# slothfulxtx/Texture-GS

Hardware: AMD Instinct MI355X
Metric: fwd+bwd views/sec @800x800, 300k Gaussians + 1024^2 texture; HBM GB/s vs roofline (higher is better)
Workload: dtype f32; 1 GPU; c3: N=300000 Gaussians, cubemap 6x1024x1024x3 f32, 800x800, fwd+bwd, sh_degree 3; parallelism=views sharded dp1, view_pipeline=3 HIP streams, order=accumulate, forwards begun one view per stream ahead, grad_allreduce=none (1 GPU)

## Files before the change

### include/texgs.h

```cpp
#ifndef TEXGS_H
#define TEXGS_H

#include <stddef.h>
#include <stdint.h>

#ifdef __cplusplus
extern "C" {
#endif

#define TEXGS_ABI_VERSION 19
#define TEXGS_TILE 16
#define TEXGS_REC_TEST_FLOATS 8
#define TEXGS_REC_SHADE_FLOATS 20
#define TEXGS_ACC_FLOATS 32

typedef struct TexGSFrame {
    int32_t image_height;
    int32_t image_width;
    float   tanfovx;
    float   tanfovy;
    float   scale_modifier;
    int32_t sh_degree;
    int32_t sh_coeffs;
    int32_t tex_res;
    int32_t num_gaussians;
    int32_t debug;
    const float* bg;
    const float* viewmatrix;
    const float* projmatrix;
    const float* campos;
} TexGSFrame;

typedef struct TexGSInputs {
    const float* means3D;
    const float* shs;
    const float* opacities;
    const float* scales;
    const float* rotations;
    const float* uvs;
    const float* gradient_uvs;
    const float* texture;
    const float* color_offset;
    const float* cov3D_precomp;
} TexGSInputs;

typedef struct TexGSGeom {
    float*    rec_test;
    float*    rec_shade;
    float*    depth;
    int32_t*  radii;
    uint32_t* rect;
    uint32_t* tiles_touched;
    uint32_t* offsets;
    void*     scan_temp;
    size_t    scan_temp_bytes;
} TexGSGeom;

typedef struct TexGSBinning {
    uint32_t  num_rendered;
    uint64_t* keys_unsorted;
    uint64_t* keys_sorted;
    uint32_t* point_list;
    uint32_t* ranges;
    uint32_t* tile_order;
    void*     sort_temp;
    size_t    sort_temp_bytes;
} TexGSBinning;

typedef struct TexGSImage {
    float*    out_color;
    float*    out_depth;
    float*    out_norm;
    float*    out_alpha;
    float*    final_T;
    uint32_t* n_contrib;
    uint32_t* tex_bin_count;
    uint32_t* survivors;
    uint16_t* surv_qmask;
    uint32_t* surv_count;
    uint32_t* tex_bin_resv;
} TexGSImage;
#define TEXGS_RESV_WORDS 192

#define TEXGS_ACC_MEANS3D 1
#define TEXGS_ACC_MEANS2D 2
#define TEXGS_ACC_SHS 4
#define TEXGS_ACC_OPACITIES 8
#define TEXGS_ACC_SCALES 16
#define TEXGS_ACC_ROTATIONS 32
#define TEXGS_ACC_UVS 64
#define TEXGS_ACC_COLOR_OFFSET 128
#define TEXGS_ACC_COV3D 256
#define TEXGS_ACC_ALL 511

#define TEXGS_WANT_TEXTURE   1
#define TEXGS_WANT_GAUSSIANS 2
#define TEXGS_WANT_ALL       3

typedef struct TexGSGrads {
    const float* dL_dcolor;
    const float* dL_ddepth;
    const float* dL_dnorm;
    const float* dL_dalpha;
    float* acc;
    float* dL_dmeans3D;
    float* dL_dmeans2D;
    float* dL_dshs;
    float* dL_dopacities;
    float* dL_dscales;
    float* dL_drotations;
    float* dL_duvs;
    float* dL_dtexture;
    float* dL_dcolor_offset;
    float* dL_dcov3D;
    uint32_t want;
    float*    tex_bins;
    uint32_t* tex_bin_cursor;
    uint32_t* tex_bin_base;
    uint32_t  tex_rec_cap;
    int32_t accumulate;
} TexGSGrads;

int         texgs_abi_version(void);
const char* texgs_build_id(void);
const char* texgs_last_error(void);

size_t texgs_scan_temp_bytes(int32_t num_gaussians);
size_t texgs_sort_temp_bytes(uint32_t num_rendered, uint32_t num_tiles);
size_t texgs_tex_bin_count(int32_t tex_res);
#define TEXGS_TEXBIN_RECORD_FLOATS 4

int texgs_preprocess_forward(const TexGSFrame* frame, const TexGSInputs* in, TexGSGeom* geom, void* stream);

size_t texgs_num_rendered_words(int32_t num_gaussians);
int texgs_num_rendered_begin(const TexGSGeom* geom, int32_t num_gaussians, uint32_t* host_pinned, size_t host_words, int32_t sort_first,
                             void* stream);
int texgs_num_rendered_reduce(const uint32_t* host_pinned, int32_t num_gaussians, uint32_t* host_out, uint64_t* fingerprint_out);
int texgs_depth_sort_scan(TexGSGeom* geom, int32_t num_gaussians, void* stream);

int texgs_bin_sort_render_forward(const TexGSFrame* frame, const TexGSInputs* in, const TexGSGeom* geom,
                                  TexGSBinning* bin, TexGSImage* img, void* stream);

int texgs_render_forward(const TexGSFrame* frame, const TexGSInputs* in, const TexGSGeom* geom,
                         const TexGSBinning* bin, TexGSImage* img, void* stream);

int texgs_backward(const TexGSFrame* frame, const TexGSInputs* in, const TexGSGeom* geom,
                   const TexGSBinning* bin, const TexGSImage* img, TexGSGrads* grads, void* stream);

int texgs_backward_render(const TexGSFrame* frame, const TexGSInputs* in, const TexGSGeom* geom,
                          const TexGSBinning* bin, const TexGSImage* img, TexGSGrads* grads, void* stream);
int texgs_backward_preprocess(const TexGSFrame* frame, const TexGSInputs* in, const TexGSGeom* geom, TexGSGrads* grads,
                              void* stream);

enum {
    TEXGS_K_PREPROCESS_FWD = 0, TEXGS_K_SCAN = 1, TEXGS_K_DUPLICATE = 2, TEXGS_K_SORT = 3, TEXGS_K_RANGES = 4,
    TEXGS_K_RENDER_FWD = 5, TEXGS_K_RENDER_BWD = 6, TEXGS_K_PREPROCESS_BWD = 7, TEXGS_K_TEXGRAD_REDUCE = 8,
    TEXGS_NUM_KERNELS = 9
};
int texgs_profile_enable(int on);
int texgs_profile_select(uint32_t kernel_mask);
int texgs_profile_read(float* ms_sum_host, uint32_t* launches_host);

int texgs_rgb_alpha_loss(const float* image, const float* gt_image, const float* alpha, const float* gt_alpha,
                         int32_t H, int32_t W, float lambda_dssim, float lambda_alpha, float* scratch, float* sums,
                         float* dL_dimage, float* dL_dalpha, void* stream);

int texgs_geom_losses(const float* norm, const float* gt_norm, const float* gt_image, const float* mask, const float* depth,
                      const float* gt_depth, int32_t H, int32_t W, float lambda_norm, float lambda_smooth, float gamma,
                      float lambda_depth, float* sums, float* dL_dnorm, float* dL_ddepth, void* stream);

int texgs_norm_from_depth(const float* depth, const float* viewmatrix, float tanfovx, float tanfovy, int32_t H, int32_t W,
                          float threshold, float* out_norm, float* out_mask, void* stream);

typedef struct TexGSUVNet {
    const float *W1, *b1;
    const float *W2, *b2;
    const float *emb;
    const float *W3, *b3, *W4, *b4;
    const float *W5, *b5;
    const float *xyz_offset, *xyz_scale;
    int32_t hidden;
} TexGSUVNet;
enum { TEXGS_UV_FP32 = 0, TEXGS_UV_BF16X3 = 1, TEXGS_UV_MIXED = 2 };
size_t texgs_uv_packed_bytes(int32_t precision);
int texgs_uv_pack(const TexGSUVNet* net, int32_t precision, void* packed, void* stream);
int texgs_uv_taylor_packed(const TexGSUVNet* net, int32_t precision, const void* packed, const float* xyz, int32_t N, float* uvs,
                           float* grad_uvs, void* stream);

typedef struct TexGSUVNetGrad {
    float *dW1, *db1;
    float *dW2, *db2;
    float *dW3, *db3, *dW4, *db4;
    float *dW5, *db5;
} TexGSUVNetGrad;
size_t texgs_uv_backward_temp_bytes(int32_t N);
int texgs_uv_backward(const TexGSUVNet* net, int32_t precision, const float* xyz, const float* g_uvs, int32_t N, const TexGSUVNetGrad* out,
                      void* temp, void* stream);

#define TEXGS_HASHGRID_MAX_LEVELS 16
#define TEXGS_HASHGRID_FEATURES 4
typedef struct TexGSHashGrid {
    int32_t n_levels;
    int32_t n_features;
    int32_t log2_hashmap_size;
    float   base_resolution;
    float   per_level_scale;
} TexGSHashGrid;
int texgs_hashgrid_levels(const TexGSHashGrid* grid, float* scale, uint32_t* res, uint32_t* size, uint32_t* offset, uint32_t* n_params);
int texgs_hashgrid_forward(const TexGSHashGrid* grid, const float* params, const float* x, int32_t N, float* enc, void* stream);
size_t texgs_hashgrid_backward_temp_bytes(const TexGSHashGrid* grid, int32_t N);
int texgs_hashgrid_backward(const TexGSHashGrid* grid, const float* params, const float* x, const float* d_enc, int32_t N,
                            float* d_params, float* d_x, void* temp, void* stream);
size_t texgs_chamfer_nn_temp_bytes(int32_t P);
int texgs_chamfer_nn(const float* a, int32_t P, const float* b, int32_t Q, float* d2, int32_t* idx, void* temp, void* stream);

size_t texgs_knn3_temp_bytes(int32_t n);
int texgs_knn3_mean_dist2(const float* xyz, int32_t n, float* mean_d2, void* temp, void* stream);
size_t texgs_fps_temp_bytes(int32_t n, int32_t k);
int texgs_farthest_points(const float* xyz, int32_t n, int32_t k, int32_t start, int32_t* idx, void* temp, void* stream);

#define TEXGS_CUBE_LINEAR 0
#define TEXGS_CUBE_NEAREST 1
int texgs_cube_sample(const float* tex, int32_t R, int32_t C, const float* dirs, int32_t N, int32_t filter, int32_t tap_map,
                      float* out, void* stream);
int texgs_cube_latlong(const float* tex, int32_t R, int32_t C, int32_t H, int32_t W, int32_t tap_map, float* out, void* stream);
int texgs_cube_sample_backward(const float* tex, int32_t R, int32_t C, const float* dirs, int32_t N, const float* g_out,
                               float* d_tex, float* d_dirs, void* stream);
int texgs_cube_sample_nearest_backward(int32_t R, int32_t C, const float* dirs, int32_t N, const float* g_out, float* d_tex,
                                       void* stream);

int texgs_density_stats(const float* grad, const int32_t* radii, int32_t n, float* accum, float* denom, float* max_radii, void* stream);

#define TEXGS_DENSITY_KEEP       1
#define TEXGS_DENSITY_CLONE      2
#define TEXGS_DENSITY_CLONE_KEPT 4
#define TEXGS_DENSITY_SPLIT      8
#define TEXGS_DENSITY_CHILD      16
typedef struct {
    const float* accum;
    const float* denom;
    const float* scaling;
    const float* opacity;
    int32_t n;
    float max_grad, min_opacity, dense_scale, big_scale;
    int32_t densify, use_big;
} TexGSDensityPlan;
size_t texgs_density_plan_temp_bytes(int32_t n);
int texgs_density_plan(const TexGSDensityPlan* plan, uint8_t* action, int32_t* rank, uint32_t* totals, void* temp, void* stream);

#define TEXGS_DENSITY_ROW_COPY    0
#define TEXGS_DENSITY_ROW_MOMENT  1
#define TEXGS_DENSITY_ROW_SCALING 2
#define TEXGS_DENSITY_ROW_XYZ     3
#define TEXGS_DENSITY_MAX_ROWS    24
typedef struct {
    const float* src;
    float* dst;
    int32_t width;
    int32_t kind;
} TexGSDensityRow;
typedef struct {
    TexGSDensityRow row[TEXGS_DENSITY_MAX_ROWS];
    int32_t rows;
    int32_t n;
    const uint8_t* action;
    const int32_t* rank;
    int32_t n_kept, n_clone, n_split, n_child;
    const float* scaling;
    const float* rotation;
    const float* noise;
} TexGSDensityMove;
int texgs_density_move(const TexGSDensityMove* move, void* stream);

#define TEXGS_METRICS_ROW     16
#define TEXGS_METRICS_L1      0
#define TEXGS_METRICS_SE      1
#define TEXGS_METRICS_SSIM    4
#define TEXGS_METRICS_MAE_NUM 7
#define TEXGS_METRICS_MAE_DEN 8
#define TEXGS_METRICS_PIXELS  9
#define TEXGS_METRICS_CROPPED 10
size_t texgs_eval_metrics_temp_bytes(int32_t H, int32_t W);
int texgs_eval_metrics(const float* image, const float* gt_image, const float* norm, const float* gt_norm, const float* alpha,
                       int32_t H, int32_t W, int32_t clamp01, void* temp, double* row, void* stream);

int texgs_selftest_waveops(const float* seed128, float* out576, void* stream);

int texgs_mark_visible(const TexGSFrame* frame, const float* means3D, uint8_t* visible, void* stream);

#ifdef __cplusplus
}
#endif
#endif
```

### texture-gs_amd/build.py

```python
import os
import subprocess
import sys

HERE = os.path.dirname(os.path.abspath(__file__))
ROOT = os.path.dirname(HERE)
CSRC = os.path.join(HERE, "csrc")
OBJ = os.path.join(HERE, "build")
LIB = os.path.join(HERE, os.environ.get("TEXGS_LIB_NAME", "libtexgs.so"))
OBJ = os.path.join(HERE, os.environ.get("TEXGS_OBJ_DIR", "build"))
HIPCC = os.environ.get("HIPCC", "/opt/rocm/bin/hipcc")

COMMON = ["--offload-arch=gfx950", "-O3", "-std=c++17", "-fPIC", "-I" + os.path.join(ROOT, "include"),
          "-I" + CSRC, "-Wall"]
UNITS = {
    "preprocess.hip": ["-ffp-contract=off"],
    "binning.hip": [],
    "render.hip": ["-munsafe-fp-atomics", "-ffp-contract=fast", "-fno-slp-vectorize"],
    "loss.hip": [],
    "selftest.hip": [],
    "uvnet.hip": [],
    "uvmap.hip": ["-munsafe-fp-atomics"],
    "points.hip": ["-ffp-contract=off"],
    "cubetex.hip": ["-munsafe-fp-atomics"],
    "density.hip": ["-ffp-contract=off"],
    "metrics.hip": ["-ffp-contract=off"],
    "optim.hip": ["-ffp-contract=off"],
    "abi.hip": [],
}
HEADERS = [os.path.join(CSRC, "common.h"), os.path.join(CSRC, "wave_ops.h"), os.path.join(CSRC, "render_bwd_body.h"),
           os.path.join(ROOT, "include", "texgs.h"), os.path.join(ROOT, "include", "texgs_optim.h")]


def build_id():
    import hashlib
    h = hashlib.sha256()
    files = sorted(os.path.join(CSRC, f) for f in os.listdir(CSRC) if f.endswith((".hip", ".h"))) \
        + [os.path.join(ROOT, "include", "texgs.h"), os.path.join(ROOT, "include", "texgs_optim.h")]
    for f in files:
        h.update(os.path.basename(f).encode())
        h.update(open(f, "rb").read())
    h.update(repr((COMMON[:4], sorted(UNITS.items()), os.environ.get("TEXGS_EXTRA_FLAGS", ""))).encode())
    return h.hexdigest()[:16]


def _newer(src_list, target):
    if not os.path.exists(target):
        return True
    t = os.path.getmtime(target)
    return any(os.path.getmtime(s) > t for s in src_list)


def build(force=False, verbose=False):
    os.makedirs(OBJ, exist_ok=True)
    objs = []
    bid = build_id()
    idfile = os.path.join(OBJ, "build_id.txt")
    stale_id = not os.path.exists(idfile) or open(idfile).read().strip() != bid
    for src, flags in UNITS.items():
        sp = os.path.join(CSRC, src)
        op = os.path.join(OBJ, src.replace(".hip", ".o"))
        objs.append(op)
        if src == "abi.hip":
            flags = flags + ['-DTEXGS_BUILD_ID="%s"' % bid]
        if force or _newer([sp] + HEADERS + [os.path.abspath(__file__)], op) or (src == "abi.hip" and stale_id):
            cmd = [HIPCC] + COMMON + flags + os.environ.get("TEXGS_EXTRA_FLAGS", "").split() + ["-c", sp, "-o", op]
            if verbose:
                print(" ".join(cmd), flush=True)
            subprocess.check_call(cmd)
    if force or _newer(objs, LIB):
        cmd = [HIPCC, "--offload-arch=gfx950", "-shared", "-fPIC", "-o", LIB] + objs
        if verbose:
            print(" ".join(cmd), flush=True)
        subprocess.check_call(cmd)
    with open(idfile, "w") as f:
        f.write(bid + "\n")
    return LIB


if __name__ == "__main__":
    print(build(force="--force" in sys.argv, verbose="--verbose" in sys.argv or True))
```

### texture-gs_amd/csrc/abi.hip

```cpp
#include "common.h"
#include <stdio.h>
#include <stdlib.h>

#include <mutex>
#include <vector>

namespace {

thread_local char g_err[512] = "";

struct EvRec { int kid; hipEvent_t a, b; };
std::mutex g_prof_mu;
bool g_prof_on = false;
uint32_t g_prof_mask = 0xFFFFFFFFu;
std::vector<EvRec> g_prof_log;
std::vector<hipEvent_t> g_prof_free;

hipEvent_t prof_event() {
    if (!g_prof_free.empty()) { hipEvent_t e = g_prof_free.back(); g_prof_free.pop_back(); return e; }
    hipEvent_t e = nullptr;
    return hipEventCreate(&e) == hipSuccess ? e : nullptr;
}

struct ProfScope {
    int kid; hipStream_t s; hipEvent_t a; bool on;
    ProfScope(int k, hipStream_t st) : kid(k), s(st), a(nullptr), on(false) {
        std::lock_guard<std::mutex> l(g_prof_mu);
        if (g_prof_on && ((g_prof_mask >> k) & 1u)) { a = prof_event(); on = a != nullptr; if (on) (void)hipEventRecord(a, s); }
    }
    ~ProfScope() {
        if (!on) return;
        std::lock_guard<std::mutex> l(g_prof_mu);
        hipEvent_t b = prof_event();
        if (!b) { g_prof_free.push_back(a); return; }
        (void)hipEventRecord(b, s);
        g_prof_log.push_back({kid, a, b});
    }
};

int fail(const char* where, hipError_t e) {
    snprintf(g_err, sizeof(g_err), "%s: %s", where, hipGetErrorString(e));
    return (int)e ? (int)e : -1;
}

int fail_msg(const char* msg) {
    snprintf(g_err, sizeof(g_err), "%s", msg);
    return -1;
}

int launched(const char* where, hipError_t st, hipStream_t s, bool debug) {
    if (st == hipSuccess && debug) st = hipStreamSynchronize(s);
    return st == hipSuccess ? 0 : fail(where, st);
}

int validate_frame(const TexGSFrame* f) {
    if (!f) return fail_msg("frame is NULL");
    if (f->image_height <= 0 || f->image_width <= 0) return fail_msg("image size must be positive");
    if (f->image_width > 65535 * TEXGS_TILE || f->image_height > 65535 * TEXGS_TILE) return fail_msg("image too large");
    {
        const long long tx = (f->image_width + TEXGS_TILE - 1) / TEXGS_TILE, ty = (f->image_height + TEXGS_TILE - 1) / TEXGS_TILE;
        if (tx * ty > (1ll << 24)) return fail_msg("image too large: more than 2^24 tiles");
    }
    if (f->sh_degree < 0 || f->sh_degree > 3) return fail_msg("sh_degree must be in [0,3]");
    if (f->num_gaussians < 0) return fail_msg("num_gaussians < 0");
    if (f->tex_res <= 0) return fail_msg("tex_res must be positive");
    if (f->tex_res > 7168) return fail_msg("tex_res > 7168: the blend kernels address texels with 32-bit byte offsets (6 R^2 x 12 B < 2^32)");
    if (!f->bg || !f->viewmatrix || !f->projmatrix || !f->campos) return fail_msg("frame device pointers must be non-NULL");
    return 0;
}

}

extern "C" {

int texgs_abi_version(void) { return TEXGS_ABI_VERSION; }

#ifndef TEXGS_BUILD_ID
#define TEXGS_BUILD_ID "unknown"
#endif
const char* texgs_build_id(void) { return TEXGS_BUILD_ID; }

const char* texgs_last_error(void) { return g_err; }

size_t texgs_scan_temp_bytes(int32_t num_gaussians) { return scan_temp_bytes(num_gaussians); }

size_t texgs_sort_temp_bytes(uint32_t num_rendered, uint32_t num_tiles) { return sort_temp_bytes(num_rendered, num_tiles); }

size_t texgs_tex_bin_count(int32_t tex_res) { return tex_bin_count(tex_res); }

int texgs_preprocess_forward(const TexGSFrame* frame, const TexGSInputs* in, TexGSGeom* geom, void* stream) {
    if (int r = validate_frame(frame)) return r;
    if (!in || !geom) return fail_msg("NULL argument");
    if (frame->num_gaussians == 0) return 0;
    if (!in->means3D || !in->opacities) return fail_msg("per-Gaussian input pointer is NULL");
    if (in->texture && (!in->uvs || !in->gradient_uvs)) return fail_msg("uvs / gradient_uvs are required with a texture");
    if (in->cov3D_precomp && in->texture) return fail_msg("cov3D_precomp is an input of the untextured surface only (texture must be NULL)");
    if (!in->cov3D_precomp && (!in->scales || !in->rotations)) return fail_msg("scales and rotations (or cov3D_precomp) are required");
    if (geom->scan_temp_bytes < scan_temp_bytes(frame->num_gaussians)) return fail_msg("scan_temp too small");
    hipStream_t s = (hipStream_t)stream;
    const CamConst c = make_cam(frame);
    hipError_t st;
    { ProfScope p(TEXGS_K_PREPROCESS_FWD, s); st = launch_preprocess_fwd(c, frame, in, geom, s); }
    return launched("preprocess_fwd", st, s, frame->debug);
}

static int depth_sort_scan(const TexGSGeom* geom, int32_t num_gaussians, hipStream_t s, bool debug) {
    if (num_gaussians == 0) return 0;
    hipError_t st;
    { ProfScope p(TEXGS_K_SCAN, s); st = launch_depth_sort_scan(geom, num_gaussians, s); }
    return launched("depth sort / scan", st, s, debug);
}

size_t texgs_num_rendered_words(int32_t num_gaussians) {
    return num_gaussians <= 0 ? 0 : 3 * (((size_t)num_gaussians + TG_BLOCK - 1) / TG_BLOCK);
}
int texgs_num_rendered_begin(const TexGSGeom* geom, int32_t num_gaussians, uint32_t* host_pinned, size_t host_words, int32_t sort_first,
                             void* stream) {
    if (!geom || !host_pinned) return fail_msg("NULL argument");
    if (num_gaussians <= 0) return 0;
    const size_t nw = texgs_num_rendered_words(num_gaussians);
    if (host_words < nw) return fail_msg("host buffer too small (texgs_num_rendered_words)");
    hipStream_t s = (hipStream_t)stream;
    hipError_t e = hipMemcpyAsync(host_pinned, bin_block_sums_ptr(geom, num_gaussians), nw * sizeof(uint32_t), hipMemcpyDeviceToHost, s);
    if (e != hipSuccess) return fail("num_rendered readback", e);
    return sort_first ? depth_sort_scan(geom, num_gaussians, s, false) : 0;
}
int texgs_num_rendered_reduce(const uint32_t* host_pinned, int32_t num_gaussians, uint32_t* host_out, uint64_t* fingerprint_out) {
    if (!host_pinned || !host_out) return fail_msg("NULL argument");
    *host_out = 0;
    if (fingerprint_out) *fingerprint_out = 0;
    if (num_gaussians <= 0) return 0;
    const size_t nblk = ((size_t)num_gaussians + TG_BLOCK - 1) / TG_BLOCK;
    unsigned long long total = 0ull;
    uint32_t fa = 0u, fb = 0u;
    for (size_t k = 0; k < nblk; ++k) { total += host_pinned[k]; fa += host_pinned[nblk + k]; fb += host_pinned[2 * nblk + k]; }
    if (total > 0xFFFFFFFFull) return fail_msg("num_rendered exceeds 2^32 - 1 instances");
    *host_out = (uint32_t)total;
    if (fingerprint_out) *fingerprint_out = ((uint64_t)fb << 32) | (uint64_t)fa;
    return 0;
}

int texgs_depth_sort_scan(TexGSGeom* geom, int32_t num_gaussians, void* stream) {
    if (!geom) return fail_msg("NULL argument");
    return depth_sort_scan(geom, num_gaussians, (hipStream_t)stream, false);
}

static int render_forward_impl(const TexGSFrame* frame, const TexGSInputs* in, const TexGSGeom* geom,
                               const TexGSBinning* bin, TexGSImage* img, void* stream, bool counters_zeroed) {
    if (int r = validate_frame(frame)) return r;
    if (!in || !geom || !bin || !img) return fail_msg("NULL argument");
    hipStream_t s = (hipStream_t)stream;
    const CamConst c = make_cam(frame);
    if (img->tex_bin_count && in->texture && !counters_zeroed) {
        hipError_t e = hipMemsetAsync(img->tex_bin_count, 0, sizeof(uint32_t) * 2 * tex_bin_count(c.R), s);
        if (e != hipSuccess) return fail("tex_bin_count memset", e);
    }
    hipError_t st;
    { ProfScope p(TEXGS_K_RENDER_FWD, s); st = launch_render_fwd(c, frame, in, geom, bin, img, s); }
    return launched("render_fwd", st, s, frame->debug);
}

int texgs_render_forward(const TexGSFrame* frame, const TexGSInputs* in, const TexGSGeom* geom,
                         const TexGSBinning* bin, TexGSImage* img, void* stream) {
    return render_forward_impl(frame, in, geom, bin, img, stream, false);
}

int texgs_bin_sort_render_forward(const TexGSFrame* frame, const TexGSInputs* in, const TexGSGeom* geom,
                                  TexGSBinning* bin, TexGSImage* img, void* stream) {
    if (int r = validate_frame(frame)) return r;
    if (!in || !geom || !bin || !img) return fail_msg("NULL argument");
    hipStream_t s = (hipStream_t)stream;
    const CamConst c = make_cam(frame);
    hipError_t st;
    if (bin->num_rendered > 0) {
        if (bin->sort_temp_bytes < sort_temp_bytes(bin->num_rendered, (uint32_t)(c.tiles_x * c.tiles_y))) return fail_msg("sort_temp too small");
        { ProfScope p(TEXGS_K_DUPLICATE, s); st = launch_duplicate(c, geom, bin, s); }
        if (int r = launched("duplicate_with_keys", st, s, frame->debug)) return r;
        { ProfScope p(TEXGS_K_SORT, s); st = launch_sort(c, geom, bin, s); }
        if (int r = launched("tile sort", st, s, frame->debug)) return r;
    }
    { ProfScope p(TEXGS_K_RANGES, s);
      st = launch_ranges(c, bin, img->tex_bin_count, img->tex_bin_count ? 2 * (int)tex_bin_count(c.R) : 0, s); }
    if (int r = launched("tile_ranges", st, s, frame->debug)) return r;
    return render_forward_impl(frame, in, geom, bin, img, stream, true);
}

int texgs_backward_render(const TexGSFrame* frame, const TexGSInputs* in, const TexGSGeom* geom,
                          const TexGSBinning* bin, const TexGSImage* img, TexGSGrads* grads, void* stream) {
    if (int r = validate_frame(frame)) return r;
    if (!in || !geom || !bin || !img || !grads) return fail_msg("NULL argument");
    if (!(grads->want & TEXGS_WANT_ALL)) return fail_msg("TexGSGrads.want is empty: ask for TEXGS_WANT_TEXTURE and / or TEXGS_WANT_GAUSSIANS");
    if ((grads->want & TEXGS_WANT_GAUSSIANS) && !grads->acc) return fail_msg("acc must be allocated (zero-filled) when Gaussian gradients are wanted");
    if ((grads->want & TEXGS_WANT_TEXTURE) && in->texture && !grads->dL_dtexture) return fail_msg("dL_dtexture must be allocated (zero-filled) when the texture gradient is wanted");
    if (!img->survivors || !img->surv_qmask || !img->surv_count)
        return fail_msg("the forward of this call left no survivor lists (TexGSImage.survivors / surv_qmask / surv_count were NULL): "
                        "run the forward with them to be able to run its backward");
    hipStream_t s = (hipStream_t)stream;
    const CamConst c = make_cam(frame);
    if (bin->num_rendered > 0) {
        hipError_t st;
        { ProfScope p(TEXGS_K_RENDER_BWD, s); st = launch_render_bwd(c, frame, in, geom, bin, img, grads, s); }
        if (int r = launched("render_bwd", st, s, frame->debug)) return r;
        if (tex_bins_enabled(c, in, img, grads)) {
            { ProfScope p(TEXGS_K_TEXGRAD_REDUCE, s); st = launch_texgrad_reduce(c, img, grads, s); }
            return launched("texgrad_reduce", st, s, frame->debug);
        }
    }
    return 0;
}

int texgs_backward_preprocess(const TexGSFrame* frame, const TexGSInputs* in, const TexGSGeom* geom, TexGSGrads* grads,
                              void* stream) {
    if (int r = validate_frame(frame)) return r;
    if (!in || !geom || !grads) return fail_msg("NULL argument");
    if (!(grads->want & TEXGS_WANT_GAUSSIANS)) return 0;
    if (!grads->acc) return fail_msg("acc must be allocated");
    if (in->cov3D_precomp && !grads->dL_dcov3D) return fail_msg("dL_dcov3D is required with cov3D_precomp");
    hipStream_t s = (hipStream_t)stream;
    const CamConst c = make_cam(frame);
    hipError_t st;
    { ProfScope p(TEXGS_K_PREPROCESS_BWD, s); st = launch_preprocess_bwd(c, frame, in, geom, grads, s); }
    return launched("preprocess_bwd", st, s, frame->debug);
}

int texgs_backward(const TexGSFrame* frame, const TexGSInputs* in, const TexGSGeom* geom,
                   const TexGSBinning* bin, const TexGSImage* img, TexGSGrads* grads, void* stream) {
    if (int r = texgs_backward_render(frame, in, geom, bin, img, grads, stream)) return r;
    return texgs_backward_preprocess(frame, in, geom, grads, stream);
}

int texgs_profile_enable(int on) {
    std::lock_guard<std::mutex> l(g_prof_mu);
    g_prof_on = on != 0;
    if (!g_prof_on) {
        for (auto& r : g_prof_log) { g_prof_free.push_back(r.a); g_prof_free.push_back(r.b); }
        g_prof_log.clear();
    }
    return 0;
}

int texgs_profile_select(uint32_t kernel_mask) {
    std::lock_guard<std::mutex> l(g_prof_mu);
    g_prof_mask = kernel_mask;
    return 0;
}

int texgs_profile_read(float* ms_sum_host, uint32_t* launches_host) {
    if (!ms_sum_host || !launches_host) return fail_msg("NULL argument");
    std::lock_guard<std::mutex> l(g_prof_mu);
    for (auto& r : g_prof_log) {
        hipError_t e = hipEventSynchronize(r.b);
        if (e != hipSuccess) return fail("profile event sync", e);
        float ms = 0.f;
        e = hipEventElapsedTime(&ms, r.a, r.b);
        if (e != hipSuccess) return fail("profile elapsed", e);
        if (r.kid >= 0 && r.kid < TEXGS_NUM_KERNELS) { ms_sum_host[r.kid] += ms; launches_host[r.kid] += 1; }
        g_prof_free.push_back(r.a); g_prof_free.push_back(r.b);
    }
    g_prof_log.clear();
    return 0;
}

int texgs_rgb_alpha_loss(const float* image, const float* gt_image, const float* alpha, const float* gt_alpha,
                         int32_t H, int32_t W, float lambda_dssim, float lambda_alpha, float* scratch, float* sums,
                         float* dL_dimage, float* dL_dalpha, void* stream) {
    if (!image || !gt_image || !scratch || !sums || !dL_dimage) return fail_msg("NULL argument");
    if (H <= 0 || W <= 0) return fail_msg("image size must be positive");
    hipStream_t s = (hipStream_t)stream;
    return launched("rgb_alpha_loss", launch_rgb_alpha_loss(image, gt_image, alpha, gt_alpha, H, W, lambda_dssim, lambda_alpha, scratch,
                                                            sums, dL_dimage, dL_dalpha, s), s, false);
}

int texgs_geom_losses(const float* norm, const float* gt_norm, const float* gt_image, const float* mask, const float* depth,
                      const float* gt_depth, int32_t H, int32_t W, float lambda_norm, float lambda_smooth, float gamma,
                      float lambda_depth, float* sums, float* dL_dnorm, float* dL_ddepth, void* stream) {
    if (!sums) return fail_msg("NULL argument");
    if (H <= 0 || W <= 0 || !(gamma > 0.f)) return fail_msg("image size and gamma must be positive");
    if (lambda_norm != 0.f && (!norm || !gt_norm || !dL_dnorm)) return fail_msg("norm term needs norm, gt_norm, dL_dnorm");
    if (lambda_smooth != 0.f && (!norm || !gt_image || !dL_dnorm)) return fail_msg("smoothness term needs norm, gt_image, dL_dnorm");
    if (lambda_depth != 0.f && (!depth || !gt_depth || !dL_ddepth)) return fail_msg("depth term needs depth, gt_depth, dL_ddepth");
    hipStream_t s = (hipStream_t)stream;
    return launched("geom_losses", launch_geom_losses(norm, gt_norm, gt_image, mask, depth, gt_depth, H, W, lambda_norm, lambda_smooth,
                                                      gamma, lambda_depth, sums, dL_dnorm, dL_ddepth, s), s, false);
}

int texgs_norm_from_depth(const float* depth, const float* viewmatrix, float tanfovx, float tanfovy, int32_t H, int32_t W,
                          float threshold, float* out_norm, float* out_mask, void* stream) {
    if (!depth || !viewmatrix || !out_norm || !out_mask) return fail_msg("NULL argument");
    if (H <= 0 || W <= 0) return fail_msg("image size must be positive");
    hipStream_t s = (hipStream_t)stream;
    return launched("norm_from_depth", launch_norm_from_depth(depth, viewmatrix, tanfovx, tanfovy, H, W, threshold, out_norm, out_mask, s),
                    s, false);
}

static int check_uvnet(const TexGSUVNet* net, int32_t precision) {
    if (precision != TEXGS_UV_FP32 && precision != TEXGS_UV_BF16X3 && precision != TEXGS_UV_MIXED)
        return fail_msg("precision must be TEXGS_UV_FP32, TEXGS_UV_BF16X3 or TEXGS_UV_MIXED");
    if (net->hidden != 128) return fail_msg("the UV-map kernels support the shipped UVNet shape only (hidden width 128)");
    if (!net->W1 || !net->W2 || !net->W3 || !net->W4 || !net->W5 || !net->emb) return fail_msg("weight pointer is NULL");
    return 0;
}

size_t texgs_uv_packed_bytes(int32_t precision) { return uv_packed_bytes(precision); }

int texgs_uv_pack(const TexGSUVNet* net, int32_t precision, void* packed, void* stream) {
    if (!net || !packed) return fail_msg("NULL argument");
    if (int r = check_uvnet(net, precision)) return r;
    hipStream_t s = (hipStream_t)stream;
    return launched("uv_pack", launch_uv_pack(net, precision, packed, s), s, false);
}

int texgs_uv_taylor_packed(const TexGSUVNet* net, int32_t precision, const void* packed, const float* xyz, int32_t N, float* uvs,
                           float* grad_uvs, void* stream) {
    if (!net || !packed) return fail_msg("NULL argument");
    if (int r = check_uvnet(net, precision)) return r;
    if (N < 0) return fail_msg("N < 0");
    if (N > 0 && (!xyz || !uvs || !grad_uvs)) return fail_msg("NULL argument");
    hipStream_t s = (hipStream_t)stream;
    return launched("uv_taylor", launch_uv_taylor_packed(net, precision, packed, xyz, N, uvs, grad_uvs, s), s, false);
}

size_t texgs_uv_backward_temp_bytes(int32_t N) { return uv_backward_temp_bytes(N < 0 ? 0 : N); }

int texgs_uv_backward(const TexGSUVNet* net, int32_t precision, const float* xyz, const float* g_uvs, int32_t N, const TexGSUVNetGrad* out,
                      void* temp, void* stream) {
    if (!net || !out || !temp) return fail_msg("NULL argument");
    if (int r = check_uvnet(net, precision)) return r;
    if (N < 0) return fail_msg("N < 0");
    if (N > 0 && (!xyz || !g_uvs)) return fail_msg("NULL argument");
    hipStream_t s = (hipStream_t)stream;
    return launched("uv_backward", launch_uv_backward(net, xyz, g_uvs, N, out, temp, precision != TEXGS_UV_FP32, s), s, false);
}

static int check_hashgrid(const TexGSHashGrid* g, uint32_t* n_params) {
    if (!g) return fail_msg("grid is NULL");
    float sc[TEXGS_HASHGRID_MAX_LEVELS];
    uint32_t r[TEXGS_HASHGRID_MAX_LEVELS], sz[TEXGS_HASHGRID_MAX_LEVELS], off[TEXGS_HASHGRID_MAX_LEVELS];
    switch (hashgrid_levels(g, sc, r, sz, off, n_params)) {
    case 0: return 0;
    case -1: return fail_msg("hash grid: n_levels must be in [1, 16]");
    case -2: return fail_msg("hash grid: n_features must be 4");
    case -3: return fail_msg("hash grid: log2_hashmap_size must be in [1, 24]");
    case -4: return fail_msg("hash grid: base_resolution must be >= 1 and per_level_scale in [1, 16]");
    case -5: return fail_msg("hash grid: a level's resolution is out of range");
    default: return fail_msg("hash grid: more than 2^31 parameters");
    }
}

int texgs_hashgrid_levels(const TexGSHashGrid* grid, float* scale, uint32_t* res, uint32_t* size, uint32_t* offset, uint32_t* n_params) {
    uint32_t n = 0;
    if (int r = check_hashgrid(grid, &n)) return r;
    float sc[TEXGS_HASHGRID_MAX_LEVELS];
    uint32_t rs[TEXGS_HASHGRID_MAX_LEVELS], sz[TEXGS_HASHGRID_MAX_LEVELS], off[TEXGS_HASHGRID_MAX_LEVELS];
    hashgrid_levels(grid, sc, rs, sz, off, &n);
    for (int l = 0; l < grid->n_levels; ++l) {
        if (scale) scale[l] = sc[l];
        if (res) res[l] = rs[l];
        if (size) size[l] = sz[l];
        if (offset) offset[l] = off[l];
    }
    if (n_params) *n_params = n;
    return 0;
}

int texgs_hashgrid_forward(const TexGSHashGrid* grid, const float* params, const float* x, int32_t N, float* enc, void* stream) {
    uint32_t n = 0;
    if (int r = check_hashgrid(grid, &n)) return r;
    if (N < 0) return fail_msg("N < 0");
    if ((int64_t)N * grid->n_levels * TEXGS_HASHGRID_FEATURES > INT32_MAX) return fail_msg("N * L * F >= 2^31");
    if (N > 0 && (!params || !x || !enc)) return fail_msg("NULL argument");
    if (N > 0 && (((uintptr_t)params | (uintptr_t)enc) & 15)) return fail_msg("params and enc must be 16-byte aligned");
    hipStream_t s = (hipStream_t)stream;
    return launched("hashgrid_forward", launch_hashgrid_forward(grid, params, x, N, enc, s), s, false);
}

size_t texgs_hashgrid_backward_temp_bytes(const TexGSHashGrid* grid, int32_t N) {
    uint32_t n = 0;
    if (!grid || check_hashgrid(grid, &n)) return 0;
    return hashgrid_backward_temp_bytes(grid, N);
}

int texgs_hashgrid_backward(const TexGSHashGrid* grid, const float* params, const float* x, const float* d_enc, int32_t N,
                            float* d_params, float* d_x, void* temp, void* stream) {
    uint32_t n = 0;
    if (int r = check_hashgrid(grid, &n)) return r;
    if (N < 0) return fail_msg("N < 0");
    if ((int64_t)N * grid->n_levels * TEXGS_HASHGRID_FEATURES > INT32_MAX) return fail_msg("N * L * F >= 2^31");
    if (N > 0 && (!params || !x || !d_enc)) return fail_msg("NULL argument");
    if (N > 0 && (((uintptr_t)params | (uintptr_t)d_enc | (uintptr_t)d_params) & 15))
        return fail_msg("params, d_enc and d_params must be 16-byte aligned");
    if (N > 0 && d_x && !temp) return fail_msg("temp is NULL (d_x needs texgs_hashgrid_backward_temp_bytes)");
    hipStream_t s = (hipStream_t)stream;
    return launched("hashgrid_backward", launch_hashgrid_backward(grid, params, x, d_enc, N, d_params, d_x, temp, s), s, false);
}

size_t texgs_chamfer_nn_temp_bytes(int32_t P) { return chamfer_nn_temp_bytes(P); }

int texgs_chamfer_nn(const float* a, int32_t P, const float* b, int32_t Q, float* d2, int32_t* idx, void* temp, void* stream) {
    if (P < 0) return fail_msg("P < 0");
    if (Q < 1) return fail_msg("the reference set is empty (Q < 1)");
    if ((int64_t)Q > 65535ll * 512) return fail_msg("Q > 65535 * 512");
    if (P > 0 && (!a || !b || !d2 || !idx || !temp)) return fail_msg("NULL argument");
    hipStream_t s = (hipStream_t)stream;
    return launched("chamfer_nn", launch_chamfer_nn(a, P, b, Q, d2, idx, temp, s), s, false);
}

size_t texgs_knn3_temp_bytes(int32_t n) { return knn3_temp_bytes(n); }

int texgs_knn3_mean_dist2(const float* xyz, int32_t n, float* mean_d2, void* temp, void* stream) {
    if (n < 4) return fail_msg("n < 4: three nearest other points need at least four points");
    if (!xyz || !mean_d2 || !temp) return fail_msg("NULL argument");
    hipStream_t s = (hipStream_t)stream;
    return launched("knn3_mean_dist2", launch_knn3_mean_dist2(xyz, n, mean_d2, temp, s), s, false);
}

size_t texgs_fps_temp_bytes(int32_t n, int32_t k) { return fps_temp_bytes(n, k); }

int texgs_farthest_points(const float* xyz, int32_t n, int32_t k, int32_t start, int32_t* idx, void* temp, void* stream) {
    if (n < 1) return fail_msg("n < 1");
    if (k < 1 || k > n) return fail_msg("k must be in [1, n]");
    if (start < 0 || start >= n) return fail_msg("start must be in [0, n)");
    if (!xyz || !idx || !temp) return fail_msg("NULL argument");
    hipStream_t s = (hipStream_t)stream;
    return launched("farthest_points", launch_farthest_points(xyz, n, k, start, idx, temp, s), s, false);
}

static int cube_shape_ok(int32_t R, int32_t C) {
    if (R < 2) return fail_msg("R < 2: a cubemap face needs at least 2 x 2 texels");
    if (C < 1) return fail_msg("C < 1");
    if (6ll * R * R * C >= (1ll << 31)) return fail_msg("6 R R C must be below 2^31");
    return 0;
}

int texgs_cube_sample(const float* tex, int32_t R, int32_t C, const float* dirs, int32_t N, int32_t filter, int32_t tap_map,
                      float* out, void* stream) {
    if (int r = cube_shape_ok(R, C)) return r;
    if (N < 0) return fail_msg("N < 0");
    if (filter != TEXGS_CUBE_LINEAR && filter != TEXGS_CUBE_NEAREST) return fail_msg("filter must be TEXGS_CUBE_LINEAR or TEXGS_CUBE_NEAREST");
    if (!tex || (N > 0 && (!dirs || !out))) return fail_msg("NULL argument");
    hipStream_t s = (hipStream_t)stream;
    return launched("cube_sample", launch_cube_sample(tex, R, C, dirs, N, filter, tap_map, out, s), s, false);
}

int texgs_cube_latlong(const float* tex, int32_t R, int32_t C, int32_t H, int32_t W, int32_t tap_map, float* out, void* stream) {
    if (int r = cube_shape_ok(R, C)) return r;
    if (H < 1 || W < 1) return fail_msg("H and W must be positive");
    if ((long long)H * W >= (1ll << 31)) return fail_msg("H W must be below 2^31");
    if (!tex || !out) return fail_msg("NULL argument");
    hipStream_t s = (hipStream_t)stream;
    return launched("cube_latlong", launch_cube_latlong(tex, R, C, H, W, tap_map, out, s), s, false);
}

int texgs_cube_sample_backward(const float* tex, int32_t R, int32_t C, const float* dirs, int32_t N, const float* g_out,
                               float* d_tex, float* d_dirs, void* stream) {
    if (int r = cube_shape_ok(R, C)) return r;
    if (N < 0) return fail_msg("N < 0");
    if (!d_tex && !d_dirs) return fail_msg("d_tex and d_dirs are both NULL: nothing to compute");
    if ((d_dirs && !tex) || (N > 0 && (!dirs || !g_out))) return fail_msg("NULL argument");
    hipStream_t s = (hipStream_t)stream;
    return launched("cube_sample_backward", launch_cube_sample_backward(tex, R, C, dirs, N, g_out, d_tex, d_dirs, s), s, false);
}

int texgs_cube_sample_nearest_backward(int32_t R, int32_t C, const float* dirs, int32_t N, const float* g_out, float* d_tex,
                                       void* stream) {
    if (int r = cube_shape_ok(R, C)) return r;
    if (N < 0) return fail_msg("N < 0");
    if (!d_tex || (N > 0 && (!dirs || !g_out))) return fail_msg("NULL argument");
    hipStream_t s = (hipStream_t)stream;
    return launched("cube_sample_nearest_backward", launch_cube_sample_nearest_backward(R, C, dirs, N, g_out, d_tex, s), s, false);
}

int texgs_density_stats(const float* grad, const int32_t* radii, int32_t n, float* accum, float* denom, float* max_radii, void* stream) {
    if (n < 0) return fail_msg("n < 0");
    if (n > 0 && (!grad || !radii || !accum || !denom || !max_radii)) return fail_msg("NULL argument");
    hipStream_t s = (hipStream_t)stream;
    return launched("density_stats", launch_density_stats(grad, radii, n, accum, denom, max_radii, s), s, false);
}

size_t texgs_density_plan_temp_bytes(int32_t n) { return density_plan_temp_bytes(n); }

int texgs_density_plan(const TexGSDensityPlan* plan, uint8_t* action, int32_t* rank, uint32_t* totals, void* temp, void* stream) {
    if (!plan || !totals) return fail_msg("NULL argument");
    if (plan->n < 0) return fail_msg("n < 0");
    if (plan->n > 0 && (!plan->scaling || !plan->opacity || !action || !rank || !temp)) return fail_msg("NULL argument");
    if (plan->n > 0 && plan->densify && (!plan->accum || !plan->denom)) return fail_msg("accum and denom are required to densify");
    if (plan->densify && !(plan->max_grad > 0.0f)) return fail_msg("max_grad must be positive (with 0 the reference splits its own clones)");
    hipStream_t s = (hipStream_t)stream;
    return launched("density_plan", launch_density_plan(plan, action, rank, totals, temp, s), s, false);
}

int texgs_density_move(const TexGSDensityMove* m, void* stream) {
    if (!m) return fail_msg("NULL argument");
    if (m->n < 0 || m->n_kept < 0 || m->n_clone < 0 || m->n_split < 0 || m->n_child < 0) return fail_msg("negative count");
    if (m->n_kept > m->n || m->n_clone > m->n || m->n_split > m->n || m->n_child > m->n_split) return fail_msg("totals exceed n");
    if ((int64_t)m->n_kept + m->n_clone + 2ll * m->n_child >= (1ll << 31)) return fail_msg("the new row count reaches 2^31");
    if (m->rows < 0 || m->rows > TEXGS_DENSITY_MAX_ROWS) return fail_msg("rows must be in [0, TEXGS_DENSITY_MAX_ROWS]");
    if (m->n == 0 || m->rows == 0) return 0;
    if (!m->action || !m->rank) return fail_msg("NULL argument");
    const bool out_rows = m->n_kept + m->n_clone + m->n_child > 0;
    for (int d = 0; d < m->rows; ++d) {
        const TexGSDensityRow& r = m->row[d];
        if (r.width < 1) return fail_msg("row width < 1");
        if (r.kind < TEXGS_DENSITY_ROW_COPY || r.kind > TEXGS_DENSITY_ROW_XYZ) return fail_msg("unknown row kind");
        if (r.kind == TEXGS_DENSITY_ROW_XYZ && r.width != 3) return fail_msg("an XYZ row has width 3");
        if (!r.src || (out_rows && !r.dst)) return fail_msg("NULL row pointer");
        if (r.kind == TEXGS_DENSITY_ROW_XYZ && m->n_child > 0 && (!m->scaling || !m->rotation || !m->noise))
            return fail_msg("an XYZ row with children needs scaling, rotation and noise");
    }
    if (!out_rows) return 0;
    return launched("density_move", launch_density_move(m, (hipStream_t)stream), (hipStream_t)stream, false);
}

size_t texgs_eval_metrics_temp_bytes(int32_t H, int32_t W) { return eval_metrics_temp_bytes(H, W); }

int texgs_eval_metrics(const float* image, const float* gt_image, const float* norm, const float* gt_norm, const float* alpha,
                       int32_t H, int32_t W, int32_t clamp01, void* temp, double* row, void* stream) {
    if (!image || !gt_image || !temp || !row) return fail_msg("NULL argument");
    if (H < 7 || W < 7) return fail_msg("H and W must be at least 7: the 7x7 SSIM window does not fit");
    if ((!norm) != (!gt_norm)) return fail_msg("norm and gt_norm must be both NULL or both set");
    if ((((int64_t)W + 31) / 32) * (((int64_t)H + 31) / 32) >= (1ll << 31)) return fail_msg("image too large: 2^31 tiles or more");
    hipStream_t s = (hipStream_t)stream;
    return launched("eval_metrics", launch_eval_metrics(image, gt_image, norm, gt_norm, alpha, H, W, clamp01 != 0, temp, row, s), s, false);
}

int texgs_adam_step(const TexGSAdamTensor* tensors, int32_t count, int32_t zero_grads, void* stream) {
    if (count < 0) return fail_msg("count < 0");
    if (count == 0) return 0;
    if (!tensors) return fail_msg("tensors is NULL");
    for (int32_t k = 0; k < count; ++k) {
        const TexGSAdamTensor& t = tensors[k];
        if (t.numel < 0) return fail_msg("numel < 0");
        if (t.numel == 0) continue;
        if (!t.p || !t.g || !t.m || !t.v) return fail_msg("NULL pointer (p, g, m or v) in a record with numel > 0");
        if (((uintptr_t)t.p | (uintptr_t)t.g | (uintptr_t)t.m | (uintptr_t)t.v) & 3)
            return fail_msg("p, g, m and v must be 4-byte aligned");
    }
    hipStream_t s = (hipStream_t)stream;
    for (int32_t first = 0; first < count; first += TEXGS_ADAM_MAX_TENSORS) {
        const int32_t n = count - first < TEXGS_ADAM_MAX_TENSORS ? count - first : TEXGS_ADAM_MAX_TENSORS;
        if (int r = launched("adam_step", launch_adam_step(tensors + first, n, zero_grads, s), s, false)) return r;
    }
    return 0;
}

int texgs_selftest_waveops(const float* seed128, float* out576, void* stream) {
    if (!seed128 || !out576) return fail_msg("NULL argument");
    return launched("selftest_waveops", launch_selftest_waveops(seed128, out576, (hipStream_t)stream), (hipStream_t)stream, false);
}

int texgs_mark_visible(const TexGSFrame* frame, const float* means3D, uint8_t* visible, void* stream) {
    if (int r = validate_frame(frame)) return r;
    if (!means3D || !visible) return fail_msg("NULL argument");
    hipStream_t s = (hipStream_t)stream;
    return launched("mark_visible", launch_mark_visible(frame, means3D, visible, s), s, frame->debug);
}

}
```

### texture-gs_amd/csrc/common.h

```cpp
#pragma once
#include <hip/hip_runtime.h>
#include <stdint.h>
#include "texgs.h"
#include "texgs_optim.h"

#define TG_NEAR_Z        0.2f
#define TG_LOWPASS       0.3f
#define TG_FRUSTUM_CLAMP 1.3f
#define TG_ALPHA_MAX     0.99f
#define TG_ALPHA_MIN     (1.0f / 255.0f)
#define TG_T_EPS         1e-4f
#define TG_PLANE_EPS     5e-2f
#define TG_DEN_MIN       0.2f
#define TG_MA_MIN        1e-20f
#define TG_SH_C0         0.28209479177387814f

enum {
    R_XY = 0, R_CONIC = 2, R_OP = 5, R_G2 = 6, R_GM = 8, R_PHI = 14, R_VD = 17, R_DEPTH = 20, R_N = 21
};
enum {
    M_P = 0, M_DEN = 6, M_DN = 9, M_PHI = 18, M_VD = 21, M_DEPTH = 24, M_N = 25
};

#define TG_BLOCK 256

struct CamConst {
    int W, H, tiles_x, tiles_y;
    float fx, fy, tanfovx, tanfovy;
    float scale_modifier;
    int sh_degree, sh_coeffs, R, N;
};

static inline CamConst make_cam(const TexGSFrame* f) {
    CamConst c;
    c.W = f->image_width; c.H = f->image_height;
    c.tiles_x = (c.W + TEXGS_TILE - 1) / TEXGS_TILE;
    c.tiles_y = (c.H + TEXGS_TILE - 1) / TEXGS_TILE;
    c.tanfovx = f->tanfovx; c.tanfovy = f->tanfovy;
    c.fx = (float)c.W / (2.0f * f->tanfovx);
    c.fy = (float)c.H / (2.0f * f->tanfovy);
    c.scale_modifier = f->scale_modifier;
    c.sh_degree = f->sh_degree; c.sh_coeffs = f->sh_coeffs; c.R = f->tex_res; c.N = f->num_gaussians;
    return c;
}

struct LaunchStatus {
    hipError_t first = hipSuccess;
    void operator+=(hipError_t e) { if (first == hipSuccess) first = e; }
    hipError_t after_launches() { *this += hipGetLastError(); return first; }
};

hipError_t launch_preprocess_fwd(const CamConst& c, const TexGSFrame* f, const TexGSInputs* in, TexGSGeom* g, hipStream_t s);
hipError_t launch_preprocess_bwd(const CamConst& c, const TexGSFrame* f, const TexGSInputs* in, const TexGSGeom* g,
                           TexGSGrads* gr, hipStream_t s);
hipError_t launch_mark_visible(const TexGSFrame* f, const float* means3D, uint8_t* visible, hipStream_t s);
hipError_t launch_depth_sort_scan(const TexGSGeom* g, int N, hipStream_t s);
uint32_t* bin_block_sums_ptr(const TexGSGeom* g, int N);
uint32_t* bin_header_ptr(const TexGSGeom* g, int N, int* words);
size_t scan_temp_bytes(int N);
size_t sort_temp_bytes(uint32_t D, uint32_t T);
hipError_t launch_duplicate(const CamConst& c, const TexGSGeom* g, TexGSBinning* b, hipStream_t s);
hipError_t launch_sort(const CamConst& c, const TexGSGeom* g, TexGSBinning* b, hipStream_t s);
hipError_t launch_ranges(const CamConst& c, TexGSBinning* b, uint32_t* zero_words, int num_zero_words, hipStream_t s);
hipError_t launch_render_fwd(const CamConst& c, const TexGSFrame* f, const TexGSInputs* in, const TexGSGeom* g,
                       const TexGSBinning* b, TexGSImage* img, hipStream_t s);
size_t tex_bin_count(int R);
bool tex_bins_enabled(const CamConst& c, const TexGSInputs* in, const TexGSImage* img, const TexGSGrads* gr);
hipError_t launch_texgrad_reduce(const CamConst& c, const TexGSImage* img, TexGSGrads* gr, hipStream_t s);
hipError_t launch_render_bwd(const CamConst& c, const TexGSFrame* f, const TexGSInputs* in, const TexGSGeom* g,
                       const TexGSBinning* b, const TexGSImage* img, TexGSGrads* gr, hipStream_t s);
hipError_t launch_rgb_alpha_loss(const float* image, const float* gt_image, const float* alpha, const float* gt_alpha, int H,
                          int W, float lambda_dssim, float lambda_alpha, float* scratch, float* sums, float* d_image,
                          float* d_alpha, hipStream_t s);
hipError_t launch_selftest_waveops(const float* seed128, float* out576, hipStream_t s);
hipError_t launch_geom_losses(const float* norm, const float* gt_norm, const float* gt_image, const float* mask, const float* depth,
                       const float* gt_depth, int H, int W, float lambda_norm, float lambda_smooth, float gamma,
                       float lambda_depth, float* sums, float* d_norm, float* d_depth, hipStream_t s);
hipError_t launch_norm_from_depth(const float* depth, const float* viewmatrix, float tanfovx, float tanfovy, int H, int W, float threshold,
                           float* out_norm, float* out_mask, hipStream_t s);
size_t uv_packed_bytes(int precision);
hipError_t launch_uv_pack(const TexGSUVNet* net, int precision, void* packed, hipStream_t s);
hipError_t launch_uv_taylor_packed(const TexGSUVNet* net, int precision, const void* packed, const float* xyz, int N, float* uvs, float* grad_uvs,
                            hipStream_t s);
size_t uv_backward_temp_bytes(int N);
hipError_t launch_uv_backward(const TexGSUVNet* net, const float* xyz, const float* g, int N, const TexGSUVNetGrad* out, void* temp, int mixed,
                       hipStream_t s);
int hashgrid_levels(const TexGSHashGrid* g, float* scale, uint32_t* res, uint32_t* size, uint32_t* offset, uint32_t* n_params);
hipError_t launch_hashgrid_forward(const TexGSHashGrid* g, const float* params, const float* x, int N, float* enc, hipStream_t s);
size_t hashgrid_backward_temp_bytes(const TexGSHashGrid* g, int N);
hipError_t launch_hashgrid_backward(const TexGSHashGrid* g, const float* params, const float* x, const float* d_enc, int N, float* d_params,
                             float* d_x, void* temp, hipStream_t s);
size_t chamfer_nn_temp_bytes(int P);
hipError_t launch_chamfer_nn(const float* a, int P, const float* b, int Q, float* d2, int32_t* idx, void* temp, hipStream_t s);
size_t sort_pairs32_temp_bytes(uint32_t n);
hipError_t launch_sort_pairs32(const uint32_t* keys_in, uint32_t n, int key_bits, uint32_t* keys_out, uint32_t* vals_out, void* temp, hipStream_t s);
size_t knn3_temp_bytes(int n);
hipError_t launch_knn3_mean_dist2(const float* xyz, int n, float* mean_d2, void* temp, hipStream_t s);
size_t fps_temp_bytes(int n, int k);
hipError_t launch_farthest_points(const float* xyz, int n, int k, int start, int32_t* idx, void* temp, hipStream_t s);
hipError_t launch_cube_sample(const float* tex, int R, int C, const float* dirs, int N, int filter, int tap_map, float* out, hipStream_t s);
hipError_t launch_cube_latlong(const float* tex, int R, int C, int H, int W, int tap_map, float* out, hipStream_t s);
hipError_t launch_cube_sample_backward(const float* tex, int R, int C, const float* dirs, int N, const float* g_out, float* d_tex,
                                float* d_dirs, hipStream_t s);
hipError_t launch_cube_sample_nearest_backward(int R, int C, const float* dirs, int N, const float* g_out, float* d_tex, hipStream_t s);
hipError_t launch_density_stats(const float* grad, const int32_t* radii, int n, float* accum, float* denom, float* max_radii, hipStream_t s);
size_t density_plan_temp_bytes(int n);
hipError_t launch_density_plan(const TexGSDensityPlan* p, uint8_t* action, int32_t* rank, uint32_t* totals, void* temp, hipStream_t s);
hipError_t launch_density_move(const TexGSDensityMove* m, hipStream_t s);
size_t eval_metrics_temp_bytes(int H, int W);
hipError_t launch_eval_metrics(const float* image, const float* gt_image, const float* norm, const float* gt_norm, const float* alpha, int H,
                        int W, int clamp01, void* temp, double* row, hipStream_t s);
hipError_t launch_adam_step(const TexGSAdamTensor* tensors, int count, int zero_grads, hipStream_t s);
```

### texture-gs_amd/csrc/preprocess.hip

```cpp
#include "common.h"

namespace {

struct Frame {
    float V[16];
    float P[16];
    float cam[3];
};

__device__ __forceinline__ Frame load_frame(const float* vm, const float* pm, const float* cp) {
    Frame f;
#pragma unroll
    for (int i = 0; i < 16; ++i) { f.V[i] = vm[i]; f.P[i] = pm[i]; }
    f.cam[0] = cp[0]; f.cam[1] = cp[1]; f.cam[2] = cp[2];
    return f;
}

struct Geo {
    bool  valid;
    float m[3], t[3];
    float hx, hy, hw, pw, xy[2];
    float q[4], s[3], R[9], M[9], S[6];
    float txc, tyc; bool clx, cly;
    float J00, J02, J11, J12, T0[3], T1[3];
    float a, b, c, det, inv, conic[3];
    int   radius;
    int   kmin; float sign; float n[3];
    float nv[3], sdot; bool degen; float gx, gy, G[6], K[9];
    float dir[3], dlen;
};

#define WR(F, r, c) ((F).V[(c) * 4 + (r)])

__device__ __forceinline__ void smallest_eigvec(const float* S6, float* n) {
    const float tr = S6[0] + S6[3] + S6[5];
    const float sc = (tr > 0.f) ? 1.0f / tr : 1.0f;
    float a00 = S6[0] * sc, a01 = S6[1] * sc, a02 = S6[2] * sc, a11 = S6[3] * sc, a12 = S6[4] * sc, a22 = S6[5] * sc;
    float v00 = 1.f, v01 = 0.f, v02 = 0.f, v10 = 0.f, v11 = 1.f, v12 = 0.f, v20 = 0.f, v21 = 0.f, v22 = 1.f;
    auto rot = [](float& app, float& aqq, float& apq, float& arp, float& arq, float& v0p, float& v0q, float& v1p, float& v1q,
                  float& v2p, float& v2q) {
        if (fabsf(apq) < 1e-30f) return;
        const float theta = (aqq - app) / (2.0f * apq);
        const float t = ((theta >= 0.f) ? 1.0f : -1.0f) / (fabsf(theta) + sqrtf(theta * theta + 1.0f));
        const float c = 1.0f / sqrtf(t * t + 1.0f), sn = t * c;
        app -= t * apq; aqq += t * apq; apq = 0.f;
        const float rp = arp, rq = arq;
        arp = c * rp - sn * rq; arq = sn * rp + c * rq;
        float x;
        x = v0p; v0p = c * x - sn * v0q; v0q = sn * x + c * v0q;
        x = v1p; v1p = c * x - sn * v1q; v1q = sn * x + c * v1q;
        x = v2p; v2p = c * x - sn * v2q; v2q = sn * x + c * v2q;
    };
#pragma unroll 1
    for (int sweep = 0; sweep < 6; ++sweep) {
        rot(a00, a11, a01, a02, a12, v00, v01, v10, v11, v20, v21);
        rot(a00, a22, a02, a01, a12, v00, v02, v10, v12, v20, v22);
        rot(a11, a22, a12, a01, a02, v01, v02, v11, v12, v21, v22);
    }
    int k = 0; float m = a00;
    if (a11 < m) { m = a11; k = 1; }
    if (a22 < m) { m = a22; k = 2; }
    n[0] = (k == 0) ? v00 : ((k == 1) ? v01 : v02);
    n[1] = (k == 0) ? v10 : ((k == 1) ? v11 : v12);
    n[2] = (k == 0) ? v20 : ((k == 1) ? v21 : v22);
}

template <bool COV = false>
__device__ __forceinline__ void geo_forward(Geo& g, const Frame& F, const CamConst& C, int i,
                                            const float* __restrict__ means, const float* __restrict__ scales,
                                            const float* __restrict__ rots, const float* __restrict__ juv,
                                            const float* __restrict__ cov6 = nullptr) {
    g.m[0] = means[3 * i + 0]; g.m[1] = means[3 * i + 1]; g.m[2] = means[3 * i + 2];
    const float mx = g.m[0], my = g.m[1], mz = g.m[2];
    g.t[0] = F.V[0] * mx + F.V[4] * my + F.V[8] * mz + F.V[12];
    g.t[1] = F.V[1] * mx + F.V[5] * my + F.V[9] * mz + F.V[13];
    g.t[2] = F.V[2] * mx + F.V[6] * my + F.V[10] * mz + F.V[14];
    g.valid = g.t[2] > TG_NEAR_Z;
    g.radius = 0;
    if (!g.valid) return;
    const float tx = g.t[0], ty = g.t[1], tz = g.t[2];

    g.hx = F.P[0] * mx + F.P[4] * my + F.P[8] * mz + F.P[12];
    g.hy = F.P[1] * mx + F.P[5] * my + F.P[9] * mz + F.P[13];
    g.hw = F.P[3] * mx + F.P[7] * my + F.P[11] * mz + F.P[15];
    g.pw = 1.0f / (g.hw + 1e-7f);
    const float ndcx = g.hx * g.pw, ndcy = g.hy * g.pw;
    g.xy[0] = ((ndcx + 1.0f) * (float)C.W - 1.0f) * 0.5f;
    g.xy[1] = ((ndcy + 1.0f) * (float)C.H - 1.0f) * 0.5f;

    float s0 = 0.f, s1 = 0.f, s2 = 0.f;
    if constexpr (COV) {
#pragma unroll
        for (int k = 0; k < 6; ++k) g.S[k] = cov6[6 * i + k];
#pragma unroll
        for (int k = 0; k < 9; ++k) { g.R[k] = 0.f; g.M[k] = 0.f; }
        g.q[0] = g.q[1] = g.q[2] = g.q[3] = 0.f; g.s[0] = g.s[1] = g.s[2] = 0.f;
    } else {
    g.q[0] = rots[4 * i + 0]; g.q[1] = rots[4 * i + 1]; g.q[2] = rots[4 * i + 2]; g.q[3] = rots[4 * i + 3];
    const float r = g.q[0], x = g.q[1], y = g.q[2], z = g.q[3];
    g.R[0] = 1.0f - 2.0f * (y * y + z * z); g.R[1] = 2.0f * (x * y - r * z); g.R[2] = 2.0f * (x * z + r * y);
    g.R[3] = 2.0f * (x * y + r * z); g.R[4] = 1.0f - 2.0f * (x * x + z * z); g.R[5] = 2.0f * (y * z - r * x);
    g.R[6] = 2.0f * (x * z - r * y); g.R[7] = 2.0f * (y * z + r * x); g.R[8] = 1.0f - 2.0f * (x * x + y * y);
    s0 = scales[3 * i + 0]; s1 = scales[3 * i + 1]; s2 = scales[3 * i + 2];
    g.s[0] = C.scale_modifier * s0; g.s[1] = C.scale_modifier * s1; g.s[2] = C.scale_modifier * s2;
#pragma unroll
    for (int rr = 0; rr < 3; ++rr)
#pragma unroll
        for (int cc = 0; cc < 3; ++cc) g.M[rr * 3 + cc] = g.R[rr * 3 + cc] * g.s[cc];
    const float* M = g.M;
    g.S[0] = M[0] * M[0] + M[1] * M[1] + M[2] * M[2];
    g.S[1] = M[0] * M[3] + M[1] * M[4] + M[2] * M[5];
    g.S[2] = M[0] * M[6] + M[1] * M[7] + M[2] * M[8];
    g.S[3] = M[3] * M[3] + M[4] * M[4] + M[5] * M[5];
    g.S[4] = M[3] * M[6] + M[4] * M[7] + M[5] * M[8];
    g.S[5] = M[6] * M[6] + M[7] * M[7] + M[8] * M[8];
    }

    const float limx = TG_FRUSTUM_CLAMP * C.tanfovx, limy = TG_FRUSTUM_CLAMP * C.tanfovy;
    const float txtz = tx / tz, tytz = ty / tz;
    g.clx = (txtz < -limx) || (txtz > limx);
    g.cly = (tytz < -limy) || (tytz > limy);
    g.txc = fminf(limx, fmaxf(-limx, txtz)) * tz;
    g.tyc = fminf(limy, fmaxf(-limy, tytz)) * tz;
    if (!g.clx) g.txc = tx;
    if (!g.cly) g.tyc = ty;
    const float tz2 = tz * tz;
    g.J00 = C.fx / tz; g.J02 = -(C.fx * g.txc) / tz2;
    g.J11 = C.fy / tz; g.J12 = -(C.fy * g.tyc) / tz2;
#pragma unroll
    for (int k = 0; k < 3; ++k) {
        g.T0[k] = g.J00 * WR(F, 0, k) + g.J02 * WR(F, 2, k);
        g.T1[k] = g.J11 * WR(F, 1, k) + g.J12 * WR(F, 2, k);
    }
    const float* S = g.S;
    const float v00 = S[0] * g.T0[0] + S[1] * g.T0[1] + S[2] * g.T0[2];
    const float v01 = S[1] * g.T0[0] + S[3] * g.T0[1] + S[4] * g.T0[2];
    const float v02 = S[2] * g.T0[0] + S[4] * g.T0[1] + S[5] * g.T0[2];
    const float v10 = S[0] * g.T1[0] + S[1] * g.T1[1] + S[2] * g.T1[2];
    const float v11 = S[1] * g.T1[0] + S[3] * g.T1[1] + S[4] * g.T1[2];
    const float v12 = S[2] * g.T1[0] + S[4] * g.T1[1] + S[5] * g.T1[2];
    g.a = (g.T0[0] * v00 + g.T0[1] * v01 + g.T0[2] * v02) + TG_LOWPASS;
    g.b = g.T1[0] * v00 + g.T1[1] * v01 + g.T1[2] * v02;
    g.c = (g.T1[0] * v10 + g.T1[1] * v11 + g.T1[2] * v12) + TG_LOWPASS;
    g.det = g.a * g.c - g.b * g.b;
    if (g.det == 0.0f) { g.valid = false; return; }
    g.inv = 1.0f / g.det;
    g.conic[0] = g.c * g.inv; g.conic[1] = -g.b * g.inv; g.conic[2] = g.a * g.inv;
    const float mid = 0.5f * (g.a + g.c);
    const float lam = mid + sqrtf(fmaxf(0.1f, mid * mid - g.det));
    g.radius = (int)ceilf(3.0f * sqrtf(lam));

    g.dir[0] = mx - F.cam[0]; g.dir[1] = my - F.cam[1]; g.dir[2] = mz - F.cam[2];
    float n0, n1, n2;
    if constexpr (COV) {
        float ev[3];
        smallest_eigvec(g.S, ev);
        n0 = ev[0]; n1 = ev[1]; n2 = ev[2];
        g.kmin = -1;
    } else {
        g.kmin = 0; float smin = s0;
        if (s1 < smin) { smin = s1; g.kmin = 1; }
        if (s2 < smin) { smin = s2; g.kmin = 2; }
        n0 = (g.kmin == 0) ? g.R[0] : ((g.kmin == 1) ? g.R[1] : g.R[2]);
        n1 = (g.kmin == 0) ? g.R[3] : ((g.kmin == 1) ? g.R[4] : g.R[5]);
        n2 = (g.kmin == 0) ? g.R[6] : ((g.kmin == 1) ? g.R[7] : g.R[8]);
    }
    g.sign = ((n0 * g.dir[0] + n1 * g.dir[1] + n2 * g.dir[2]) > 0.0f) ? -1.0f : 1.0f;
    g.n[0] = g.sign * n0; g.n[1] = g.sign * n1; g.n[2] = g.sign * n2;
    g.dlen = sqrtf(g.dir[0] * g.dir[0] + g.dir[1] * g.dir[1] + g.dir[2] * g.dir[2]);
    g.dir[0] /= g.dlen; g.dir[1] /= g.dlen; g.dir[2] /= g.dlen;

#pragma unroll
    for (int k = 0; k < 3; ++k)
        g.nv[k] = WR(F, k, 0) * g.n[0] + WR(F, k, 1) * g.n[1] + WR(F, k, 2) * g.n[2];
    g.sdot = g.nv[0] * tx + g.nv[1] * ty + g.nv[2] * tz;
    const float tn = sqrtf(tx * tx + ty * ty + tz * tz);
    g.degen = (juv == nullptr) || fabsf(g.sdot) <= TG_PLANE_EPS * tn;
#pragma unroll
    for (int rr = 0; rr < 3; ++rr)
#pragma unroll
        for (int cc = 0; cc < 3; ++cc)
            g.K[rr * 3 + cc] = (juv == nullptr) ? 0.0f
                             : juv[9 * i + rr * 3 + 0] * WR(F, cc, 0) + juv[9 * i + rr * 3 + 1] * WR(F, cc, 1)
                             + juv[9 * i + rr * 3 + 2] * WR(F, cc, 2);
    if (g.degen) {
        g.gx = 0.0f; g.gy = 0.0f;
#pragma unroll
        for (int k = 0; k < 6; ++k) g.G[k] = 0.0f;
    } else {
        const float ax = tz * g.nv[0] / g.sdot, ay = tz * g.nv[1] / g.sdot;
        g.gx = ax / C.fx; g.gy = ay / C.fy;
        const float B00 = tz / C.fx - tx * g.gx, B01 = -tx * g.gy;
        const float B10 = -ty * g.gx,            B11 = tz / C.fy - ty * g.gy;
        const float B20 = -tz * g.gx,            B21 = -tz * g.gy;
#pragma unroll
        for (int rr = 0; rr < 3; ++rr) {
            g.G[rr * 2 + 0] = g.K[rr * 3 + 0] * B00 + g.K[rr * 3 + 1] * B10 + g.K[rr * 3 + 2] * B20;
            g.G[rr * 2 + 1] = g.K[rr * 3 + 0] * B01 + g.K[rr * 3 + 1] * B11 + g.K[rr * 3 + 2] * B21;
        }
    }
}

__device__ __forceinline__ void tile_rect(const Geo& g, const CamConst& C, int& x0, int& y0, int& x1, int& y1) {
    const float rf = (float)g.radius;
    x0 = min(C.tiles_x, max(0, (int)((g.xy[0] - rf) / (float)TEXGS_TILE)));
    y0 = min(C.tiles_y, max(0, (int)((g.xy[1] - rf) / (float)TEXGS_TILE)));
    x1 = min(C.tiles_x, max(0, (int)((g.xy[0] + rf + (float)(TEXGS_TILE - 1)) / (float)TEXGS_TILE)));
    y1 = min(C.tiles_y, max(0, (int)((g.xy[1] + rf + (float)(TEXGS_TILE - 1)) / (float)TEXGS_TILE)));
}

__device__ __forceinline__ void sh_basis(int deg, float x, float y, float z, float* b) {
    const float C1 = 0.4886025119029199f;
    b[0] = -C1 * y; b[1] = C1 * z; b[2] = -C1 * x;
    if (deg > 1) {
        const float xx = x * x, yy = y * y, zz = z * z, xy = x * y, yz = y * z, xz = x * z;
        b[3] = 1.0925484305920792f * xy;
        b[4] = -1.0925484305920792f * yz;
        b[5] = 0.31539156525252005f * (2.0f * zz - xx - yy);
        b[6] = -1.0925484305920792f * xz;
        b[7] = 0.5462742152960396f * (xx - yy);
        if (deg > 2) {
            b[8]  = -0.5900435899266435f * y * (3.0f * xx - yy);
            b[9]  = 2.890611442640554f * xy * z;
            b[10] = -0.4570457994644658f * y * (4.0f * zz - xx - yy);
            b[11] = 0.3731763325901154f * z * (2.0f * zz - 3.0f * xx - 3.0f * yy);
            b[12] = -0.4570457994644658f * x * (4.0f * zz - xx - yy);
            b[13] = 1.445305721320277f * z * (xx - yy);
            b[14] = -0.5900435899266435f * x * (xx - 3.0f * yy);
        }
    }
}

__device__ __forceinline__ void sh_basis_grad(int deg, float x, float y, float z, float* bx, float* by, float* bz) {
    const float C1 = 0.4886025119029199f;
    bx[0] = 0.f; by[0] = -C1; bz[0] = 0.f;
    bx[1] = 0.f; by[1] = 0.f; bz[1] = C1;
    bx[2] = -C1; by[2] = 0.f; bz[2] = 0.f;
    if (deg > 1) {
        const float c20 = 1.0925484305920792f, c22 = 0.31539156525252005f, c24 = 0.5462742152960396f;
        bx[3] = c20 * y;   by[3] = c20 * x;   bz[3] = 0.f;
        bx[4] = 0.f;       by[4] = -c20 * z;  bz[4] = -c20 * y;
        bx[5] = c22 * (-2.0f * x); by[5] = c22 * (-2.0f * y); bz[5] = c22 * 4.0f * z;
        bx[6] = -c20 * z;  by[6] = 0.f;       bz[6] = -c20 * x;
        bx[7] = c24 * 2.0f * x; by[7] = -c24 * 2.0f * y; bz[7] = 0.f;
        if (deg > 2) {
            const float xx = x * x, yy = y * y, zz = z * z;
            const float c30 = -0.5900435899266435f, c31 = 2.890611442640554f, c32 = -0.4570457994644658f,
                        c33 = 0.3731763325901154f, c35 = 1.445305721320277f;
            bx[8]  = c30 * 6.0f * x * y;            by[8]  = c30 * (3.0f * xx - 3.0f * yy);        bz[8]  = 0.f;
            bx[9]  = c31 * y * z;                   by[9]  = c31 * x * z;                          bz[9]  = c31 * x * y;
            bx[10] = c32 * (-2.0f * x * y);         by[10] = c32 * (4.0f * zz - xx - 3.0f * yy);   bz[10] = c32 * 8.0f * y * z;
            bx[11] = c33 * (-6.0f * x * z);         by[11] = c33 * (-6.0f * y * z);                bz[11] = c33 * (6.0f * zz - 3.0f * xx - 3.0f * yy);
            bx[12] = c32 * (4.0f * zz - 3.0f * xx - yy); by[12] = c32 * (-2.0f * x * y);           bz[12] = c32 * 8.0f * x * z;
            bx[13] = c35 * 2.0f * x * z;            by[13] = -c35 * 2.0f * y * z;                  bz[13] = c35 * (xx - yy);
            bx[14] = c30 * (3.0f * xx - 3.0f * yy); by[14] = c30 * (-6.0f * x * y);                bz[14] = 0.f;
        }
    }
}

__device__ __forceinline__ int sh_active(int deg, int K) {
    const int want = (deg + 1) * (deg + 1) - 1;
    return want < K ? want : K;
}

template <int BLOCK, bool ADD>
__device__ __forceinline__ void sh_rows_out(float* __restrict__ g, const float* __restrict__ s, int count, bool vec) {
    const int tid = (int)threadIdx.x;
    int done = 0;
    if (vec) {
        const int n4 = count >> 2;
        float4* __restrict__ g4 = reinterpret_cast<float4*>(g);
        const float4* s4 = reinterpret_cast<const float4*>(s);
        for (int k = tid; k < n4; k += 4 * BLOCK) {
            float4 v[4], o[4];
            bool nz[4];
#pragma unroll
            for (int u = 0; u < 4; ++u) {
                const bool in = k + u * BLOCK < n4;
                v[u] = in ? s4[k + u * BLOCK] : make_float4(0.f, 0.f, 0.f, 0.f);
                nz[u] = in && (!ADD || v[u].x != 0.f || v[u].y != 0.f || v[u].z != 0.f || v[u].w != 0.f);
            }
            if (ADD) {
#pragma unroll
                for (int u = 0; u < 4; ++u) if (nz[u]) o[u] = g4[k + u * BLOCK];
#pragma unroll
                for (int u = 0; u < 4; ++u) if (nz[u]) g4[k + u * BLOCK] = make_float4(o[u].x + v[u].x, o[u].y + v[u].y, o[u].z + v[u].z, o[u].w + v[u].w);
            } else {
#pragma unroll
                for (int u = 0; u < 4; ++u) if (nz[u]) g4[k + u * BLOCK] = v[u];
            }
        }
        done = n4 << 2;
    }
    for (int k = done + tid; k < count; k += BLOCK) {
        const float v = s[k];
        if (ADD) { if (v != 0.f) g[k] += v; } else g[k] = v;
    }
}

template <bool COV>
__global__ void __launch_bounds__(TG_BLOCK)
k_preprocess_fwd(CamConst C, const float* __restrict__ vm, const float* __restrict__ pm, const float* __restrict__ cp,
                 const float* __restrict__ means, const float* __restrict__ shs, const float* __restrict__ opac,
                 const float* __restrict__ scales, const float* __restrict__ rots, const float* __restrict__ uvs,
                 const float* __restrict__ juv, const float* __restrict__ coff, const float* __restrict__ cov6,
                 float4* __restrict__ rec_test, float4* __restrict__ rec_shade, float* __restrict__ depth, int32_t* __restrict__ radii,
                 uint2* __restrict__ rect, uint32_t* __restrict__ tiles_touched, uint32_t* __restrict__ block_D,
                 uint32_t* __restrict__ zero_words, int num_zero_words) {
    extern __shared__ __attribute__((aligned(16))) float s_sh[];
    __shared__ uint32_t s_tt[5 * (TG_BLOCK / 64)];
    const int i = blockIdx.x * TG_BLOCK + threadIdx.x;
    const bool live = i < C.N;
    for (int k = i; k < num_zero_words; k += (int)gridDim.x * TG_BLOCK) zero_words[k] = 0u;
    const Frame F = load_frame(vm, pm, cp);
    Geo g;
    g.valid = false;
    if (live) geo_forward<COV>(g, F, C, i, means, scales, rots, juv, cov6);
    int x0 = 0, y0 = 0, x1 = 0, y1 = 0;
    if (g.valid) {
        tile_rect(g, C, x0, y0, x1, y1);
        if ((x1 - x0) * (y1 - y0) == 0) g.valid = false;
    }
    const int na = (shs != nullptr && C.sh_degree > 0) ? sh_active(C.sh_degree, C.sh_coeffs) : 0;
    const int row = 3 * C.sh_coeffs;
    if (na > 0) {
        const size_t first = (size_t)blockIdx.x * TG_BLOCK * row;
        const size_t total = (size_t)C.N * row;
        const int count = (int)min((size_t)TG_BLOCK * row, total - first);
        for (int k = threadIdx.x; k < count; k += TG_BLOCK) s_sh[k] = shs[first + k];
        __syncthreads();
    }
    uint32_t tt = 0u, ha = 0u, hb = 0u;
    if (live) {
        ha = (uint32_t)i * 0x9E3779B1u + 0x85EBCA77u;
        hb = ((uint32_t)i * 0xC2B2AE3Du) ^ 0x27D4EB2Fu;
    }
    auto mix = [&](uint32_t w) {
        ha = (ha ^ w) * 0x01000193u;
        hb = __builtin_rotateleft32(hb ^ w, 13) * 5u + 0xE6546B64u;
    };
    if (live && !g.valid) {
        radii[i] = 0; tiles_touched[i] = 0; rect[i] = make_uint2(0u, 0u);
        depth[i] = __uint_as_float(0xFFFFFFFFu);
        mix(0xFFFFFFFFu);
    }
    if (live && g.valid) {
    float vd[3] = {0.f, 0.f, 0.f};
    if (na > 0) {
        float b[15];
#pragma unroll
        for (int k = 0; k < 15; ++k) b[k] = 0.f;
        sh_basis(C.sh_degree, g.dir[0], g.dir[1], g.dir[2], b);
        const float* sp = s_sh + threadIdx.x * row;
#pragma unroll
        for (int k = 0; k < 15; ++k) {
            if (k < na) { vd[0] += b[k] * sp[3 * k + 0]; vd[1] += b[k] * sp[3 * k + 1]; vd[2] += b[k] * sp[3 * k + 2]; }
        }
    }
    if (coff) { vd[0] += coff[3 * i + 0]; vd[1] += coff[3 * i + 1]; vd[2] += coff[3 * i + 2]; }
    radii[i] = g.radius;
    tt = (uint32_t)((x1 - x0) * (y1 - y0));
    tiles_touched[i] = tt;
    depth[i] = g.t[2];
    const uint2 rc = make_uint2((uint32_t)x0 | ((uint32_t)y0 << 16), (uint32_t)x1 | ((uint32_t)y1 << 16));
    rect[i] = rc;
    const float op = opac[i];
    const float thr = (op > 0.0f) ? (-logf(255.0f * op) - 1e-3f) : 1.0f;
    const float cmid = 0.5f * (g.a + g.c);
    const float clam = cmid + sqrtf(fmaxf(0.1f, cmid * cmid - g.det));
    const float rcull = (thr < 0.0f) ? (sqrtf(-2.0f * thr * clam) * 1.001f + 0.01f) : -1.0f;
    const float4 t0 = make_float4(g.xy[0], g.xy[1], -0.5f * g.conic[0], -g.conic[1]);
    const float4 t1 = make_float4(-0.5f * g.conic[2], op, rcull, thr);
    const float4 s0 = make_float4(g.gx, g.gy, g.G[0], g.G[1]);
    const float4 s1 = make_float4(g.G[2], g.G[3], g.G[4], g.G[5]);
    const float4 s2 = uvs ? make_float4(uvs[3 * i + 0], uvs[3 * i + 1], uvs[3 * i + 2], vd[0]) : make_float4(0.f, 0.f, 1.f, vd[0]);
    float4* rt = rec_test + (size_t)i * (TEXGS_REC_TEST_FLOATS / 4);
    rt[0] = t0; rt[1] = t1;
    float4* rs = rec_shade + (size_t)i * (TEXGS_REC_SHADE_FLOATS / 4);
    rs[0] = s0; rs[1] = s1; rs[2] = s2;
    rs[3] = make_float4(vd[1], vd[2], g.t[2], g.n[0]);
    rs[4] = make_float4(g.n[1], g.n[2], g.xy[0], g.xy[1]);
    mix(__float_as_uint(g.t[2])); mix(rc.x); mix(rc.y);
    mix(__float_as_uint(t0.x)); mix(__float_as_uint(t0.y)); mix(__float_as_uint(t0.z)); mix(__float_as_uint(t0.w));
    mix(__float_as_uint(t1.x)); mix(__float_as_uint(t1.y)); mix(__float_as_uint(t1.z)); mix(__float_as_uint(t1.w));
    mix(__float_as_uint(s0.x)); mix(__float_as_uint(s0.y)); mix(__float_as_uint(s0.z)); mix(__float_as_uint(s0.w));
    mix(__float_as_uint(s1.x)); mix(__float_as_uint(s1.y)); mix(__float_as_uint(s1.z)); mix(__float_as_uint(s1.w));
    mix(__float_as_uint(s2.x)); mix(__float_as_uint(s2.y)); mix(__float_as_uint(s2.z));
    }
    ha ^= ha >> 15; ha *= 0x2C1B3C6Du; ha ^= ha >> 12;
    hb ^= hb >> 16; hb *= 0x85EBCA6Bu; hb ^= hb >> 13;
    if (!live) { ha = 0u; hb = 0u; }
    uint32_t kmin = (live && g.valid) ? __float_as_uint(g.t[2]) : 0xFFFFFFFFu, kmax = (live && g.valid) ? __float_as_uint(g.t[2]) : 0u;
    for (int d = 32; d >= 1; d >>= 1) {
        tt += __shfl_xor(tt, d, 64); ha += __shfl_xor(ha, d, 64); hb += __shfl_xor(hb, d, 64);
        kmin = min(kmin, (uint32_t)__shfl_xor((int)kmin, d, 64)); kmax = max(kmax, (uint32_t)__shfl_xor((int)kmax, d, 64));
    }
    constexpr int NW = TG_BLOCK / 64;
    if ((threadIdx.x & 63) == 0) {
        const int w = threadIdx.x >> 6;
        s_tt[w] = tt; s_tt[NW + w] = ha; s_tt[2 * NW + w] = hb; s_tt[3 * NW + w] = kmin; s_tt[4 * NW + w] = kmax;
    }
    __syncthreads();
    if (threadIdx.x < 5) {
        uint32_t r = s_tt[threadIdx.x * NW];
        for (int w = 1; w < NW; ++w) {
            const uint32_t v = s_tt[threadIdx.x * NW + w];
            r = (threadIdx.x < 3) ? r + v : ((threadIdx.x == 3) ? min(r, v) : max(r, v));
        }
        block_D[threadIdx.x * gridDim.x + blockIdx.x] = r;
    }
}

#ifndef K8_BLOCK
#define K8_BLOCK 256
#endif
template <bool COV>
__global__ void __launch_bounds__(K8_BLOCK)
k_preprocess_bwd(CamConst C, const float* __restrict__ vm, const float* __restrict__ pm, const float* __restrict__ cp,
                 const float* __restrict__ means, const float* __restrict__ shs, const float* __restrict__ opac,
                 const float* __restrict__ scales,
                 const float* __restrict__ rots, const float* __restrict__ juv, const float* __restrict__ cov6,
                 const int32_t* __restrict__ radii, float* __restrict__ acc,
                 float* __restrict__ d_means, float* __restrict__ d_means2D, float* __restrict__ d_shs,
                 float* __restrict__ d_op, float* __restrict__ d_scales, float* __restrict__ d_rots,
                 float* __restrict__ d_uvs, float* __restrict__ d_coff, float* __restrict__ d_cov6, int accumulate) {
    extern __shared__ __attribute__((aligned(16))) float s_sh[];
    const int i = blockIdx.x * K8_BLOCK + threadIdx.x;
    const int K = C.sh_coeffs;
    const bool live = i < C.N;
    const int row = 3 * K;
    const int na = (shs != nullptr && C.sh_degree > 0) ? sh_active(C.sh_degree, K) : 0;
    const size_t first = (size_t)blockIdx.x * K8_BLOCK * row;
    const int count = d_shs ? (int)min((size_t)K8_BLOCK * row, (size_t)C.N * row - first) : 0;
    const bool vec = d_shs && (((size_t)d_shs) & 15) == 0;
    if (na > 0 && d_shs) {
        for (int k = threadIdx.x; k < count; k += K8_BLOCK) s_sh[k] = shs[first + k];
        __syncthreads();
    }
    const bool visible = live && radii[i] > 0;
    if (live && !visible) {
        if (!(accumulate & TEXGS_ACC_MEANS3D)) d_means[3 * i] = d_means[3 * i + 1] = d_means[3 * i + 2] = 0.f;
        if (!(accumulate & TEXGS_ACC_MEANS2D)) d_means2D[3 * i] = d_means2D[3 * i + 1] = d_means2D[3 * i + 2] = 0.f;
        if (!(accumulate & TEXGS_ACC_OPACITIES)) d_op[i] = 0.f;
        if constexpr (COV) {
            if (!(accumulate & TEXGS_ACC_COV3D)) { for (int k = 0; k < 6; ++k) d_cov6[6 * i + k] = 0.f; }
        } else {
            if (!(accumulate & TEXGS_ACC_SCALES)) d_scales[3 * i] = d_scales[3 * i + 1] = d_scales[3 * i + 2] = 0.f;
            if (!(accumulate & TEXGS_ACC_ROTATIONS)) d_rots[4 * i] = d_rots[4 * i + 1] = d_rots[4 * i + 2] = d_rots[4 * i + 3] = 0.f;
        }
        if (d_uvs && !(accumulate & TEXGS_ACC_UVS)) d_uvs[3 * i] = d_uvs[3 * i + 1] = d_uvs[3 * i + 2] = 0.f;
        if (d_coff && !(accumulate & TEXGS_ACC_COLOR_OFFSET)) d_coff[3 * i] = d_coff[3 * i + 1] = d_coff[3 * i + 2] = 0.f;
    }
    if (visible) {
#define OUT(BIT, P, V) do { if (accumulate & (BIT)) (P) += (V); else (P) = (V); } while (0)
    const Frame F = load_frame(vm, pm, cp);
    Geo g;
    geo_forward<COV>(g, F, C, i, means, scales, rots, juv, cov6);
    float A[24];
    {
        float Mo[TEXGS_ACC_FLOATS];
        float4* ap = reinterpret_cast<float4*>(acc + (size_t)i * TEXGS_ACC_FLOATS);
#pragma unroll
        for (int k = 0; k < TEXGS_ACC_FLOATS / 4; ++k) {
            const float4 v = ap[k];
            Mo[4 * k] = v.x; Mo[4 * k + 1] = v.y; Mo[4 * k + 2] = v.z; Mo[4 * k + 3] = v.w;
            ap[k] = make_float4(0.f, 0.f, 0.f, 0.f);
        }
        const float ca = g.conic[0], cb = g.conic[1], cc = g.conic[2];
        const float m00 = Mo[M_P], m10 = Mo[M_P + 1], m01 = Mo[M_P + 2];
        const float N00 = Mo[M_DN], N10 = Mo[M_DN + 3], N20 = Mo[M_DN + 6], D0 = Mo[M_DEN];
        A[R_XY]     = -(ca * m10 + cb * m01) - ((g.G[0] * N00 + g.G[2] * N10 + g.G[4] * N20) + g.gx * D0);
        A[R_XY + 1] = -(cc * m01 + cb * m10) - ((g.G[1] * N00 + g.G[3] * N10 + g.G[5] * N20) + g.gy * D0);
        A[R_CONIC] = -0.5f * Mo[M_P + 3]; A[R_CONIC + 1] = -Mo[M_P + 4]; A[R_CONIC + 2] = -0.5f * Mo[M_P + 5];
        const float op = opac[i];
        A[R_OP] = (op > 0.0f) ? m00 / op : 0.0f;
        A[R_G2] = Mo[M_DEN + 1]; A[R_G2 + 1] = Mo[M_DEN + 2];
#pragma unroll
        for (int cidx = 0; cidx < 3; ++cidx) {
            A[R_GM + 2 * cidx] = Mo[M_DN + 3 * cidx + 1]; A[R_GM + 2 * cidx + 1] = Mo[M_DN + 3 * cidx + 2];
            A[R_PHI + cidx] = Mo[M_PHI + cidx]; A[R_VD + cidx] = Mo[M_VD + cidx]; A[R_N + cidx] = Mo[M_N + cidx];
        }
        A[R_DEPTH] = Mo[M_DEPTH];
    }
    const float tx = g.t[0], ty = g.t[1], tz = g.t[2];
    float dt[3] = {0.f, 0.f, 0.f};
    float dm[3] = {0.f, 0.f, 0.f};
    float dR[9];
#pragma unroll
    for (int k = 0; k < 9; ++k) dR[k] = 0.f;

    OUT(TEXGS_ACC_OPACITIES, d_op[i], A[R_OP]);
    if (d_uvs) { OUT(TEXGS_ACC_UVS, d_uvs[3 * i + 0], A[R_PHI]); OUT(TEXGS_ACC_UVS, d_uvs[3 * i + 1], A[R_PHI + 1]); OUT(TEXGS_ACC_UVS, d_uvs[3 * i + 2], A[R_PHI + 2]); }
    if (d_coff) { OUT(TEXGS_ACC_COLOR_OFFSET, d_coff[3 * i + 0], A[R_VD]); OUT(TEXGS_ACC_COLOR_OFFSET, d_coff[3 * i + 1], A[R_VD + 1]); OUT(TEXGS_ACC_COLOR_OFFSET, d_coff[3 * i + 2], A[R_VD + 2]); }

    const float dA = A[R_CONIC], dB = A[R_CONIC + 1], dC = A[R_CONIC + 2];
    const float inv = g.inv, inv2 = inv * inv;
    const float da = dA * (-g.c * g.c * inv2) + dB * (g.b * g.c * inv2) + dC * (inv - g.a * g.c * inv2);
    const float db = dA * (2.0f * g.b * g.c * inv2) + dB * (-inv - 2.0f * g.b * g.b * inv2) + dC * (2.0f * g.a * g.b * inv2);
    const float dc = dA * (inv - g.a * g.c * inv2) + dB * (g.a * g.b * inv2) + dC * (-g.a * g.a * inv2);
    const float hb = 0.5f * db;
    const float* S = g.S;
    float TS0[3], TS1[3];
    TS0[0] = g.T0[0] * S[0] + g.T0[1] * S[1] + g.T0[2] * S[2];
    TS0[1] = g.T0[0] * S[1] + g.T0[1] * S[3] + g.T0[2] * S[4];
    TS0[2] = g.T0[0] * S[2] + g.T0[1] * S[4] + g.T0[2] * S[5];
    TS1[0] = g.T1[0] * S[0] + g.T1[1] * S[1] + g.T1[2] * S[2];
    TS1[1] = g.T1[0] * S[1] + g.T1[1] * S[3] + g.T1[2] * S[4];
    TS1[2] = g.T1[0] * S[2] + g.T1[1] * S[4] + g.T1[2] * S[5];
    float dT0[3], dT1[3];
#pragma unroll
    for (int k = 0; k < 3; ++k) {
        dT0[k] = 2.0f * (da * TS0[k] + hb * TS1[k]);
        dT1[k] = 2.0f * (hb * TS0[k] + dc * TS1[k]);
    }
    float dS[9];
#pragma unroll
    for (int k = 0; k < 3; ++k)
#pragma unroll
        for (int l = 0; l < 3; ++l)
            dS[k * 3 + l] = g.T0[k] * g.T0[l] * da + (g.T0[k] * g.T1[l] + g.T1[k] * g.T0[l]) * hb + g.T1[k] * g.T1[l] * dc;
    float dM[9];
#pragma unroll
    for (int rr = 0; rr < 3; ++rr)
#pragma unroll
        for (int cc = 0; cc < 3; ++cc)
            dM[rr * 3 + cc] = 2.0f * (dS[rr * 3 + 0] * g.M[0 * 3 + cc] + dS[rr * 3 + 1] * g.M[1 * 3 + cc] + dS[rr * 3 + 2] * g.M[2 * 3 + cc]);
    float dscale[3];
#pragma unroll
    for (int cc = 0; cc < 3; ++cc) {
        dscale[cc] = (dM[0 + cc] * g.R[0 + cc] + dM[3 + cc] * g.R[3 + cc] + dM[6 + cc] * g.R[6 + cc]) * C.scale_modifier;
#pragma unroll
        for (int rr = 0; rr < 3; ++rr) dR[rr * 3 + cc] += dM[rr * 3 + cc] * g.s[cc];
    }
    const float dJ00 = dT0[0] * WR(F, 0, 0) + dT0[1] * WR(F, 0, 1) + dT0[2] * WR(F, 0, 2);
    const float dJ02 = dT0[0] * WR(F, 2, 0) + dT0[1] * WR(F, 2, 1) + dT0[2] * WR(F, 2, 2);
    const float dJ11 = dT1[0] * WR(F, 1, 0) + dT1[1] * WR(F, 1, 1) + dT1[2] * WR(F, 1, 2);
    const float dJ12 = dT1[0] * WR(F, 2, 0) + dT1[1] * WR(F, 2, 1) + dT1[2] * WR(F, 2, 2);
    const float tz2 = tz * tz, tz3 = tz2 * tz;
    dt[2] += -dJ00 * C.fx / tz2 - dJ11 * C.fy / tz2 + 2.0f * dJ02 * C.fx * g.txc / tz3 + 2.0f * dJ12 * C.fy * g.tyc / tz3;
    if (!g.clx) dt[0] += -dJ02 * C.fx / tz2;
    if (!g.cly) dt[1] += -dJ12 * C.fy / tz2;

    const float dndx = A[R_XY] * 0.5f * (float)C.W, dndy = A[R_XY + 1] * 0.5f * (float)C.H;
    OUT(TEXGS_ACC_MEANS2D, d_means2D[3 * i + 0], dndx); OUT(TEXGS_ACC_MEANS2D, d_means2D[3 * i + 1], dndy); if (!(accumulate & TEXGS_ACC_MEANS2D)) d_means2D[3 * i + 2] = 0.f;
    {
        const float dhx = dndx * g.pw, dhy = dndy * g.pw;
        const float dhw = -(dndx * g.hx + dndy * g.hy) * g.pw * g.pw;
#pragma unroll
        for (int k = 0; k < 3; ++k) dm[k] += dhx * F.P[k * 4 + 0] + dhy * F.P[k * 4 + 1] + dhw * F.P[k * 4 + 3];
    }
    dt[2] += A[R_DEPTH];
    float dn[3] = {A[R_N], A[R_N + 1], A[R_N + 2]};

    if (!g.degen) {
        const float* dG = &A[R_GM];
        float dBm[6];
#pragma unroll
        for (int k = 0; k < 3; ++k)
#pragma unroll
            for (int cc = 0; cc < 2; ++cc)
                dBm[k * 2 + cc] = g.K[0 * 3 + k] * dG[0 * 2 + cc] + g.K[1 * 3 + k] * dG[1 * 2 + cc] + g.K[2 * 3 + k] * dG[2 * 2 + cc];
        float dtz = dBm[0] / C.fx + dBm[3] / C.fy;
        float dgt[2];
#pragma unroll
        for (int cc = 0; cc < 2; ++cc)
            dgt[cc] = A[R_G2 + cc] - (dBm[0 * 2 + cc] * tx + dBm[1 * 2 + cc] * ty + dBm[2 * 2 + cc] * tz);
#pragma unroll
        for (int k = 0; k < 3; ++k) dt[k] -= dBm[k * 2 + 0] * g.gx + dBm[k * 2 + 1] * g.gy;
        const float dax = dgt[0] / C.fx, day = dgt[1] / C.fy;
        const float dot_a_nv = dax * g.nv[0] + day * g.nv[1];
        dtz += dot_a_nv / g.sdot;
        float dnv[3] = {tz * dax / g.sdot, tz * day / g.sdot, 0.f};
        const float ds = -tz * dot_a_nv / (g.sdot * g.sdot);
        dnv[0] += ds * tx; dnv[1] += ds * ty; dnv[2] += ds * tz;
        dt[0] += ds * g.nv[0]; dt[1] += ds * g.nv[1]; dt[2] += ds * g.nv[2] + dtz;
#pragma unroll
        for (int k = 0; k < 3; ++k)
            dn[k] += dnv[0] * WR(F, 0, k) + dnv[1] * WR(F, 1, k) + dnv[2] * WR(F, 2, k);
    }
#pragma unroll
    for (int k = 0; k < 3; ++k) {
        const float on = (g.kmin == k) ? g.sign : 0.0f;
        dR[0 + k] += on * dn[0]; dR[3 + k] += on * dn[1]; dR[6 + k] += on * dn[2];
    }

    if (d_shs && na > 0) {
        float b[15], bx[15], by[15], bz[15];
#pragma unroll
        for (int k = 0; k < 15; ++k) { b[k] = 0.f; bx[k] = 0.f; by[k] = 0.f; bz[k] = 0.f; }
        sh_basis(C.sh_degree, g.dir[0], g.dir[1], g.dir[2], b);
        sh_basis_grad(C.sh_degree, g.dir[0], g.dir[1], g.dir[2], bx, by, bz);
        float* sp = s_sh + threadIdx.x * row;
        const float v0 = A[R_VD], v1 = A[R_VD + 1], v2 = A[R_VD + 2];
        float ddx = 0.f, ddy = 0.f, ddz = 0.f;
#pragma unroll
        for (int k = 0; k < 15; ++k) {
            if (k < na) {
                const float w = sp[3 * k + 0] * v0 + sp[3 * k + 1] * v1 + sp[3 * k + 2] * v2;
                ddx += bx[k] * w; ddy += by[k] * w; ddz += bz[k] * w;
                sp[3 * k + 0] = b[k] * v0; sp[3 * k + 1] = b[k] * v1; sp[3 * k + 2] = b[k] * v2;
            }
        }
        for (int k = 3 * na; k < row; ++k) sp[k] = 0.f;
        const float dd = g.dir[0] * ddx + g.dir[1] * ddy + g.dir[2] * ddz;
        dm[0] += (ddx - g.dir[0] * dd) / g.dlen;
        dm[1] += (ddy - g.dir[1] * dd) / g.dlen;
        dm[2] += (ddz - g.dir[2] * dd) / g.dlen;
    }

#pragma unroll
    for (int k = 0; k < 3; ++k) dm[k] += dt[0] * F.V[k * 4 + 0] + dt[1] * F.V[k * 4 + 1] + dt[2] * F.V[k * 4 + 2];
    OUT(TEXGS_ACC_MEANS3D, d_means[3 * i + 0], dm[0]); OUT(TEXGS_ACC_MEANS3D, d_means[3 * i + 1], dm[1]); OUT(TEXGS_ACC_MEANS3D, d_means[3 * i + 2], dm[2]);
    if constexpr (COV) {
        OUT(TEXGS_ACC_COV3D, d_cov6[6 * i + 0], dS[0]); OUT(TEXGS_ACC_COV3D, d_cov6[6 * i + 1], dS[1] + dS[3]);
        OUT(TEXGS_ACC_COV3D, d_cov6[6 * i + 2], dS[2] + dS[6]); OUT(TEXGS_ACC_COV3D, d_cov6[6 * i + 3], dS[4]);
        OUT(TEXGS_ACC_COV3D, d_cov6[6 * i + 4], dS[5] + dS[7]); OUT(TEXGS_ACC_COV3D, d_cov6[6 * i + 5], dS[8]);
    }
    if constexpr (!COV) { OUT(TEXGS_ACC_SCALES, d_scales[3 * i + 0], dscale[0]); OUT(TEXGS_ACC_SCALES, d_scales[3 * i + 1], dscale[1]); OUT(TEXGS_ACC_SCALES, d_scales[3 * i + 2], dscale[2]); }

    if constexpr (!COV) {
    const float r = g.q[0], x = g.q[1], y = g.q[2], z = g.q[3];
    OUT(TEXGS_ACC_ROTATIONS, d_rots[4 * i + 0], 2.0f * (-z * dR[1] + y * dR[2] + z * dR[3] - x * dR[5] - y * dR[6] + x * dR[7]));
    OUT(TEXGS_ACC_ROTATIONS, d_rots[4 * i + 1], 2.0f * (y * dR[1] + z * dR[2] + y * dR[3] - 2.0f * x * dR[4] - r * dR[5] + z * dR[6] + r * dR[7] - 2.0f * x * dR[8]));
    OUT(TEXGS_ACC_ROTATIONS, d_rots[4 * i + 2], 2.0f * (-2.0f * y * dR[0] + x * dR[1] + r * dR[2] + x * dR[3] + z * dR[5] - r * dR[6] + z * dR[7] - 2.0f * y * dR[8]));
    OUT(TEXGS_ACC_ROTATIONS, d_rots[4 * i + 3], 2.0f * (-2.0f * z * dR[0] - r * dR[1] + x * dR[2] + r * dR[3] - 2.0f * z * dR[4] + y * dR[5] + x * dR[6] + y * dR[7]));
    }
#undef OUT
    }
    if (d_shs) {
        if (na == 0 || (live && !visible)) {
            if (live) for (int k = 0; k < row; ++k) s_sh[threadIdx.x * row + k] = 0.f;
        }
        __syncthreads();
        if (accumulate & TEXGS_ACC_SHS) sh_rows_out<K8_BLOCK, true>(d_shs + first, s_sh, count, vec);
        else sh_rows_out<K8_BLOCK, false>(d_shs + first, s_sh, count, vec);
    }
}

__global__ void __launch_bounds__(TG_BLOCK)
k_mark_visible(int N, const float* __restrict__ vm, const float* __restrict__ means, uint8_t* __restrict__ visible) {
    const int i = blockIdx.x * TG_BLOCK + threadIdx.x;
    if (i >= N) return;
    const float tz = vm[2] * means[3 * i] + vm[6] * means[3 * i + 1] + vm[10] * means[3 * i + 2] + vm[14];
    visible[i] = tz > TG_NEAR_Z ? 1 : 0;
}

}

hipError_t launch_preprocess_fwd(const CamConst& c, const TexGSFrame* f, const TexGSInputs* in, TexGSGeom* g, hipStream_t s) {
    if (c.N <= 0) return hipSuccess;
    const int blocks = (c.N + TG_BLOCK - 1) / TG_BLOCK;
    const size_t lds = (in->shs && c.sh_degree > 0) ? (size_t)TG_BLOCK * 3 * c.sh_coeffs * sizeof(float) : 0;
    int hdr_words = 0;
    uint32_t* hdr = bin_header_ptr(g, c.N, &hdr_words);
#define K1_LAUNCH(COV) hipLaunchKernelGGL(k_preprocess_fwd<COV>, dim3(blocks), dim3(TG_BLOCK), lds, s, c, f->viewmatrix, f->projmatrix, f->campos, \
                       in->means3D, in->shs, in->opacities, in->scales, in->rotations, in->uvs, in->gradient_uvs, in->color_offset, \
                       in->cov3D_precomp, reinterpret_cast<float4*>(g->rec_test), reinterpret_cast<float4*>(g->rec_shade), g->depth, g->radii, \
                       reinterpret_cast<uint2*>(g->rect), g->tiles_touched, bin_block_sums_ptr(g, c.N), hdr, hdr_words)
    if (in->cov3D_precomp) K1_LAUNCH(true); else K1_LAUNCH(false);
#undef K1_LAUNCH
    return hipGetLastError();
}

hipError_t launch_preprocess_bwd(const CamConst& c, const TexGSFrame* f, const TexGSInputs* in, const TexGSGeom* g,
                           TexGSGrads* gr, hipStream_t s) {
    if (c.N <= 0) return hipSuccess;
    const int blocks = (c.N + K8_BLOCK - 1) / K8_BLOCK;
    const size_t lds = gr->dL_dshs ? (size_t)K8_BLOCK * 3 * c.sh_coeffs * sizeof(float) : 0;
#define K8_LAUNCH(COV) hipLaunchKernelGGL(k_preprocess_bwd<COV>, dim3(blocks), dim3(K8_BLOCK), lds, s, c, f->viewmatrix, f->projmatrix, f->campos, \
                       in->means3D, in->shs, in->opacities, in->scales, in->rotations, in->gradient_uvs, in->cov3D_precomp, \
                       g->radii, gr->acc, gr->dL_dmeans3D, gr->dL_dmeans2D, gr->dL_dshs, gr->dL_dopacities, gr->dL_dscales, \
                       gr->dL_drotations, gr->dL_duvs, gr->dL_dcolor_offset, gr->dL_dcov3D, gr->accumulate)
    if (in->cov3D_precomp) K8_LAUNCH(true); else K8_LAUNCH(false);
#undef K8_LAUNCH
    return hipGetLastError();
}

hipError_t launch_mark_visible(const TexGSFrame* f, const float* means3D, uint8_t* visible, hipStream_t s) {
    if (f->num_gaussians <= 0) return hipSuccess;
    const int blocks = (f->num_gaussians + TG_BLOCK - 1) / TG_BLOCK;
    hipLaunchKernelGGL(k_mark_visible, dim3(blocks), dim3(TG_BLOCK), 0, s, f->num_gaussians, f->viewmatrix, means3D, visible);
    return hipGetLastError();
}
```

### texture-gs_amd/texgs/_lib.py

```python
import contextlib
import ctypes as C
import os

_HERE = os.path.dirname(os.path.abspath(__file__))
LIB_PATH = os.environ.get("TEXGS_LIB") or os.path.join(os.path.dirname(_HERE), "libtexgs.so")

ABI_VERSION = 19
TILE = 16
REC_TEST_FLOATS = 8
REC_SHADE_FLOATS = 20
TEXBIN_RECORD_FLOATS = 4
RESV_WORDS = 192
ACC_FLOATS = 32
WANT_TEXTURE, WANT_GAUSSIANS, WANT_ALL = 1, 2, 3

_fp = C.c_void_p


class Frame(C.Structure):
    _fields_ = [("image_height", C.c_int32), ("image_width", C.c_int32), ("tanfovx", C.c_float),
                ("tanfovy", C.c_float), ("scale_modifier", C.c_float), ("sh_degree", C.c_int32),
                ("sh_coeffs", C.c_int32), ("tex_res", C.c_int32), ("num_gaussians", C.c_int32),
                ("debug", C.c_int32), ("bg", _fp), ("viewmatrix", _fp), ("projmatrix", _fp), ("campos", _fp)]


class Inputs(C.Structure):
    _fields_ = [("means3D", _fp), ("shs", _fp), ("opacities", _fp), ("scales", _fp), ("rotations", _fp),
                ("uvs", _fp), ("gradient_uvs", _fp), ("texture", _fp), ("color_offset", _fp), ("cov3D_precomp", _fp)]


class Geom(C.Structure):
    _fields_ = [("rec_test", _fp), ("rec_shade", _fp), ("depth", _fp), ("radii", _fp), ("rect", _fp), ("tiles_touched", _fp),
                ("offsets", _fp), ("scan_temp", _fp), ("scan_temp_bytes", C.c_size_t)]


class Binning(C.Structure):
    _fields_ = [("num_rendered", C.c_uint32), ("keys_unsorted", _fp), ("keys_sorted", _fp), ("point_list", _fp),
                ("ranges", _fp), ("tile_order", _fp), ("sort_temp", _fp), ("sort_temp_bytes", C.c_size_t)]


class Image(C.Structure):
    _fields_ = [("out_color", _fp), ("out_depth", _fp), ("out_norm", _fp), ("out_alpha", _fp),
                ("final_T", _fp), ("n_contrib", _fp), ("tex_bin_count", _fp),
                ("survivors", _fp), ("surv_qmask", _fp), ("surv_count", _fp), ("tex_bin_resv", _fp)]


class Grads(C.Structure):
    _fields_ = [("dL_dcolor", _fp), ("dL_ddepth", _fp), ("dL_dnorm", _fp), ("dL_dalpha", _fp), ("acc", _fp),
                ("dL_dmeans3D", _fp), ("dL_dmeans2D", _fp), ("dL_dshs", _fp), ("dL_dopacities", _fp),
                ("dL_dscales", _fp), ("dL_drotations", _fp), ("dL_duvs", _fp), ("dL_dtexture", _fp),
                ("dL_dcolor_offset", _fp), ("dL_dcov3D", _fp), ("want", C.c_uint32), ("tex_bins", _fp), ("tex_bin_cursor", _fp), ("tex_bin_base", _fp),
                ("tex_rec_cap", C.c_uint32),
                ("accumulate", C.c_int32)]


class UVNetStruct(C.Structure):
    _fields_ = [(n, _fp) for n in ("W1", "b1", "W2", "b2", "emb", "W3", "b3", "W4", "b4", "W5", "b5", "xyz_offset", "xyz_scale")] \
        + [("hidden", C.c_int32)]


class HashGridStruct(C.Structure):
    _fields_ = [("n_levels", C.c_int32), ("n_features", C.c_int32), ("log2_hashmap_size", C.c_int32), ("base_resolution", C.c_float),
                ("per_level_scale", C.c_float)]


HASHGRID_MAX_LEVELS = 16
HASHGRID_FEATURES = 4


class UVNetGradStruct(C.Structure):
    _fields_ = [(n, _fp) for n in ("dW1", "db1", "dW2", "db2", "dW3", "db3", "dW4", "db4", "dW5", "db5")]


DENSITY_KEEP, DENSITY_CLONE, DENSITY_CLONE_KEPT, DENSITY_SPLIT, DENSITY_CHILD = 1, 2, 4, 8, 16
DENSITY_ROW = {"copy": 0, "moment": 1, "scaling": 2, "xyz": 3}
DENSITY_MAX_ROWS = 24
METRICS_ROW = 16


class DensityPlanStruct(C.Structure):
    _fields_ = [("accum", _fp), ("denom", _fp), ("scaling", _fp), ("opacity", _fp), ("n", C.c_int32), ("max_grad", C.c_float),
                ("min_opacity", C.c_float), ("dense_scale", C.c_float), ("big_scale", C.c_float), ("densify", C.c_int32),
                ("use_big", C.c_int32)]


class DensityRowStruct(C.Structure):
    _fields_ = [("src", _fp), ("dst", _fp), ("width", C.c_int32), ("kind", C.c_int32)]


class DensityMoveStruct(C.Structure):
    _fields_ = [("row", DensityRowStruct * DENSITY_MAX_ROWS), ("rows", C.c_int32), ("n", C.c_int32), ("action", _fp), ("rank", _fp),
                ("n_kept", C.c_int32), ("n_clone", C.c_int32), ("n_split", C.c_int32), ("n_child", C.c_int32), ("scaling", _fp),
                ("rotation", _fp), ("noise", _fp)]


UV_PRECISION = {"fp32": 0, "bf16x3": 1, "mixed": 2}


_P = C.POINTER
_i32, _u32, _f32, _size, _vp = C.c_int32, C.c_uint32, C.c_float, C.c_size_t, C.c_void_p
_frame5 = [_P(Frame), _P(Inputs), _P(Geom), _P(Binning), _P(Image)]
SIGNATURES = {
    "texgs_abi_version": (C.c_int, []),
    "texgs_build_id": (C.c_char_p, []),
    "texgs_last_error": (C.c_char_p, []),
    "texgs_scan_temp_bytes": (_size, [_i32]),
    "texgs_sort_temp_bytes": (_size, [_u32, _u32]),
    "texgs_tex_bin_count": (_size, [_i32]),
    "texgs_preprocess_forward": (C.c_int, [_P(Frame), _P(Inputs), _P(Geom), _vp]),
    "texgs_num_rendered_words": (_size, [_i32]),
    "texgs_num_rendered_begin": (C.c_int, [_P(Geom), _i32, _vp, _size, _i32, _vp]),
    "texgs_num_rendered_reduce": (C.c_int, [_vp, _i32, _P(_u32), _P(C.c_uint64)]),
    "texgs_depth_sort_scan": (C.c_int, [_P(Geom), _i32, _vp]),
    "texgs_bin_sort_render_forward": (C.c_int, _frame5 + [_vp]),
    "texgs_render_forward": (C.c_int, _frame5 + [_vp]),
    "texgs_backward": (C.c_int, _frame5 + [_P(Grads), _vp]),
    "texgs_backward_render": (C.c_int, _frame5 + [_P(Grads), _vp]),
    "texgs_backward_preprocess": (C.c_int, [_P(Frame), _P(Inputs), _P(Geom), _P(Grads), _vp]),
    "texgs_profile_enable": (C.c_int, [C.c_int]),
    "texgs_profile_select": (C.c_int, [_u32]),
    "texgs_profile_read": (C.c_int, [_P(_f32), _P(_u32)]),
    "texgs_rgb_alpha_loss": (C.c_int, [_vp] * 4 + [_i32, _i32, _f32, _f32] + [_vp] * 5),
    "texgs_geom_losses": (C.c_int, [_vp] * 6 + [_i32, _i32, _f32, _f32, _f32, _f32] + [_vp] * 4),
    "texgs_norm_from_depth": (C.c_int, [_vp, _vp, _f32, _f32, _i32, _i32, _f32, _vp, _vp, _vp]),
    "texgs_uv_packed_bytes": (_size, [_i32]),
    "texgs_uv_pack": (C.c_int, [_P(UVNetStruct), _i32, _vp, _vp]),
    "texgs_uv_taylor_packed": (C.c_int, [_P(UVNetStruct), _i32, _vp, _vp, _i32, _vp, _vp, _vp]),
    "texgs_uv_backward_temp_bytes": (_size, [_i32]),
    "texgs_uv_backward": (C.c_int, [_P(UVNetStruct), _i32, _vp, _vp, _i32, _P(UVNetGradStruct), _vp, _vp]),
    "texgs_hashgrid_levels": (C.c_int, [_P(HashGridStruct), _vp, _vp, _vp, _vp, _P(_u32)]),
    "texgs_hashgrid_forward": (C.c_int, [_P(HashGridStruct), _vp, _vp, _i32, _vp, _vp]),
    "texgs_hashgrid_backward_temp_bytes": (_size, [_P(HashGridStruct), _i32]),
    "texgs_hashgrid_backward": (C.c_int, [_P(HashGridStruct), _vp, _vp, _vp, _i32, _vp, _vp, _vp, _vp]),
    "texgs_chamfer_nn_temp_bytes": (_size, [_i32]),
    "texgs_chamfer_nn": (C.c_int, [_vp, _i32, _vp, _i32, _vp, _vp, _vp, _vp]),
    "texgs_knn3_temp_bytes": (_size, [_i32]),
    "texgs_knn3_mean_dist2": (C.c_int, [_vp, _i32, _vp, _vp, _vp]),
    "texgs_fps_temp_bytes": (_size, [_i32, _i32]),
    "texgs_farthest_points": (C.c_int, [_vp, _i32, _i32, _i32, _vp, _vp, _vp]),
    "texgs_cube_sample": (C.c_int, [_vp, _i32, _i32, _vp, _i32, _i32, _i32, _vp, _vp]),
    "texgs_cube_latlong": (C.c_int, [_vp, _i32, _i32, _i32, _i32, _i32, _vp, _vp]),
    "texgs_cube_sample_backward": (C.c_int, [_vp, _i32, _i32, _vp, _i32, _vp, _vp, _vp, _vp]),
    "texgs_cube_sample_nearest_backward": (C.c_int, [_i32, _i32, _vp, _i32, _vp, _vp, _vp]),
    "texgs_density_stats": (C.c_int, [_vp, _vp, _i32, _vp, _vp, _vp, _vp]),
    "texgs_density_plan_temp_bytes": (_size, [_i32]),
    "texgs_density_plan": (C.c_int, [_P(DensityPlanStruct), _vp, _vp, _vp, _vp, _vp]),
    "texgs_density_move": (C.c_int, [_P(DensityMoveStruct), _vp]),
    "texgs_eval_metrics_temp_bytes": (_size, [_i32, _i32]),
    "texgs_eval_metrics": (C.c_int, [_vp] * 5 + [_i32, _i32, _i32, _vp, _vp, _vp]),
    "texgs_selftest_waveops": (C.c_int, [_vp, _vp, _vp]),
    "texgs_mark_visible": (C.c_int, [_P(Frame), _vp, _vp, _vp]),
}
EXPORTS = list(SIGNATURES)
KERNEL_NAMES = ["preprocess_fwd", "scan", "duplicate", "sort", "ranges", "render_fwd", "render_bwd", "preprocess_bwd",
                "texgrad_reduce"]

_lib = None


def load():
    global _lib
    if _lib is not None:
        return _lib
    if not os.path.exists(LIB_PATH):
        raise RuntimeError(
            f"libtexgs.so not found at {LIB_PATH}: build it with `python texture-gs_amd/build.py` "
            "(hipcc --offload-arch=gfx950). There is no CPU fallback for the rasterizer.")
    lib = C.CDLL(LIB_PATH)
    missing = [n for n in EXPORTS if not hasattr(lib, n)]
    if missing:
        raise RuntimeError(f"libtexgs.so at {LIB_PATH} does not export {', '.join(missing)}; rebuild it with "
                           "`python texture-gs_amd/build.py`")
    for name, (restype, argtypes) in SIGNATURES.items():
        fn = getattr(lib, name)
        fn.restype, fn.argtypes = restype, argtypes
    v = lib.texgs_abi_version()
    if v != ABI_VERSION:
        raise RuntimeError(f"libtexgs.so ABI version {v} != expected {ABI_VERSION}; rebuild it")
    global BUILD_ID
    BUILD_ID = lib.texgs_build_id().decode()
    if not os.environ.get("TEXGS_LIB"):
        want = tree_build_id()
        if want is not None and BUILD_ID != want:
            raise RuntimeError(f"libtexgs.so was built from other sources (build id {BUILD_ID}, this tree is {want}); "
                               "rebuild it with `python texture-gs_amd/build.py`")
    _lib = lib
    return lib


BUILD_ID = None


def tree_build_id():
    import importlib.util
    path = os.path.join(os.path.dirname(_HERE), "build.py")
    if not os.path.exists(path):
        return None
    spec = importlib.util.spec_from_file_location("texgs_build_script", path)
    mod = importlib.util.module_from_spec(spec)
    spec.loader.exec_module(mod)
    return mod.build_id()


def check(rc, what):
    if rc != 0:
        msg = load().texgs_last_error().decode("utf-8", "replace")
        raise RuntimeError(f"{what} failed (code {rc}): {msg}")


def call(fn, *args):
    rc = fn(*args)
    if rc != 0:
        check(rc, fn.__name__)


def ptr(t):
    return None if t is None else t.data_ptr()


@contextlib.contextmanager
def on(device):
    import torch
    with torch.cuda.device(device):
        yield torch.cuda.current_stream(device).cuda_stream


def profile_enable(on: bool, only=None):
    mask = 0xFFFFFFFF if only is None else sum(1 << KERNEL_NAMES.index(n) for n in only)
    call(load().texgs_profile_select, mask)
    call(load().texgs_profile_enable, 1 if on else 0)


def profile_read():
    n = len(KERNEL_NAMES)
    ms = (C.c_float * n)()
    cnt = (C.c_uint32 * n)()
    call(load().texgs_profile_read, ms, cnt)
    return {KERNEL_NAMES[i]: (float(ms[i]), int(cnt[i])) for i in range(n)}
```

### texture-gs_amd/texgs/multiview.py

```python
from typing import List, Sequence

import torch


def shard_views(num_views: int, rank: int, world: int) -> List[int]:
    if not (0 <= rank < world):
        raise ValueError(f"rank {rank} outside world {world}")
    views = list(range(rank, num_views, world))
    if not views:
        raise ValueError(f"rank {rank} gets no view: {num_views} views over {world} ranks")
    return views


def lpt_shard_views(costs: Sequence[float], rank: int, world: int) -> List[int]:
    if not (0 <= rank < world):
        raise ValueError(f"rank {rank} outside world {world}")
    n = len(costs)
    if n < world:
        raise ValueError(f"{n} views over {world} ranks")
    order = sorted(range(n), key=lambda v: (-float(costs[v]), v))
    quota = [n // world + (1 if r < n % world else 0) for r in range(world)]
    load = [0.0] * world
    mine = [[] for _ in range(world)]
    for v in order:
        r = min((r for r in range(world) if len(mine[r]) < quota[r]), key=lambda r: (load[r], r))
        mine[r].append(v)
        load[r] += float(costs[v])
    return sorted(mine[rank])


class GradBucket:

    def __init__(self, params: Sequence[torch.Tensor]):
        self.params = [p for p in params if p is not None and p.requires_grad]
        if not self.params:
            raise ValueError("no parameter requires grad")
        dev = self.params[0].device
        total = sum(p.numel() for p in self.params)
        self.flat = torch.zeros(total, dtype=torch.float32, device=dev)
        off = 0
        self.slices = []
        for p in self.params:
            if p.dtype != torch.float32 or p.device != dev:
                raise ValueError("GradBucket needs float32 parameters on one device")
            n = p.numel()
            p.grad = self.flat[off:off + n].view_as(p)
            self.slices.append((off, n))
            off += n
        self.replicas = []
        self.active = 0
        self.before_accumulate = None

    def select(self, k: int):
        while len(self.replicas) < k:
            self.replicas.append(torch.zeros_like(self.flat))
        self.active = k

    def fold(self):
        self.active = 0
        for r in self.replicas:
            self.flat.add_(r)
            r.zero_()

    def sink_for(self, tensor):
        for p, (off, n) in zip(self.params, self.slices):
            if p is tensor:
                sl = self.flat[off:off + n]
                if p.grad is None:
                    sl.zero_()
                    p.grad = sl.view_as(p)
                elif p.grad.data_ptr() != self.flat.data_ptr() + 4 * off or not p.grad.is_contiguous():
                    return None
                return sl if self.active == 0 else self.replicas[self.active - 1][off:off + n]
        return None

    def zero(self):
        self.flat.zero_()
        for p, (off, n) in zip(self.params, self.slices):
            if p.grad is None or p.grad.data_ptr() != self.flat.data_ptr() + 4 * off:
                p.grad = self.flat[off:off + n].view_as(p)

    def segment_of(self, tensors) -> tuple:
        idx = sorted(i for i, p in enumerate(self.params) if any(p is t for t in tensors))
        if not idx or idx != list(range(idx[0], idx[-1] + 1)):
            raise ValueError("the tensors of a segment must be registered parameters that are adjacent in the bucket")
        off = self.slices[idx[0]][0]
        return off, self.slices[idx[-1]][0] + self.slices[idx[-1]][1] - off

    def all_reduce_async(self, dist, segment=None, after=(), timing=False, wire_dtype=None):
        off, n = segment if segment is not None else (0, self.flat.numel())
        buf = self.flat[off:off + n]
        if dist.get_backend() != "nccl" or not self.flat.is_cuda:
            for ev in after:
                ev.synchronize()
            self._reduce_now(dist, buf, wire_dtype)
            return self
        cur = torch.cuda.current_stream(self.flat.device)
        if getattr(self, "_comm", None) is None:
            self._comm = torch.cuda.Stream(self.flat.device)
            self._comm_events = []
        self._comm.wait_stream(cur)
        for ev in after:
            self._comm.wait_event(ev)
        with torch.cuda.stream(self._comm):
            e0 = e1 = None
            if timing:
                e0, e1 = torch.cuda.Event(enable_timing=True), torch.cuda.Event(enable_timing=True)
                e0.record(self._comm)
            if wire_dtype is None or wire_dtype == torch.float32:
                dist.all_reduce(buf, op=dist.ReduceOp.SUM)
                wire_bytes = n * 4
            else:
                stage = buf.to(wire_dtype)
                dist.all_reduce(stage, op=dist.ReduceOp.SUM)
                buf.copy_(stage)
                wire_bytes = n * stage.element_size()
            if timing:
                e1.record(self._comm)
                self._comm_events.append((wire_bytes, e0, e1))
        self._pending = True
        return self

    def wait(self):
        if getattr(self, "_pending", False):
            torch.cuda.current_stream(self.flat.device).wait_stream(self._comm)
            self._pending = False
        return self.flat

    def comm_timings(self):
        out = []
        for nbytes, e0, e1 in getattr(self, "_comm_events", []):
            e1.synchronize()
            out.append((nbytes, e0.elapsed_time(e1)))
        if getattr(self, "_comm_events", None):
            self._comm_events.clear()
        return out

    def _reduce_now(self, dist, buf, wire_dtype=None):
        wd = torch.float32 if wire_dtype is None else wire_dtype
        if buf.is_cuda:
            host = torch.empty(buf.shape, dtype=wd).pin_memory()
            host.copy_(buf, non_blocking=True)
            torch.cuda.current_stream(buf.device).synchronize()
            dist.all_reduce(host, op=dist.ReduceOp.SUM)
            buf.copy_(host, non_blocking=True)
        elif wd != torch.float32:
            stage = buf.to(wd)
            dist.all_reduce(stage, op=dist.ReduceOp.SUM)
            buf.copy_(stage)
        else:
            dist.all_reduce(buf, op=dist.ReduceOp.SUM)

    def all_reduce(self, dist, average_over: int = 0):
        if dist.get_backend() == "nccl":
            dist.all_reduce(self.flat, op=dist.ReduceOp.SUM)
        else:
            if self.flat.is_cuda:
                if getattr(self, "_host", None) is None:
                    self._host = torch.empty(self.flat.shape, dtype=torch.float32).pin_memory()
                self._host.copy_(self.flat, non_blocking=True)
                torch.cuda.current_stream(self.flat.device).synchronize()
                dist.all_reduce(self._host, op=dist.ReduceOp.SUM)
                self.flat.copy_(self._host, non_blocking=True)
            else:
                dist.all_reduce(self.flat, op=dist.ReduceOp.SUM)
        if average_over:
            self.flat.div_(float(average_over))
        return self.flat


class ViewPipeline:

    def __init__(self, device, depth: int = 2):
        if depth < 1:
            raise ValueError("depth must be >= 1")
        self.device = torch.device(device)
        self.streams = [torch.cuda.Stream(self.device) for _ in range(depth)] if depth > 1 else []

    def close(self):
        from . import rasterizer
        for s in self.streams:
            s.synchronize()
            rasterizer.release_scratch(self.device, s.cuda_stream)
        self.streams = []

    def __del__(self):
        try:
            self.close()
        except Exception:
            pass

    def run(self, views, forward_fn, backward_fn=None, sink=None, order="accumulate", texture_ready=None, prefetch_fn=None,
            prefetch_ahead=1):
        results = []
        views = list(views)
        if not self.streams:
            for i, v in enumerate(views):
                obj = forward_fn(v)
                if prefetch_fn is not None and i + 1 < len(views):
                    prefetch_fn(views[i + 1])
                if backward_fn is not None:
                    if texture_ready is not None and sink is not None and i == len(views) - 1:
                        sink.before_accumulate = lambda: texture_ready([])
                    try:
                        backward_fn(obj)
                    finally:
                        if sink is not None:
                            sink.before_accumulate = None
                results.append(obj)
            return results
        if order not in ("backward", "accumulate", "none"):
            raise ValueError(order)
        if sink is None and order != "backward":
            order = "backward"
        cur = torch.cuda.current_stream(self.device)
        for s in self.streams:
            s.wait_stream(cur)
        prev_bwd = None
        render_done = {}
        depth = len(self.streams)
        try:
            ahead = depth * max(1, int(prefetch_ahead))
            if prefetch_fn is not None:
                for i, v in enumerate(views[:ahead]):
                    with torch.cuda.stream(self.streams[i % depth]):
                        prefetch_fn(v)
            for i, v in enumerate(views):
                k = i % depth
                s = self.streams[k]
                with torch.cuda.stream(s):
                    if order == "none":
                        sink.select(k)
                    obj = forward_fn(v)
                    if prefetch_fn is not None and i + ahead < len(views):
                        prefetch_fn(views[i + ahead])
                    if backward_fn is not None:
                        if order == "backward" and prev_bwd is not None:
                            s.wait_event(prev_bwd)
                        if order == "accumulate":
                            last = i == len(views) - 1

                            def hook(ev=prev_bwd, s=s, k=k, last=last):
                                if texture_ready is not None:
                                    e = torch.cuda.Event()
                                    e.record(s)
                                    render_done[k] = e
                                    if last:
                                        texture_ready([render_done[j] for j in sorted(render_done)])
                                if ev is not None:
                                    s.wait_event(ev)
                            sink.before_accumulate = hook
                        backward_fn(obj)
                        prev_bwd = torch.cuda.Event()
                        prev_bwd.record(s)
                results.append(obj)
        finally:
            if sink is not None:
                sink.before_accumulate = None
            for s in self.streams:
                cur.wait_stream(s)
            if sink is not None and order == "none":
                sink.fold()
        return results
```

### texture-gs_amd/texgs/rasterizer.py

```python
import ctypes as C
import math
import os as _os
import threading as _threading
from collections import namedtuple
from types import SimpleNamespace
from typing import NamedTuple

import torch
from torch import nn

from . import _lib

USE_TEX_BINS = _os.environ.get("TEXGS_TEX_BINS", "1") != "0"
TEX_REC_CAP = int(_os.environ.get("TEXGS_REC_CAP", "0"))
DIRECT_LEAF_GRADS = _os.environ.get("TEXGS_DIRECT_LEAF_GRADS", "0") != "0"
TEX_REC_BYTES_MAX = int(float(_os.environ.get("TEXGS_BIN_GB_MAX", "4")) * (1 << 30))
_ACC_BITS = dict(means3D=1, means2D=2, shs=4, opacities=8, scales=16, rotations=32, uvs=64, color_offset=128, cov3D=256)


class GaussianRasterizationSettings(NamedTuple):
    image_height: int
    image_width: int
    tanfovx: float
    tanfovy: float
    bg: torch.Tensor
    scale_modifier: float
    viewmatrix: torch.Tensor
    projmatrix: torch.Tensor
    sh_degree: int
    campos: torch.Tensor
    prefiltered: bool
    debug: bool


_ptr = _lib.ptr


def _f32c(t: torch.Tensor, name: str, device) -> torch.Tensor:
    if not isinstance(t, torch.Tensor):
        raise TypeError(f"{name} must be a torch.Tensor")
    if t.device != device:
        raise ValueError(f"{name} is on {t.device}, expected {device}")
    if t.dtype != torch.float32:
        raise TypeError(f"{name} must be float32, got {t.dtype}")
    return t.contiguous()


class _Arena:

    def __init__(self, device):
        self.device, self.specs, self.size, self.buf = device, {}, 0, None

    def add(self, name, shape, dtype):
        off = (self.size + 255) & ~255
        self.specs[name] = (off, tuple(shape), dtype)
        self.size = off + math.prod(shape) * dtype.itemsize

    def commit(self):
        self.buf = torch.empty(max(self.size, 1), dtype=torch.uint8, device=self.device)

    def ptr(self, name):
        return self.buf.data_ptr() + self.specs[name][0] if name in self.specs else None

    def view(self, name):
        off, shape, dtype = self.specs[name]
        return self.buf[off:off + math.prod(shape) * dtype.itemsize].view(dtype).view(shape)


class _Tensors(dict):

    def __init__(self, arenas, **real):
        super().__init__(**real)
        self._arenas = arenas

    def __missing__(self, name):
        for ar in self._arenas:
            if name in ar.specs:
                self[name] = v = ar.view(name)
                return v
        self[name] = None
        return None

    def get(self, name, default=None):
        v = self[name]
        return default if v is None else v


GEOM_CACHE = _os.environ.get("TEXGS_GEOM_CACHE", "1") != "0"
_CAPACITY_HINT = {}
_GEOM = {}
_GeomEntry = namedtuple("_GeomEntry", "ints cam_key fingerprint D cap bin arenas handoff counts")
_GEOM_STATS = {"hits": 0, "misses": 0, "late_handoffs": 0}
_SERIAL = [0]
_LAST_DIFFERENTIATED = {}
_DROPPED = {}
_PRED_LOCK = _threading.RLock()


def unused_streak(dev_index):
    with _PRED_LOCK:
        last = _LAST_DIFFERENTIATED.get(dev_index, -1)
        return sum(1 for n in _DROPPED.get(dev_index, ()) if n > last)


def reset_handoff_predictor():
    with _PRED_LOCK:
        _LAST_DIFFERENTIATED.clear()
        _DROPPED.clear()


def geometry_cache_stats():
    return dict(_GEOM_STATS)


_SCRATCH = {}


def release_scratch(device=None, stream=None):
    for cache in (_SCRATCH, _GEOM, _PREFETCH):
        for key in list(cache):
            if (device is None or key[0] == torch.device(device).index) and (stream is None or key[1] == int(stream)):
                for _, fwd in (cache[key] if cache is _PREFETCH else ()):
                    fwd.abandon()
                del cache[key]


def scratch_bytes():
    total = 0
    for sc in _SCRATCH.values():
        if sc.acc is not None:
            total += sc.acc.numel() * 4
        if sc.bins is not None:
            total += sc.bins.nbytes()
    for e in _GEOM.values():
        total += sum(ar.buf.numel() for ar in e.arenas if ar is not None and ar.buf is not None)
    return total


class _TexBins:

    def __init__(self, lib, device, R):
        self.device, self.R = device, R
        self.nbins = int(lib.texgs_tex_bin_count(R))
        self.cursor = torch.zeros(self.nbins + 2, dtype=torch.int32, device=device)
        self.base = torch.empty(2 * self.nbins + 1, dtype=torch.int32, device=device)
        self.cap = 0
        self.rec = None
        self.host_stat = torch.zeros(1, dtype=torch.int32).pin_memory()
        self.event = None
        self.calls = 0

    def nbytes(self):
        return ((0 if self.rec is None else self.rec.numel()) + self.cursor.numel() + self.base.numel()) * 4

    def _resize(self, cap):
        cap = max(1024, min(int(cap), TEX_REC_BYTES_MAX // (4 * _lib.TEXBIN_RECORD_FLOATS)))
        if cap != self.cap:
            self.rec = None
            self.rec = torch.empty(cap * _lib.TEXBIN_RECORD_FLOATS, dtype=torch.float32, device=self.device)
            self.cap = cap

    def before_call(self, D, counts=None):
        if TEX_REC_CAP:
            self._resize(TEX_REC_CAP)
            return
        if self.rec is None and counts is not None and not torch.cuda.is_current_stream_capturing():
            self._resize(int(counts.sum().item() * 1.25) + 4096)
        if self.event is not None and self.event.query():
            self.event = None
            wanted = int(self.host_stat[0])
            if wanted > self.cap:
                self._resize(int(wanted * 1.25) + 4096)
        if self.rec is None:
            self._resize(24 * max(int(D), 1024))

    def after_call(self):
        self.calls += 1
        if self.event is None and not TEX_REC_CAP and (self.calls <= 4 or self.calls % 16 == 0):
            self.host_stat.copy_(self.cursor[self.nbins:self.nbins + 1], non_blocking=True)
            self.event = torch.cuda.Event()
            self.event.record(torch.cuda.current_stream(self.device))


class _State:
    __slots__ = ("frame", "inputs", "geom", "bin", "img", "tensors", "args", "N", "K", "R", "H", "W", "D", "cap", "tiles",
                 "want_counts", "lazy", "backward_ran", "shared_geometry", "serial", "__weakref__")

    def __init__(self, frame, inputs, geom, bin, img, tensors, args, D, cap, tiles, want_counts, lazy, shared_geometry):
        self.frame, self.inputs, self.geom, self.bin, self.img, self.tensors, self.args = frame, inputs, geom, bin, img, tensors, args
        self.N, self.K, self.R, self.H, self.W = args.N, args.K, args.R, frame.image_height, frame.image_width
        self.D, self.cap, self.tiles = D, cap, tiles
        self.want_counts, self.lazy, self.backward_ran, self.shared_geometry = want_counts, lazy, False, shared_geometry
        with _PRED_LOCK:
            _SERIAL[0] += 1
            self.serial = _SERIAL[0]

    def __del__(self):
        try:
            if getattr(self, "lazy", False) and not self.backward_ran:
                dev = self.args.means3D.device.index
                with _PRED_LOCK:
                    last = _LAST_DIFFERENTIATED.get(dev, -1)
                    _DROPPED[dev] = [n for n in _DROPPED.get(dev, []) if n > last][-8:] + [self.serial]
        except Exception:
            pass


def _make_frame(st: GaussianRasterizationSettings, N, K, R, device, keep):
    bg = _f32c(st.bg, "bg", device).reshape(-1)
    vm = _f32c(st.viewmatrix, "viewmatrix", device).reshape(-1)
    pm = _f32c(st.projmatrix, "projmatrix", device).reshape(-1)
    cp = _f32c(st.campos, "campos", device).reshape(-1)
    if bg.numel() != 3 or vm.numel() != 16 or pm.numel() != 16 or cp.numel() != 3:
        raise ValueError("bg/campos must have 3 elements and viewmatrix/projmatrix 16")
    keep.extend([bg, vm, pm, cp])
    return _lib.Frame(int(st.image_height), int(st.image_width), float(st.tanfovx), float(st.tanfovy), float(st.scale_modifier),
                      int(st.sh_degree), int(K), int(R), int(N), 1 if st.debug else 0, _ptr(bg), _ptr(vm), _ptr(pm), _ptr(cp))


_PREFETCH = {}
_PIN_POOL = {}


def _pin_take(words):
    pool = _PIN_POOL.setdefault(words, [])
    return pool.pop() if pool else torch.empty(max(words, 1), dtype=torch.int32).pin_memory()


def _pin_give(t):
    pool = _PIN_POOL.setdefault(t.numel(), [])
    if len(pool) < 16:
        pool.append(t)


def _prefetch_take(device, key):
    skey = (device.index, int(torch.cuda.current_stream(device).cuda_stream))
    lst = _PREFETCH.get(skey, ())
    for k, (key_k, fwd) in enumerate(lst):
        if key_k == key:
            del lst[k]
            if not lst:
                del _PREFETCH[skey]
            return fwd


_Args = namedtuple("_Args", "means3D shs opacities scales rotations uvs gradient_uvs texture color_offset cov3D_precomp N K R")
_HANDOFF = tuple(n for n, _ in _lib.Image._fields_[6:])


def _check_inputs(st, means3D, shs, opacities, scales, rotations, uvs, gradient_uvs, texture, color_offset=None, cov3D_precomp=None):
    device = means3D.device
    N = means3D.shape[0]
    means3D = _f32c(means3D, "means3D", device)
    if means3D.dim() != 2 or means3D.shape[1] != 3:
        raise ValueError("means3D must be [N,3]")
    opacities = _f32c(opacities, "opacities", device)
    if opacities.numel() != N:
        raise ValueError(f"per-Gaussian inputs must have exactly N rows (N={N}; opacities {tuple(opacities.shape)})")
    if cov3D_precomp is not None:
        if texture is not None:
            raise ValueError("cov3D_precomp is an input of the untextured surface only")
        cov3D_precomp = _f32c(cov3D_precomp, "cov3D_precomp", device)
        if cov3D_precomp.shape != (N, 6):
            raise ValueError(f"cov3D_precomp must be [N,6], got {tuple(cov3D_precomp.shape)}")
        scales = rotations = None
    else:
        scales = _f32c(scales, "scales", device)
        rotations = _f32c(rotations, "rotations", device)
        if scales.shape != (N, 3) or rotations.shape != (N, 4):
            raise ValueError("per-Gaussian inputs must have exactly N rows "
                             f"(N={N}; scales {tuple(scales.shape)}, rotations {tuple(rotations.shape)})")
    if texture is not None:
        uvs = _f32c(uvs, "uvs", device)
        gradient_uvs = _f32c(gradient_uvs, "gradient_uvs", device)
        texture = _f32c(texture, "texture", device)
        if uvs.shape != (N, 3) or gradient_uvs.numel() != 9 * N:
            raise ValueError("per-Gaussian inputs must have exactly N rows "
                             f"(N={N}; uvs {tuple(uvs.shape)}, gradient_uvs {tuple(gradient_uvs.shape)})")
        if texture.dim() != 4 or texture.shape[0] != 6 or texture.shape[1] != texture.shape[2] or texture.shape[3] != 3:
            raise ValueError(f"texture must be [6,R,R,3], got {tuple(texture.shape)}")
        R = texture.shape[1]
    else:
        uvs = gradient_uvs = None
        R = 1
    K = 0
    if shs is not None:
        shs = _f32c(shs, "shs", device)
        if shs.dim() != 3 or shs.shape[0] != N or shs.shape[2] != 3:
            raise ValueError(f"shs must be [N,K,3], got {tuple(shs.shape)}")
        K = shs.shape[1]
        if K > 15:
            raise ValueError("shs holds at most 15 view-dependent coefficients (degree 3)")
    if color_offset is not None:
        color_offset = _f32c(color_offset, "color_offset", device)
        if color_offset.shape != (N, 3):
            raise ValueError(f"color_offset must be [N,3], got {tuple(color_offset.shape)}")
    if int(st.sh_degree) < 0 or int(st.sh_degree) > 3:
        raise ValueError("sh_degree must be in [0,3]")
    return _Args(means3D, shs, opacities, scales, rotations, uvs, gradient_uvs, texture, color_offset, cov3D_precomp, N, K, R)


def _add_handoff(ar, cap, tiles, R, want_counts):
    if cap is not None:
        ar.add("survivors", (4 * max(cap, 1), 2), torch.int32)
        ar.add("surv_qmask", (4 * max(cap, 1),), torch.int16)
    if tiles is not None:
        ar.add("surv_count", (4 * tiles,), torch.int32)
        if want_counts:
            ar.add("tex_bin_count", (2 * int(_lib.load().texgs_tex_bin_count(R)),), torch.int32)
            ar.add("tex_bin_resv", (4 * tiles, _lib.RESV_WORDS), torch.int32)


class _Forward:

    def __init__(self, st, tensors, for_backward, count_bins, lazy):
        self.st, self.raw, self.flags = st, tensors, (for_backward, count_bins, lazy)

    def key(self):
        t = lambda x: None if x is None else (x.data_ptr(), x._version, tuple(x.shape), x.requires_grad)
        st = self.st
        return (int(st.image_height), int(st.image_width), float(st.tanfovx), float(st.tanfovy), float(st.scale_modifier), int(st.sh_degree),
                bool(st.debug), t(st.bg), t(st.viewmatrix), t(st.projmatrix), t(st.campos)) + tuple(t(x) for x in self.raw) + self.flags

    def begin(self):
        lib, st = _lib.load(), self.st
        a = self.args = _check_inputs(st, *self.raw)
        for_backward, count_bins, lazy = self.flags
        device, N = a.means3D.device, a.N
        if count_bins is None:
            count_bins = for_backward
        self.handoff = bool(for_backward) and not (lazy and unused_streak(device.index) >= 2)
        self.want_counts = bool(count_bins and for_backward and a.texture is not None and USE_TEX_BINS)
        H, W = int(st.image_height), int(st.image_width)
        self.tiles = ((W + _lib.TILE - 1) // _lib.TILE) * ((H + _lib.TILE - 1) // _lib.TILE)
        cur_stream = torch.cuda.current_stream(device)
        stream = self.stream = cur_stream.cuda_stream
        self.keep = list(a[:10])
        with torch.cuda.device(device):
            self.frame = _make_frame(st, N, a.K, a.R, device, self.keep)
            self.inputs = _lib.Inputs(*map(_ptr, a[:10]))
            i32, f32, u8, n1 = torch.int32, torch.float32, torch.uint8, max(N, 1)
            self.gints = (N, H, W, a.R if a.texture is not None else 0, float(st.tanfovx), float(st.tanfovy), float(st.scale_modifier),
                          a.cov3D_precomp is not None)
            self.cam_key = tuple((t.data_ptr(), t._version) for t in (st.viewmatrix, st.projmatrix, st.campos))
            gkey = self.gkey = (device.index, int(stream))
            entry = _GEOM.get(gkey) if GEOM_CACHE else None
            if entry is not None and not (entry.ints == self.gints and entry.cam_key == self.cam_key):
                del _GEOM[gkey]
                entry = None
            self.entry = entry
            scan_bytes = lib.texgs_scan_temp_bytes(N)
            fix = self.fix = _Arena(device)
            fix.add("rec", (n1, _lib.REC_TEST_FLOATS), f32)
            fix.add("rec_shade", (n1, _lib.REC_SHADE_FLOATS), f32)
            fix.add("depth", (n1,), f32)
            fix.add("rect", (n1, 2), i32)
            fix.add("tiles_touched", (n1,), i32)
            fix.add("offsets", (n1,), i32)
            fix.add("scan_temp", (scan_bytes,), u8)
            fix.add("final_T", (H, W), f32)
            fix.add("n_contrib", (H, W), i32)
            if entry is None:
                self._add_lists(fix)
            fix.commit()
            radii = torch.empty(N, dtype=i32, device=device)
            self.geom = _lib.Geom(fix.ptr("rec"), fix.ptr("rec_shade"), fix.ptr("depth"), _ptr(radii), fix.ptr("rect"),
                                  fix.ptr("tiles_touched"), fix.ptr("offsets"), fix.ptr("scan_temp"), scan_bytes)
            self.outs = (torch.empty(3, H, W, dtype=f32, device=device), torch.empty(1, H, W, dtype=f32, device=device),
                         torch.empty(3, H, W, dtype=f32, device=device), torch.empty(1, H, W, dtype=f32, device=device), radii)
            self.img = _lib.Image(*map(_ptr, self.outs[:4]), fix.ptr("final_T"), fix.ptr("n_contrib"), None, None, None, None, None)
            self.hint_key = (device.index, N, H, W)
            self.cap = _CAPACITY_HINT.get(self.hint_key, max(4 * N, 1024))
            self.binning = self.bin_ar = None
            if entry is None:
                self._alloc_bin(self.cap, fix)
            refs = self.refs = [C.byref(x) for x in (self.frame, self.inputs, self.geom)]
            _lib.call(lib.texgs_preprocess_forward, *refs, stream)
            pin = self.pin = _pin_take(int(lib.texgs_num_rendered_words(N)))
            _lib.call(lib.texgs_num_rendered_begin, refs[2], N, pin.data_ptr(), pin.numel(), 0, stream)
            self.d_ev = torch.cuda.Event()
            self.d_ev.record(cur_stream)
            if entry is None:
                _lib.call(lib.texgs_depth_sort_scan, refs[2], N, stream)
        return self

    def _add_lists(self, ar):
        ar.add("ranges", (self.tiles, 2), torch.int32)
        ar.add("tile_order", (self.tiles,), torch.int32)
        if self.handoff:
            _add_handoff(ar, None, self.tiles, self.args.R, self.want_counts)

    def _alloc_bin(self, cap, lists_ar):
        c1, tiles = max(cap, 1), self.tiles
        sort_bytes = _lib.load().texgs_sort_temp_bytes(cap, tiles)
        ar = self.bin_ar = _Arena(self.fix.device)
        ar.add("keys_unsorted", (c1,), torch.int64)
        ar.add("keys_sorted", (c1,), torch.int64)
        ar.add("point_list", (c1,), torch.int32)
        ar.add("sort_temp", (sort_bytes,), torch.uint8)
        if lists_ar is None:
            self._add_lists(ar)
        if self.handoff:
            _add_handoff(ar, cap, None, self.args.R, self.want_counts)
        ar.commit()
        la = lists_ar if lists_ar is not None else ar
        self.binning = _lib.Binning(0, ar.ptr("keys_unsorted"), ar.ptr("keys_sorted"), ar.ptr("point_list"), la.ptr("ranges"),
                                    la.ptr("tile_order"), ar.ptr("sort_temp"), sort_bytes)
        for n in _HANDOFF:
            setattr(self.img, n, (ar if n in ar.specs else la).ptr(n))

    def finish(self):
        lib, a, img, entry, refs = _lib.load(), self.args, self.img, self.entry, self.refs
        for_backward, _, lazy = self.flags
        stream, cap, pin = self.stream, self.cap, self.pin
        with torch.cuda.device(a.means3D.device):
            self.d_ev.synchronize()
            d_host, fp_host = C.c_uint32(0), C.c_uint64(0)
            _lib.call(lib.texgs_num_rendered_reduce, pin.data_ptr(), a.N, C.byref(d_host), C.byref(fp_host))
            _pin_give(pin)
            D, fp = int(d_host.value), int(fp_host.value)
            shared = entry is not None and fp == entry.fingerprint and D == entry.D
            if shared:
                _GEOM_STATS["hits"] += 1
                binning, cap = _lib.Binning(D, *entry.bin), entry.cap
                _lib.call(lib.texgs_render_forward, *refs, C.byref(binning), C.byref(img), stream)
                if for_backward and entry.handoff and (entry.counts or not self.want_counts):
                    img.survivors, img.surv_qmask, img.surv_count = entry.handoff
                    img.tex_bin_count, img.tex_bin_resv = entry.counts if self.want_counts else (None, None)
            else:
                _GEOM_STATS["misses"] += 1
                grown = int(D * 1.25) + 1024
                if entry is not None:
                    cap = max(cap, grown)
                    self._alloc_bin(cap, None)
                    _lib.call(lib.texgs_depth_sort_scan, refs[2], a.N, stream)
                elif D > cap:
                    cap = grown
                    self._alloc_bin(cap, self.fix)
                binning = self.binning
                binning.num_rendered = D
                _lib.call(lib.texgs_bin_sort_render_forward, *refs, C.byref(binning), C.byref(img), stream)
                _CAPACITY_HINT[self.hint_key] = max(_CAPACITY_HINT.get(self.hint_key, 0), grown)
                if GEOM_CACHE:
                    _GEOM[self.gkey] = _GeomEntry(
                        self.gints, self.cam_key, fp, D, cap, tuple(getattr(binning, n) for n, _ in _lib.Binning._fields_[1:]),
                        (self.fix, self.bin_ar), (img.survivors, img.surv_qmask, img.surv_count) if self.handoff else None,
                        (img.tex_bin_count, img.tex_bin_resv) if (self.handoff and img.tex_bin_count) else None)
        arenas = (self.fix,) + ((self.bin_ar,) if self.bin_ar is not None else ()) + (tuple(entry.arenas) if shared else ())
        tensors = _Tensors(arenas, keep=self.keep, radii=self.outs[4], for_backward=bool(for_backward))
        for n in _HANDOFF:
            if getattr(img, n) is None:
                tensors[n] = None
        return self.outs, _State(self.frame, self.inputs, self.geom, binning, img, tensors, a, D, cap, self.tiles, self.want_counts,
                                 bool(lazy and for_backward), shared)

    def abandon(self):
        self.d_ev.synchronize()
        _pin_give(self.pin)


def _gpu_only(device):
    _lib.load()
    if device.type != "cuda":
        raise RuntimeError("the textured rasterizer runs on an AMD GPU (torch device 'cuda' = HIP); "
                           f"got tensors on {device}. There is no CPU fallback.")


def prefetch_forward(st, means3D, shs, opacities, scales, rotations, uvs, gradient_uvs, texture, color_offset=None,
                     for_backward=True, cov3D_precomp=None, count_bins=None, lazy=False):
    device = means3D.device
    _gpu_only(device)
    fwd = _Forward(st, (means3D, shs, opacities, scales, rotations, uvs, gradient_uvs, texture, color_offset, cov3D_precomp),
                   for_backward, count_bins, lazy).begin()
    lst = _PREFETCH.setdefault((device.index, int(torch.cuda.current_stream(device).cuda_stream)), [])
    lst.append((fwd.key(), fwd))
    for _, old in lst[:-4]:
        old.abandon()
    del lst[:-4]


def forward_raw(st, means3D, shs, opacities, scales, rotations, uvs, gradient_uvs, texture, color_offset=None,
                for_backward=True, cov3D_precomp=None, count_bins=None, lazy=False):
    _gpu_only(means3D.device)
    fwd = _Forward(st, (means3D, shs, opacities, scales, rotations, uvs, gradient_uvs, texture, color_offset, cov3D_precomp),
                   for_backward, count_bins, lazy)
    pend = _prefetch_take(means3D.device, fwd.key()) if _PREFETCH else None
    return (pend or fwd.begin()).finish()


def _late_handoff(s: _State):
    lib = _lib.load()
    device = s.args.means3D.device
    stream = torch.cuda.current_stream(device).cuda_stream
    ar = _Arena(device)
    _add_handoff(ar, s.cap, s.tiles, s.R, s.want_counts)
    ar.add("scratch_out", (8, s.H, s.W), torch.float32)
    ar.add("final_T", (s.H, s.W), torch.float32)
    ar.add("n_contrib", (s.H, s.W), torch.int32)
    ar.commit()
    so = ar.ptr("scratch_out")
    hw = 4 * s.H * s.W
    img = _lib.Image(so, so + 3 * hw, so + 4 * hw, so + 7 * hw, ar.ptr("final_T"), ar.ptr("n_contrib"), *(ar.ptr(n) for n in _HANDOFF))
    _lib.call(lib.texgs_render_forward, C.byref(s.frame), C.byref(s.inputs), C.byref(s.geom), C.byref(s.bin), C.byref(img), stream)
    s.tensors._arenas = tuple(s.tensors._arenas) + (ar,)
    for n in _HANDOFF:
        setattr(s.img, n, ar.ptr(n))
        s.tensors.pop(n, None)
        if n not in ar.specs:
            s.tensors[n] = None
    _GEOM_STATS["late_handoffs"] += 1


def _plan_outputs(N, K, textured, has_cov, has_coff, want, sinks, device):
    shapes = {}
    if want & _lib.WANT_GAUSSIANS:
        shapes = dict(means3D=(N, 3), means2D=(N, 3), opacities=(N, 1))
        if has_cov:
            shapes["cov3D"] = (N, 6)
        else:
            shapes.update(scales=(N, 3), rotations=(N, 4))
        if textured:
            shapes["uvs"] = (N, 3)
        if K > 0:
            shapes["shs"] = (N, K, 3)
        if has_coff:
            shapes["color_offset"] = (N, 3)
    fresh = [n for n in shapes if n not in sinks]
    sizes = [math.prod(shapes[n]) for n in fresh]
    flat = torch.empty(sum(sizes), dtype=torch.float32, device=device).split(sizes) if fresh else ()
    outs, mask = {n: v.view(shapes[n]) for n, v in zip(fresh, flat)}, 0
    for n in shapes.keys() - set(fresh):
        t = outs[n] = sinks[n]
        assert t.dtype == torch.float32 and t.is_contiguous() and t.numel() == math.prod(shapes[n]), n
        mask |= _ACC_BITS[n]
    return outs, mask, {n: (None if n in sinks else outs[n]) for n in shapes}


def backward_raw(s: _State, dL_dcolor, dL_ddepth, dL_dnorm, dL_dalpha, sinks=None, before_accumulate=None,
                 want=_lib.WANT_ALL):
    lib = _lib.load()
    if not s.tensors["for_backward"]:
        raise RuntimeError("this forward ran with for_backward=False (no survivor lists were kept): its backward cannot run")
    a = s.args
    device = a.means3D.device
    f32 = dict(dtype=torch.float32, device=device)
    N, R = s.N, s.R
    stream = torch.cuda.current_stream(device).cuda_stream
    textured = a.texture is not None
    want &= _lib.WANT_ALL if textured else _lib.WANT_GAUSSIANS
    want_g, want_t = bool(want & _lib.WANT_GAUSSIANS), bool(want & _lib.WANT_TEXTURE)
    if not want:
        return (None,) * 8

    def g(t, shape):
        if t is None:
            return None
        t = t.to(torch.float32).contiguous()
        assert tuple(t.shape) == shape, (tuple(t.shape), shape)
        return t
    dc, dd, dn, da = g(dL_dcolor, (3, s.H, s.W)), g(dL_ddepth, (1, s.H, s.W)), g(dL_dnorm, (3, s.H, s.W)), g(dL_dalpha, (1, s.H, s.W))
    with torch.cuda.device(device):
        if s.img.survivors is None:
            _late_handoff(s)
        s.backward_ran = True
        if s.lazy:
            with _PRED_LOCK:
                _LAST_DIFFERENTIATED[device.index] = max(_LAST_DIFFERENTIATED.get(device.index, -1), s.serial)
        skey = (device.index, int(stream))
        sc = _SCRATCH.pop(skey, None) or SimpleNamespace(acc=None, bins=None)
        if want_g and (sc.acc is None or sc.acc.shape[0] < max(N, 1)):
            sc.acc = torch.zeros(max(N, 1), _lib.ACC_FLOATS, **f32)
        acc = sc.acc if want_g else None
        sinks = sinks or {}
        outs, mask, res = _plan_outputs(N, s.K, textured, a.cov3D_precomp is not None, a.color_offset is not None, want, sinks, device)
        tex_sink = sinks.get("texture") if want_t else None
        d_tex = (tex_sink if tex_sink is not None else torch.zeros(6, R, R, 3, **f32)) if want_t else None
        bins = None
        if want_t and USE_TEX_BINS and s.tensors.get("tex_bin_count") is not None:
            bins = sc.bins if (sc.bins is not None and sc.bins.R == R) else _TexBins(lib, device, R)
            sc.bins = None
            bins.before_call(s.D, s.tensors.get("tex_bin_count"))
        grads = _lib.Grads(_ptr(dc), _ptr(dd), _ptr(dn), _ptr(da), _ptr(acc), _ptr(outs.get("means3D")), _ptr(outs.get("means2D")),
                           _ptr(outs.get("shs")), _ptr(outs.get("opacities")), _ptr(outs.get("scales")), _ptr(outs.get("rotations")),
                           _ptr(outs.get("uvs")), _ptr(d_tex), _ptr(outs.get("color_offset")), _ptr(outs.get("cov3D")), want,
                           _ptr(bins.rec) if bins else None, _ptr(bins.cursor) if bins else None,
                           _ptr(bins.base) if bins else None, bins.cap if bins else 0, mask)
        refs = [C.byref(x) for x in (s.frame, s.inputs, s.geom, s.bin, s.img, grads)]
        if before_accumulate is None:
            _lib.call(lib.texgs_backward, *refs, stream)
        else:
            _lib.call(lib.texgs_backward_render, *refs, stream)
            before_accumulate()
            _lib.call(lib.texgs_backward_preprocess, *refs[:3], refs[5], stream)
    if bins is not None:
        bins.after_call()
        sc.bins = bins
    _SCRATCH[skey] = sc
    s.tensors["d_color_offset"] = res.get("color_offset")
    s.tensors["d_cov3D"] = res.get("cov3D")
    return tuple(res.get(n) for n in ("means3D", "means2D", "shs", "opacities", "scales", "rotations", "uvs")) \
        + (None if tex_sink is not None else d_tex,)


def _leaf_grad_sink(t):
    if t is None or not (t.is_leaf and t.requires_grad):
        return None
    if getattr(t, "_backward_hooks", None) or getattr(t, "_post_accumulate_grad_hooks", None):
        return None
    gr = t.grad
    if gr is None or gr.dtype != torch.float32 or not gr.is_contiguous() or gr.shape != t.shape or gr.device != t.device:
        return None
    return gr


_ARG = dict(means3D=0, means2D=1, shs=2, opacities=3, scales=4, rotations=5, uvs=6, gradient_uvs=7, texture=8, st=9,
            color_offset=10, grad_sink=11, cov3D_precomp=12)
_GAUSSIAN_ARGS = ("means3D", "means2D", "shs", "opacities", "scales", "rotations", "uvs", "color_offset", "cov3D_precomp")


class _RasterizeGaussians(torch.autograd.Function):
    @staticmethod
    def forward(ctx, means3D, means2D, shs, opacities, scales, rotations, uvs, gradient_uvs, texture, st, color_offset=None,
                grad_sink=None, cov3D_precomp=None):
        ctx.grad_sink = grad_sink
        ctx.set_materialize_grads(False)
        ctx.named = dict(means3D=means3D, means2D=means2D, shs=shs, opacities=opacities, scales=scales,
                         rotations=rotations, uvs=uvs, texture=texture, color_offset=color_offset, cov3D=cov3D_precomp)
        nig = tuple(ctx.needs_input_grad) + (False,) * len(_ARG)
        want = (_lib.WANT_TEXTURE if (texture is not None and nig[_ARG["texture"]]) else 0) \
            | (_lib.WANT_GAUSSIANS if any(nig[_ARG[n]] for n in _GAUSSIAN_ARGS) else 0)
        ctx.want = want
        ctx.nargs = len(ctx.needs_input_grad)
        outs, state = forward_raw(st, means3D, shs, opacities, scales, rotations, uvs, gradient_uvs, texture, color_offset,
                                  for_backward=bool(want), cov3D_precomp=cov3D_precomp,
                                  count_bins=bool(want & _lib.WANT_TEXTURE), lazy=True)
        color, depth, norm, alpha, radii = outs
        ctx.state = state
        ctx.versions = [(t, t._version) for t in state.tensors["keep"] if t is not None]
        ctx.op_shape = opacities.shape
        ctx.mark_non_differentiable(radii)
        return color, depth, norm, alpha, radii

    @staticmethod
    def backward(ctx, dL_dcolor, dL_ddepth, dL_dnorm, dL_dalpha, _dradii):
        s = ctx.state
        if s is None:
            raise RuntimeError("the rasterizer's backward ran a second time: its per-call state was released after the "
                               "first backward (retain_graph=True is not supported); run the forward again")
        for t, v in ctx.versions:
            if t._version != v:
                raise RuntimeError("an input of the rasterizer was modified in place between its forward and backward "
                                   "(the backward re-reads inputs through saved pointers); clone it before modifying")
        sinks, bucket = {}, False
        if ctx.grad_sink is not None:
            sinks = {k: g for k, g in ((k, ctx.grad_sink.sink_for(v)) for k, v in ctx.named.items() if v is not None)
                     if g is not None}
            bucket = bool(sinks)
        if not bucket and DIRECT_LEAF_GRADS:
            sinks = {k: g for k, g in ((k, _leaf_grad_sink(v)) for k, v in ctx.named.items()) if g is not None}
        d_means3D, d_means2D, d_shs, d_op, d_scales, d_rot, d_uvs, d_tex = backward_raw(
            s, dL_dcolor, dL_ddepth, dL_dnorm, dL_dalpha, sinks=sinks or None,
            before_accumulate=getattr(ctx.grad_sink, "before_accumulate", None) if bucket else None, want=ctx.want)
        d_coff = s.tensors.get("d_color_offset")
        d_cov = s.tensors.get("d_cov3D")
        ctx.state = None
        ctx.versions = None
        ctx.named = None
        if d_op is not None:
            d_op = d_op.reshape(ctx.op_shape)
        return (d_means3D, d_means2D, d_shs, d_op, d_scales, d_rot, d_uvs, None, d_tex, None, d_coff, None, d_cov)[:ctx.nargs]


EXTRA_ATTRS_MAX = 32


def blend_extra_attrs(st, means3D, means2D, opacities, scales, rotations, extra_attrs, grad_sink=None, cov3D_precomp=None):
    N = means3D.shape[0]
    if not isinstance(extra_attrs, torch.Tensor) or extra_attrs.dim() != 2 or extra_attrs.shape[0] != N:
        raise ValueError(f"extra_attrs must be a [N, C] tensor with N = {N} rows")
    C_ = int(extra_attrs.shape[1])
    if C_ > EXTRA_ATTRS_MAX:
        raise ValueError(f"extra_attrs has {C_} channels; at most {EXTRA_ATTRS_MAX} are blended")
    H, W = int(st.image_height), int(st.image_width)
    ea = extra_attrs.to(torch.float32)
    if C_ == 0 or N == 0:
        return torch.zeros(C_, H, W, dtype=torch.float32, device=means3D.device) + 0.0 * ea.sum()
    m = ea.detach().amin() - 1.0
    st0 = st._replace(bg=torch.zeros_like(st.bg), sh_degree=0)
    if means2D is None:
        means2D = torch.zeros_like(means3D)
    outs = []
    for c0 in range(0, C_, 3):
        grp = ea[:, c0:c0 + 3]
        if grp.shape[1] < 3:
            grp = torch.cat([grp, (m + 1.0).expand(N, 3 - grp.shape[1])], dim=1)
        color, _, _, alpha, _ = _RasterizeGaussians.apply(means3D, means2D, None, opacities, scales, rotations, None, None, None, st0,
                                                          ((grp - m) - 0.5).contiguous(), grad_sink, cov3D_precomp)
        outs.append(color + m * alpha)
    return torch.cat(outs, dim=0)[:C_]


class GaussianRasterizer(nn.Module):

    def __init__(self, raster_settings: GaussianRasterizationSettings, grad_sink=None):
        super().__init__()
        self.raster_settings = raster_settings
        self.grad_sink = grad_sink

    def markVisible(self, positions):
        lib = _lib.load()
        st = self.raster_settings
        positions = _f32c(positions, "positions", positions.device)
        N = positions.shape[0]
        keep = []
        frame = _make_frame(st, N, 0, 1, positions.device, keep)
        vis = torch.zeros(N, dtype=torch.uint8, device=positions.device)
        stream = torch.cuda.current_stream(positions.device).cuda_stream
        with torch.cuda.device(positions.device):
            _lib.call(lib.texgs_mark_visible, C.byref(frame), positions.data_ptr(), vis.data_ptr(), stream)
        return vis.bool()

    def prefetch(self, means3D, means2D, opacities, shs=None, scales=None, rotations=None, uvs=None,
                 gradient_uvs=None, texture=None, extra_attrs=None):
        grad = torch.is_grad_enabled()
        rg = lambda t: bool(grad and t is not None and t.requires_grad)
        want_tex = rg(texture)
        want_g = any(rg(t) for t in (means3D, means2D, shs, opacities, scales, rotations, uvs))
        prefetch_forward(self.raster_settings, means3D, shs, opacities, scales, rotations, uvs, gradient_uvs, texture, None,
                         for_backward=want_tex or want_g, cov3D_precomp=None, count_bins=want_tex, lazy=True)

    def forward(self, means3D, means2D, opacities, shs=None, scales=None, rotations=None, uvs=None,
                gradient_uvs=None, texture=None, extra_attrs=None):
        st = self.raster_settings
        if scales is None or rotations is None:
            raise ValueError("scales and rotations are required (the textured operator has no cov3D_precomp path)")
        if uvs is None or gradient_uvs is None or texture is None:
            raise ValueError("uvs, gradient_uvs and texture are required")
        if means2D is None:
            means2D = torch.zeros_like(means3D)
        color, depth, norm, alpha, radii = _RasterizeGaussians.apply(
            means3D, means2D, shs, opacities, scales, rotations, uvs, gradient_uvs, texture, st, None, self.grad_sink)
        extra = None
        if extra_attrs is not None:
            extra = blend_extra_attrs(st, means3D, means2D, opacities, scales, rotations, extra_attrs, self.grad_sink)
        return color, depth, norm, alpha, radii, extra
```

Before: 1019 views/s.

## Defer SH gradient scatter into a batched multi-view flush kernel

The per-view preprocess backward no longer reads and writes the full 48-float SH gradient row for every Gaussian. It instead writes a 3-float view-direction residue per Gaussian, and a new sh_flush kernel later folds up to 16 views' residues into dL_dshs and dL_dmeans3D in one pass. This cuts the SH gradient read-modify-write traffic from once per view to once per batch of views. In exchange it adds residue buffers, Python bookkeeping in the grad bucket and pipeline, a recompute of the SH basis per view inside the flush, and flush assertions guarding all-reduce and zero.

```diff
diff --git a/include/texgs.h b/include/texgs.h
--- a/include/texgs.h
+++ b/include/texgs.h
@@ -119,6 +119,7 @@
     uint32_t* tex_bin_base;
     uint32_t  tex_rec_cap;
     int32_t accumulate;
+    float* dL_dvd_residue;
 } TexGSGrads;
 
 int         texgs_abi_version(void);
diff --git a/include/texgs_multiview.h b/include/texgs_multiview.h
--- /dev/null
+++ b/include/texgs_multiview.h
@@ -0,0 +1,27 @@
+#ifndef TEXGS_MULTIVIEW_H
+#define TEXGS_MULTIVIEW_H
+
+#include <stddef.h>
+#include <stdint.h>
+
+#ifdef __cplusplus
+extern "C" {
+#endif
+
+#define TEXGS_SH_FLUSH_MAX_VIEWS 16
+
+typedef struct TexGSShFlushView {
+    const float* campos;
+    const float* residue;
+    int32_t sh_degree;
+    int32_t sh_coeffs;
+} TexGSShFlushView;
+
+int texgs_sh_flush(int32_t N, int32_t K, const float* means3D, const float* shs, float* dL_dshs, float* dL_dmeans3D,
+                   const TexGSShFlushView* views, int32_t count, void* stream);
+
+#ifdef __cplusplus
+}
+#endif
+
+#endif
diff --git a/texture-gs_amd/build.py b/texture-gs_amd/build.py
--- a/texture-gs_amd/build.py
+++ b/texture-gs_amd/build.py
@@ -28,14 +28,15 @@
     "abi.hip": [],
 }
 HEADERS = [os.path.join(CSRC, "common.h"), os.path.join(CSRC, "wave_ops.h"), os.path.join(CSRC, "render_bwd_body.h"),
-           os.path.join(ROOT, "include", "texgs.h"), os.path.join(ROOT, "include", "texgs_optim.h")]
+           os.path.join(ROOT, "include", "texgs.h"), os.path.join(ROOT, "include", "texgs_optim.h"),
+           os.path.join(ROOT, "include", "texgs_multiview.h")]
 
 
 def build_id():
     import hashlib
     h = hashlib.sha256()
     files = sorted(os.path.join(CSRC, f) for f in os.listdir(CSRC) if f.endswith((".hip", ".h"))) \
-        + [os.path.join(ROOT, "include", "texgs.h"), os.path.join(ROOT, "include", "texgs_optim.h")]
+        + [os.path.join(ROOT, "include", f) for f in ("texgs.h", "texgs_optim.h", "texgs_multiview.h")]
     for f in files:
         h.update(os.path.basename(f).encode())
         h.update(open(f, "rb").read())
diff --git a/texture-gs_amd/csrc/abi.hip b/texture-gs_amd/csrc/abi.hip
--- a/texture-gs_amd/csrc/abi.hip
+++ b/texture-gs_amd/csrc/abi.hip
@@ -216,6 +216,8 @@
     if (!(grads->want & TEXGS_WANT_GAUSSIANS)) return 0;
     if (!grads->acc) return fail_msg("acc must be allocated");
     if (in->cov3D_precomp && !grads->dL_dcov3D) return fail_msg("dL_dcov3D is required with cov3D_precomp");
+    if (grads->dL_dvd_residue && (grads->accumulate & (TEXGS_ACC_SHS | TEXGS_ACC_MEANS3D)) != (TEXGS_ACC_SHS | TEXGS_ACC_MEANS3D))
+        return fail_msg("dL_dvd_residue needs TEXGS_ACC_SHS and TEXGS_ACC_MEANS3D in accumulate: texgs_sh_flush adds into both");
     hipStream_t s = (hipStream_t)stream;
     const CamConst c = make_cam(frame);
     hipError_t st;
@@ -543,6 +545,29 @@
     return 0;
 }
 
+int texgs_sh_flush(int32_t N, int32_t K, const float* means3D, const float* shs, float* dL_dshs, float* dL_dmeans3D,
+                   const TexGSShFlushView* views, int32_t count, void* stream) {
+    if (count < 0) return fail_msg("count < 0");
+    if (count > TEXGS_SH_FLUSH_MAX_VIEWS) return fail_msg("count exceeds TEXGS_SH_FLUSH_MAX_VIEWS: flush in several calls");
+    if (N < 0) return fail_msg("N < 0");
+    if (count == 0 || N == 0) return 0;
+    if (!dL_dshs || !dL_dmeans3D) return fail_msg("NULL sink (dL_dshs or dL_dmeans3D) with views pending");
+    if (!means3D || !shs || !views) return fail_msg("NULL argument (means3D, shs or views) with views pending");
+    if (K < 1 || K > 16) return fail_msg("K must be in [1,16]");
+    for (int32_t k = 0; k < count; ++k) {
+        const TexGSShFlushView& v = views[k];
+        if (!v.campos || !v.residue) return fail_msg("NULL campos or residue in a view record");
+        if (v.sh_degree < 0 || v.sh_degree > 3) return fail_msg("sh_degree of a view record must be in [0,3]");
+        if (v.sh_coeffs != K) {
+            snprintf(g_err, sizeof(g_err), "K does not match: view %d wrote its residue with K = %d, the flush has K = %d", (int)k,
+                     (int)v.sh_coeffs, (int)K);
+            return -1;
+        }
+    }
+    hipStream_t s = (hipStream_t)stream;
+    return launched("sh_flush", launch_sh_flush(N, K, means3D, shs, dL_dshs, dL_dmeans3D, views, count, s), s, false);
+}
+
 int texgs_selftest_waveops(const float* seed128, float* out576, void* stream) {
     if (!seed128 || !out576) return fail_msg("NULL argument");
     return launched("selftest_waveops", launch_selftest_waveops(seed128, out576, (hipStream_t)stream), (hipStream_t)stream, false);
diff --git a/texture-gs_amd/csrc/common.h b/texture-gs_amd/csrc/common.h
--- a/texture-gs_amd/csrc/common.h
+++ b/texture-gs_amd/csrc/common.h
@@ -3,6 +3,7 @@
 #include <stdint.h>
 #include "texgs.h"
 #include "texgs_optim.h"
+#include "texgs_multiview.h"
 
 #define TG_NEAR_Z        0.2f
 #define TG_LOWPASS       0.3f
@@ -53,6 +54,8 @@
 hipError_t launch_preprocess_fwd(const CamConst& c, const TexGSFrame* f, const TexGSInputs* in, TexGSGeom* g, hipStream_t s);
 hipError_t launch_preprocess_bwd(const CamConst& c, const TexGSFrame* f, const TexGSInputs* in, const TexGSGeom* g,
                            TexGSGrads* gr, hipStream_t s);
+hipError_t launch_sh_flush(int N, int K, const float* means3D, const float* shs, float* dL_dshs, float* dL_dmeans3D,
+                           const TexGSShFlushView* views, int count, hipStream_t s);
 hipError_t launch_mark_visible(const TexGSFrame* f, const float* means3D, uint8_t* visible, hipStream_t s);
 hipError_t launch_depth_sort_scan(const TexGSGeom* g, int N, hipStream_t s);
 uint32_t* bin_block_sums_ptr(const TexGSGeom* g, int N);
diff --git a/texture-gs_amd/csrc/preprocess.hip b/texture-gs_amd/csrc/preprocess.hip
--- a/texture-gs_amd/csrc/preprocess.hip
+++ b/texture-gs_amd/csrc/preprocess.hip
@@ -65,6 +65,13 @@
     n[2] = (k == 0) ? v20 : ((k == 1) ? v21 : v22);
 }
 
+__device__ __forceinline__ float view_direction(const float* m, const float* cam, float* raw, float* dir) {
+    raw[0] = m[0] - cam[0]; raw[1] = m[1] - cam[1]; raw[2] = m[2] - cam[2];
+    const float dlen = sqrtf(raw[0] * raw[0] + raw[1] * raw[1] + raw[2] * raw[2]);
+    dir[0] = raw[0] / dlen; dir[1] = raw[1] / dlen; dir[2] = raw[2] / dlen;
+    return dlen;
+}
+
 template <bool COV = false>
 __device__ __forceinline__ void geo_forward(Geo& g, const Frame& F, const CamConst& C, int i,
                                             const float* __restrict__ means, const float* __restrict__ scales,
@@ -150,7 +157,8 @@
     const float lam = mid + sqrtf(fmaxf(0.1f, mid * mid - g.det));
     g.radius = (int)ceilf(3.0f * sqrtf(lam));
 
-    g.dir[0] = mx - F.cam[0]; g.dir[1] = my - F.cam[1]; g.dir[2] = mz - F.cam[2];
+    float raw[3];
+    g.dlen = view_direction(g.m, F.cam, raw, g.dir);
     float n0, n1, n2;
     if constexpr (COV) {
         float ev[3];
@@ -165,10 +173,8 @@
         n1 = (g.kmin == 0) ? g.R[3] : ((g.kmin == 1) ? g.R[4] : g.R[5]);
         n2 = (g.kmin == 0) ? g.R[6] : ((g.kmin == 1) ? g.R[7] : g.R[8]);
     }
-    g.sign = ((n0 * g.dir[0] + n1 * g.dir[1] + n2 * g.dir[2]) > 0.0f) ? -1.0f : 1.0f;
+    g.sign = ((n0 * raw[0] + n1 * raw[1] + n2 * raw[2]) > 0.0f) ? -1.0f : 1.0f;
     g.n[0] = g.sign * n0; g.n[1] = g.sign * n1; g.n[2] = g.sign * n2;
-    g.dlen = sqrtf(g.dir[0] * g.dir[0] + g.dir[1] * g.dir[1] + g.dir[2] * g.dir[2]);
-    g.dir[0] /= g.dlen; g.dir[1] /= g.dlen; g.dir[2] /= g.dlen;
 
 #pragma unroll
     for (int k = 0; k < 3; ++k)
@@ -414,8 +420,11 @@
 #ifndef K8_BLOCK
 #define K8_BLOCK 256
 #endif
-template <bool COV>
-__global__ void __launch_bounds__(K8_BLOCK)
+#ifndef K8_DEFER_BLOCK
+#define K8_DEFER_BLOCK 256
+#endif
+template <bool COV, bool DEFER, int BLOCK>
+__global__ void __launch_bounds__(BLOCK)
 k_preprocess_bwd(CamConst C, const float* __restrict__ vm, const float* __restrict__ pm, const float* __restrict__ cp,
                  const float* __restrict__ means, const float* __restrict__ shs, const float* __restrict__ opac,
                  const float* __restrict__ scales,
@@ -423,18 +432,20 @@
                  const int32_t* __restrict__ radii, float* __restrict__ acc,
                  float* __restrict__ d_means, float* __restrict__ d_means2D, float* __restrict__ d_shs,
                  float* __restrict__ d_op, float* __restrict__ d_scales, float* __restrict__ d_rots,
-                 float* __restrict__ d_uvs, float* __restrict__ d_coff, float* __restrict__ d_cov6, int accumulate) {
+                 float* __restrict__ d_uvs, float* __restrict__ d_coff, float* __restrict__ d_cov6, float* __restrict__ d_vd_res,
+                 int accumulate) {
     extern __shared__ __attribute__((aligned(16))) float s_sh[];
-    const int i = blockIdx.x * K8_BLOCK + threadIdx.x;
+    const int i = blockIdx.x * BLOCK + threadIdx.x;
     const int K = C.sh_coeffs;
     const bool live = i < C.N;
     const int row = 3 * K;
     const int na = (shs != nullptr && C.sh_degree > 0) ? sh_active(C.sh_degree, K) : 0;
-    const size_t first = (size_t)blockIdx.x * K8_BLOCK * row;
-    const int count = d_shs ? (int)min((size_t)K8_BLOCK * row, (size_t)C.N * row - first) : 0;
+    const size_t first = (size_t)blockIdx.x * BLOCK * row;
+    const int count = d_shs ? (int)min((size_t)BLOCK * row, (size_t)C.N * row - first) : 0;
     const bool vec = d_shs && (((size_t)d_shs) & 15) == 0;
-    if (na > 0 && d_shs) {
-        for (int k = threadIdx.x; k < count; k += K8_BLOCK) s_sh[k] = shs[first + k];
+    if constexpr (DEFER) { (void)first; (void)count; (void)vec; }
+    if (!DEFER && na > 0 && d_shs) {
+        for (int k = threadIdx.x; k < count; k += BLOCK) s_sh[k] = shs[first + k];
         __syncthreads();
     }
     const bool visible = live && radii[i] > 0;
@@ -450,6 +461,7 @@
         }
         if (d_uvs && !(accumulate & TEXGS_ACC_UVS)) d_uvs[3 * i] = d_uvs[3 * i + 1] = d_uvs[3 * i + 2] = 0.f;
         if (d_coff && !(accumulate & TEXGS_ACC_COLOR_OFFSET)) d_coff[3 * i] = d_coff[3 * i + 1] = d_coff[3 * i + 2] = 0.f;
+        if constexpr (DEFER) d_vd_res[3 * i] = d_vd_res[3 * i + 1] = d_vd_res[3 * i + 2] = 0.f;
     }
     if (visible) {
 #define OUT(BIT, P, V) do { if (accumulate & (BIT)) (P) += (V); else (P) = (V); } while (0)
@@ -584,7 +596,10 @@
         dR[0 + k] += on * dn[0]; dR[3 + k] += on * dn[1]; dR[6 + k] += on * dn[2];
     }
 
-    if (d_shs && na > 0) {
+    if constexpr (DEFER) {
+        d_vd_res[3 * i + 0] = (na > 0) ? A[R_VD] : 0.f; d_vd_res[3 * i + 1] = (na > 0) ? A[R_VD + 1] : 0.f;
+        d_vd_res[3 * i + 2] = (na > 0) ? A[R_VD + 2] : 0.f;
+    } else if (d_shs && na > 0) {
         float b[15], bx[15], by[15], bz[15];
 #pragma unroll
         for (int k = 0; k < 15; ++k) { b[k] = 0.f; bx[k] = 0.f; by[k] = 0.f; bz[k] = 0.f; }
@@ -627,14 +642,82 @@
     }
 #undef OUT
     }
-    if (d_shs) {
+    if constexpr (!DEFER) if (d_shs) {
         if (na == 0 || (live && !visible)) {
             if (live) for (int k = 0; k < row; ++k) s_sh[threadIdx.x * row + k] = 0.f;
         }
         __syncthreads();
-        if (accumulate & TEXGS_ACC_SHS) sh_rows_out<K8_BLOCK, true>(d_shs + first, s_sh, count, vec);
-        else sh_rows_out<K8_BLOCK, false>(d_shs + first, s_sh, count, vec);
-    }
+        if (accumulate & TEXGS_ACC_SHS) sh_rows_out<BLOCK, true>(d_shs + first, s_sh, count, vec);
+        else sh_rows_out<BLOCK, false>(d_shs + first, s_sh, count, vec);
+    }
+}
+
+constexpr int FL_BLOCK = 256;
+constexpr int FL_MAX = TEXGS_SH_FLUSH_MAX_VIEWS;
+
+struct ShFlushArgs {
+    TexGSShFlushView v[FL_MAX];
+    int32_t count;
+};
+
+__global__ void __launch_bounds__(FL_BLOCK)
+k_sh_flush(ShFlushArgs a, int N, int K, const float* __restrict__ means, const float* __restrict__ shs,
+           float* __restrict__ d_shs, float* __restrict__ d_means) {
+    extern __shared__ __attribute__((aligned(16))) float s_row[];
+    const int i = blockIdx.x * FL_BLOCK + threadIdx.x;
+    const bool live = i < N;
+    const int row = 3 * K;
+    const size_t first = (size_t)blockIdx.x * FL_BLOCK * row;
+    const int count = (int)min((size_t)FL_BLOCK * row, (size_t)N * row - first);
+    const bool vec = (((size_t)d_shs) & 15) == 0;
+    for (int k = threadIdx.x; k < count; k += FL_BLOCK) s_row[k] = shs[first + k];
+    __syncthreads();
+    float sp[45];
+#pragma unroll
+    for (int k = 0; k < 45; ++k) sp[k] = (live && k < row) ? s_row[threadIdx.x * row + k] : 0.f;
+    __syncthreads();
+    for (int k = threadIdx.x; k < count; k += FL_BLOCK) s_row[k] = d_shs[first + k];
+    __syncthreads();
+    if (live) {
+        const float m[3] = {means[3 * i + 0], means[3 * i + 1], means[3 * i + 2]};
+        float* gp = s_row + threadIdx.x * row;
+        float dm[3] = {d_means[3 * i + 0], d_means[3 * i + 1], d_means[3 * i + 2]};
+        bool any = false;
+        for (int v = 0; v < a.count; ++v) {
+            const float* __restrict__ res = a.v[v].residue;
+            const float v0 = res[3 * i + 0], v1 = res[3 * i + 1], v2 = res[3 * i + 2];
+            const int deg = a.v[v].sh_degree;
+            const int na = deg > 0 ? sh_active(deg, K) : 0;
+            if ((v0 == 0.f && v1 == 0.f && v2 == 0.f) || na == 0) continue;
+            const float* __restrict__ cp = a.v[v].campos;
+            const float cam[3] = {cp[0], cp[1], cp[2]};
+            float raw[3], dir[3];
+            const float dlen = view_direction(m, cam, raw, dir);
+            float b[15], bx[15], by[15], bz[15];
+#pragma unroll
+            for (int k = 0; k < 15; ++k) { b[k] = 0.f; bx[k] = 0.f; by[k] = 0.f; bz[k] = 0.f; }
+            sh_basis(deg, dir[0], dir[1], dir[2], b);
+            sh_basis_grad(deg, dir[0], dir[1], dir[2], bx, by, bz);
+            float ddx = 0.f, ddy = 0.f, ddz = 0.f;
+#pragma unroll
+            for (int k = 0; k < 15; ++k) {
+                if (k < na) {
+                    const float w = sp[3 * k + 0] * v0 + sp[3 * k + 1] * v1 + sp[3 * k + 2] * v2;
+                    ddx += bx[k] * w; ddy += by[k] * w; ddz += bz[k] * w;
+                    gp[3 * k + 0] = gp[3 * k + 0] + b[k] * v0; gp[3 * k + 1] = gp[3 * k + 1] + b[k] * v1;
+                    gp[3 * k + 2] = gp[3 * k + 2] + b[k] * v2;
+                }
+            }
+            const float dd = dir[0] * ddx + dir[1] * ddy + dir[2] * ddz;
+            dm[0] += (ddx - dir[0] * dd) / dlen;
+            dm[1] += (ddy - dir[1] * dd) / dlen;
+            dm[2] += (ddz - dir[2] * dd) / dlen;
+            any = true;
+        }
+        if (any) { d_means[3 * i + 0] = dm[0]; d_means[3 * i + 1] = dm[1]; d_means[3 * i + 2] = dm[2]; }
+    }
+    __syncthreads();
+    sh_rows_out<FL_BLOCK, false>(d_shs + first, s_row, count, vec);
 }
 
 __global__ void __launch_bounds__(TG_BLOCK)
@@ -665,14 +748,30 @@
 hipError_t launch_preprocess_bwd(const CamConst& c, const TexGSFrame* f, const TexGSInputs* in, const TexGSGeom* g,
                            TexGSGrads* gr, hipStream_t s) {
     if (c.N <= 0) return hipSuccess;
-    const int blocks = (c.N + K8_BLOCK - 1) / K8_BLOCK;
-    const size_t lds = gr->dL_dshs ? (size_t)K8_BLOCK * 3 * c.sh_coeffs * sizeof(float) : 0;
-#define K8_LAUNCH(COV) hipLaunchKernelGGL(k_preprocess_bwd<COV>, dim3(blocks), dim3(K8_BLOCK), lds, s, c, f->viewmatrix, f->projmatrix, f->campos, \
+#define K8_LAUNCH(COV, DEFER, BLOCK, LDS) hipLaunchKernelGGL((k_preprocess_bwd<COV, DEFER, BLOCK>), dim3((c.N + BLOCK - 1) / BLOCK), dim3(BLOCK), LDS, s, \
+                       c, f->viewmatrix, f->projmatrix, f->campos, \
                        in->means3D, in->shs, in->opacities, in->scales, in->rotations, in->gradient_uvs, in->cov3D_precomp, \
                        g->radii, gr->acc, gr->dL_dmeans3D, gr->dL_dmeans2D, gr->dL_dshs, gr->dL_dopacities, gr->dL_dscales, \
-                       gr->dL_drotations, gr->dL_duvs, gr->dL_dcolor_offset, gr->dL_dcov3D, gr->accumulate)
-    if (in->cov3D_precomp) K8_LAUNCH(true); else K8_LAUNCH(false);
+                       gr->dL_drotations, gr->dL_duvs, gr->dL_dcolor_offset, gr->dL_dcov3D, gr->dL_dvd_residue, gr->accumulate)
+    if (gr->dL_dvd_residue) {
+        if (in->cov3D_precomp) K8_LAUNCH(true, true, K8_DEFER_BLOCK, 0); else K8_LAUNCH(false, true, K8_DEFER_BLOCK, 0);
+    } else {
+        const size_t lds = gr->dL_dshs ? (size_t)K8_BLOCK * 3 * c.sh_coeffs * sizeof(float) : 0;
+        if (in->cov3D_precomp) K8_LAUNCH(true, false, K8_BLOCK, lds); else K8_LAUNCH(false, false, K8_BLOCK, lds);
+    }
 #undef K8_LAUNCH
+    return hipGetLastError();
+}
+
+hipError_t launch_sh_flush(int N, int K, const float* means3D, const float* shs, float* dL_dshs, float* dL_dmeans3D,
+                           const TexGSShFlushView* views, int count, hipStream_t s) {
+    if (count < 0 || count > FL_MAX) return hipErrorInvalidValue;
+    if (N <= 0 || count == 0) return hipSuccess;
+    ShFlushArgs a;
+    for (int k = 0; k < FL_MAX; ++k) a.v[k] = k < count ? views[k] : TexGSShFlushView{nullptr, nullptr, 0, 0};
+    a.count = count;
+    const size_t lds = (size_t)FL_BLOCK * 3 * K * sizeof(float);
+    hipLaunchKernelGGL(k_sh_flush, dim3((N + FL_BLOCK - 1) / FL_BLOCK), dim3(FL_BLOCK), lds, s, a, N, K, means3D, shs, dL_dshs, dL_dmeans3D);
     return hipGetLastError();
 }
 
diff --git a/texture-gs_amd/texgs/_lib.py b/texture-gs_amd/texgs/_lib.py
--- a/texture-gs_amd/texgs/_lib.py
+++ b/texture-gs_amd/texgs/_lib.py
@@ -51,7 +51,7 @@
                 ("dL_dscales", _fp), ("dL_drotations", _fp), ("dL_duvs", _fp), ("dL_dtexture", _fp),
                 ("dL_dcolor_offset", _fp), ("dL_dcov3D", _fp), ("want", C.c_uint32), ("tex_bins", _fp), ("tex_bin_cursor", _fp), ("tex_bin_base", _fp),
                 ("tex_rec_cap", C.c_uint32),
-                ("accumulate", C.c_int32)]
+                ("accumulate", C.c_int32), ("dL_dvd_residue", _fp)]
 
 
 class UVNetStruct(C.Structure):
diff --git a/texture-gs_amd/texgs/multiview.py b/texture-gs_amd/texgs/multiview.py
--- a/texture-gs_amd/texgs/multiview.py
+++ b/texture-gs_amd/texgs/multiview.py
@@ -1,6 +1,32 @@
+import ctypes as C
 from typing import List, Sequence
 
 import torch
+
+SH_FLUSH_MAX_VIEWS = 16
+
+
+class ShFlushView(C.Structure):
+    _fields_ = [("campos", C.c_void_p), ("residue", C.c_void_p), ("sh_degree", C.c_int32), ("sh_coeffs", C.c_int32)]
+
+
+SH_FLUSH_SIGNATURE = (C.c_int, [C.c_int32, C.c_int32, C.c_void_p, C.c_void_p, C.c_void_p, C.c_void_p, C.POINTER(ShFlushView), C.c_int32,
+                                C.c_void_p])
+_sh_flush_fn = None
+
+
+def sh_flush_entry():
+    global _sh_flush_fn
+    if _sh_flush_fn is None:
+        from . import _lib
+        lib = _lib.load()
+        if not hasattr(lib, "texgs_sh_flush"):
+            raise RuntimeError(f"libtexgs.so at {_lib.LIB_PATH} does not export texgs_sh_flush; rebuild it with "
+                               "`python texture-gs_amd/build.py`")
+        fn = lib.texgs_sh_flush
+        fn.restype, fn.argtypes = SH_FLUSH_SIGNATURE
+        _sh_flush_fn = fn
+    return _sh_flush_fn
 
 
 def shard_views(num_views: int, rank: int, world: int) -> List[int]:
@@ -50,6 +76,88 @@
         self.replicas = []
         self.active = 0
         self.before_accumulate = None
+        self.deferred = False
+        self.deferred_early_flush = True
+        self._param_ids = frozenset(id(p) for p in self.params)
+        self.residue_pool_size = SH_FLUSH_MAX_VIEWS
+        self._residues = {}
+        self._residues_used = {}
+        self._pending_sh = []
+        self.sh_flushes = 0
+
+
+    def begin_deferred(self, early_flush=True):
+        assert not self._pending_sh, "begin_deferred with views pending: flush_deferred first"
+        self.deferred = True
+        self.deferred_early_flush = bool(early_flush)
+
+    def wants_deferred(self, means3D, shs):
+        if not self.deferred or means3D is None or shs is None or means3D is shs:
+            return False
+        ids = self._param_ids
+        return id(means3D) in ids and id(shs) in ids and shs.dim() == 3 and shs.shape[1] >= 1
+
+    def deferred_pool_full(self, means3D):
+        key = (means3D.shape[0], means3D.device)
+        return self.deferred_early_flush and self._residues_used.get(key, 0) >= self.residue_pool_size
+
+    def sh_residue_for(self, leaf_means3D, leaf_shs, means3D, shs, campos, sh_degree):
+        assert self.deferred, "sh_residue_for outside begin_deferred / flush_deferred"
+        key = (means3D.shape[0], means3D.device)
+        pool = self._residues.setdefault(key, [])
+        used = self._residues_used.get(key, 0)
+        if used == len(pool):
+            pool.append(torch.empty(means3D.shape[0], 3, dtype=torch.float32, device=means3D.device))
+        self._residues_used[key] = used + 1
+        res = pool[used]
+        self._pending_sh.append((leaf_means3D, leaf_shs, means3D, shs, campos, int(sh_degree), res))
+        return res
+
+    def _slice_of(self, tensor):
+        for p, (off, n) in zip(self.params, self.slices):
+            if p is tensor:
+                return self.flat[off:off + n]
+        raise KeyError("not a registered parameter")
+
+    def flush_pending(self):
+        pending, self._pending_sh = self._pending_sh, []
+        self._residues_used = {}
+        if not pending:
+            return
+        from . import _lib
+        fn = sh_flush_entry()
+        k = 0
+        while k < len(pending):
+            leaf_m, leaf_s, m3, shs = pending[k][:4]
+            same = lambda e: e[0] is leaf_m and e[1] is leaf_s and e[2].data_ptr() == m3.data_ptr() and e[3].data_ptr() == shs.data_ptr()
+            run = []
+            while k < len(pending) and len(run) < SH_FLUSH_MAX_VIEWS and same(pending[k]):
+                run.append(pending[k])
+                k += 1
+            recs = (ShFlushView * len(run))(*[ShFlushView(e[4].data_ptr(), e[6].data_ptr(), e[5], shs.shape[1]) for e in run])
+            with _lib.on(m3.device) as stream:
+                _lib.call(fn, m3.shape[0], shs.shape[1], m3.data_ptr(), shs.data_ptr(), self._slice_of(leaf_s).data_ptr(),
+                          self._slice_of(leaf_m).data_ptr(), recs, len(run), stream)
+            self.sh_flushes += 1
+
+    def flush_deferred(self):
+        try:
+            self.flush_pending()
+        finally:
+            self.deferred = False
+            self._pending_sh = []
+            self._residues_used = {}
+
+    def _assert_flushed(self, what, segment=None):
+        if not self._pending_sh:
+            return
+        if segment is not None:
+            lo, hi = segment[0], segment[0] + segment[1]
+            slices = {id(p): sl for p, sl in zip(self.params, self.slices)}
+            touched = any(off < hi and lo < off + n for e in self._pending_sh for off, n in (slices[id(e[0])], slices[id(e[1])]))
+            if not touched:
+                return
+        raise AssertionError(f"GradBucket.{what} with deferred SH gradients pending: flush_deferred() first")
 
     def select(self, k: int):
         while len(self.replicas) < k:
@@ -75,6 +183,7 @@
         return None
 
     def zero(self):
+        self._assert_flushed("zero")
         self.flat.zero_()
         for p, (off, n) in zip(self.params, self.slices):
             if p.grad is None or p.grad.data_ptr() != self.flat.data_ptr() + 4 * off:
@@ -89,6 +198,7 @@
 
     def all_reduce_async(self, dist, segment=None, after=(), timing=False, wire_dtype=None):
         off, n = segment if segment is not None else (0, self.flat.numel())
+        self._assert_flushed("all_reduce_async", (off, n))
         buf = self.flat[off:off + n]
         if dist.get_backend() != "nccl" or not self.flat.is_cuda:
             for ev in after:
@@ -122,6 +232,7 @@
         return self
 
     def wait(self):
+        self._assert_flushed("wait")
         if getattr(self, "_pending", False):
             torch.cuda.current_stream(self.flat.device).wait_stream(self._comm)
             self._pending = False
@@ -152,6 +263,7 @@
             dist.all_reduce(buf, op=dist.ReduceOp.SUM)
 
     def all_reduce(self, dist, average_over: int = 0):
+        self._assert_flushed("all_reduce")
         if dist.get_backend() == "nccl":
             dist.all_reduce(self.flat, op=dist.ReduceOp.SUM)
         else:
@@ -194,26 +306,36 @@
             prefetch_ahead=1):
         results = []
         views = list(views)
+        begin_deferred = getattr(sink, "begin_deferred", None) if backward_fn is not None else None
+        flush_deferred = getattr(sink, "flush_deferred", None) if begin_deferred is not None else None
         if not self.streams:
-            for i, v in enumerate(views):
-                obj = forward_fn(v)
-                if prefetch_fn is not None and i + 1 < len(views):
-                    prefetch_fn(views[i + 1])
-                if backward_fn is not None:
-                    if texture_ready is not None and sink is not None and i == len(views) - 1:
-                        sink.before_accumulate = lambda: texture_ready([])
-                    try:
-                        backward_fn(obj)
-                    finally:
-                        if sink is not None:
-                            sink.before_accumulate = None
-                results.append(obj)
+            if flush_deferred is not None:
+                begin_deferred()
+            try:
+                for i, v in enumerate(views):
+                    obj = forward_fn(v)
+                    if prefetch_fn is not None and i + 1 < len(views):
+                        prefetch_fn(views[i + 1])
+                    if backward_fn is not None:
+                        if texture_ready is not None and sink is not None and i == len(views) - 1:
+                            sink.before_accumulate = lambda: texture_ready([])
+                        try:
+                            backward_fn(obj)
+                        finally:
+                            if sink is not None:
+                                sink.before_accumulate = None
+                    results.append(obj)
+            finally:
+                if flush_deferred is not None:
+                    flush_deferred()
             return results
         if order not in ("backward", "accumulate", "none"):
             raise ValueError(order)
         if sink is None and order != "backward":
             order = "backward"
         cur = torch.cuda.current_stream(self.device)
+        if flush_deferred is not None:
+            begin_deferred(early_flush=order != "none")
         for s in self.streams:
             s.wait_stream(cur)
         prev_bwd = None
@@ -261,4 +383,6 @@
                 cur.wait_stream(s)
             if sink is not None and order == "none":
                 sink.fold()
+            if flush_deferred is not None:
+                flush_deferred()
         return results
diff --git a/texture-gs_amd/texgs/rasterizer.py b/texture-gs_amd/texgs/rasterizer.py
--- a/texture-gs_amd/texgs/rasterizer.py
+++ b/texture-gs_amd/texgs/rasterizer.py
@@ -537,7 +537,7 @@
 
 
 def backward_raw(s: _State, dL_dcolor, dL_ddepth, dL_dnorm, dL_dalpha, sinks=None, before_accumulate=None,
-                 want=_lib.WANT_ALL):
+                 want=_lib.WANT_ALL, defer_sh=None):
     lib = _lib.load()
     if not s.tensors["for_backward"]:
         raise RuntimeError("this forward ran with for_backward=False (no survivor lists were kept): its backward cannot run")
@@ -584,13 +584,23 @@
                            _ptr(outs.get("shs")), _ptr(outs.get("opacities")), _ptr(outs.get("scales")), _ptr(outs.get("rotations")),
                            _ptr(outs.get("uvs")), _ptr(d_tex), _ptr(outs.get("color_offset")), _ptr(outs.get("cov3D")), want,
                            _ptr(bins.rec) if bins else None, _ptr(bins.cursor) if bins else None,
-                           _ptr(bins.base) if bins else None, bins.cap if bins else 0, mask)
+                           _ptr(bins.base) if bins else None, bins.cap if bins else 0, mask, None)
         refs = [C.byref(x) for x in (s.frame, s.inputs, s.geom, s.bin, s.img, grads)]
-        if before_accumulate is None:
+        defer = defer_sh is not None and want_g and "shs" in outs and "means3D" in sinks and "shs" in sinks
+        if before_accumulate is None and not defer:
             _lib.call(lib.texgs_backward, *refs, stream)
         else:
             _lib.call(lib.texgs_backward_render, *refs, stream)
-            before_accumulate()
+            if before_accumulate is not None:
+                before_accumulate()
+            if defer:
+                bucket, leaf_m, leaf_s = defer_sh
+                if bucket.deferred_pool_full(a.means3D):
+                    bucket.flush_pending()
+                campos = s.tensors["keep"][-1]
+                assert campos.data_ptr() == s.frame.campos
+                residue = bucket.sh_residue_for(leaf_m, leaf_s, a.means3D, a.shs, campos, s.frame.sh_degree)
+                grads.dL_dvd_residue = residue.data_ptr()
             _lib.call(lib.texgs_backward_preprocess, *refs[:3], refs[5], stream)
     if bins is not None:
         bins.after_call()
@@ -658,9 +668,12 @@
             bucket = bool(sinks)
         if not bucket and DIRECT_LEAF_GRADS:
             sinks = {k: g for k, g in ((k, _leaf_grad_sink(v)) for k, v in ctx.named.items()) if g is not None}
+        wants_deferred = getattr(ctx.grad_sink, "wants_deferred", None) if bucket else None
+        defer = wants_deferred is not None and wants_deferred(ctx.named["means3D"], ctx.named["shs"])
         d_means3D, d_means2D, d_shs, d_op, d_scales, d_rot, d_uvs, d_tex = backward_raw(
             s, dL_dcolor, dL_ddepth, dL_dnorm, dL_dalpha, sinks=sinks or None,
-            before_accumulate=getattr(ctx.grad_sink, "before_accumulate", None) if bucket else None, want=ctx.want)
+            before_accumulate=getattr(ctx.grad_sink, "before_accumulate", None) if bucket else None, want=ctx.want,
+            defer_sh=(ctx.grad_sink, ctx.named["means3D"], ctx.named["shs"]) if defer else None)
         d_coff = s.tensors.get("d_color_offset")
         d_cov = s.tensors.get("d_cov3D")
         ctx.state = None
```

After: 1033 views/s (median of 6 runs). 1.01x the previous value.
